# njspix/frender

Measured on AMD Instinct MI355X. Metric: M reads/sec scanned+classified (96 samples, 8+8bp, n=1) at 1/2/4/8 MI355X, higher is better.
Workload: dtype u8; 1 GPU; BASELINE config 2: 100000000 SYN-v1 reads/GPU, 96 samples, 8+8bp, n=1, R=8 (74 B/record), decoded FASTQ resident in HBM; reads_per_gpu=100000000, bytes_per_record=74, samples=96, nsubs=1, rc=False, unique_codes=1383958, table_checksum=a89b0e2c6adb2921, parallelism=1 GPU

## Files before the change

frender_amd/_lib.py:

```python
from __future__ import annotations

import ctypes as C
import os

import numpy as np

from . import _runtime

torch = None
if _runtime.USE_TORCH:
    try:
        import torch
    except Exception:
        torch = None

HERE = os.path.dirname(os.path.abspath(__file__))
LIB_PATH = os.environ.get("FRENDER_HIP_LIB", os.path.join(HERE, "libfrender_hip.so"))


def source_tree_hash() -> str:
    import hashlib

    h = hashlib.sha256()
    csrc = os.path.join(HERE, "csrc")
# ... 720 lines not shown
    def exotic_table(self):
        n, nb, npres = C.c_uint64(), C.c_uint64(), C.c_uint64()
        self._ck(lib.fr_exotic_sizes(self.h, C.byref(n), C.byref(nb), C.byref(npres)), "fr_exotic_sizes")
        counts = np.empty(n.value, np.uint64)
        first = np.empty(n.value, np.uint64)
        offs = np.empty(n.value + 1, np.uint64)
        data = np.empty(max(nb.value, 1), np.uint8)
        pc = np.empty(npres.value, np.uint32)
        pf = np.empty(npres.value, np.uint32)
        self._ck(lib.fr_get_exotic_table(self.h, _ptr(counts), _ptr(first), _ptr(offs), _ptr(data), _ptr(pc),
                                         _ptr(pf)), "fr_get_exotic_table")
        raw = data.tobytes()
        o = offs.tolist()
        codes = [raw[o[i]:o[i + 1]] for i in range(n.value)]
        return codes, counts, first, pc, pf

    def classify(self, num_subs: int, rc: bool, to_host: bool = True):
        n = self.U if to_host else 0
        out = {k: (np.empty(n, dtype=np.int16) if to_host else None) for k in ("m1", "m2", "row", "rc_m2", "rc_row")}
        out["cls"] = np.empty(n, dtype=np.uint8) if to_host else None
        out["rc_cls"] = np.empty(n, dtype=np.uint8) if to_host else None
        eu, ew = C.c_int64(), C.c_int32()
        self._ck(lib.fr_classify(self.h, num_subs, 1 if rc else 0, _ptr(out["m1"]), _ptr(out["m2"]),
                                 _ptr(out["cls"]), _ptr(out["row"]), _ptr(out["rc_m2"]), _ptr(out["rc_cls"]),
                                 _ptr(out["rc_row"]), C.byref(eu), C.byref(ew)), "fr_classify")
        out["err_unique"], out["err_which"] = eu.value, ew.value
        return out

    def rc_counts(self):
        f = np.zeros(max(self.n_names, 1), dtype=np.uint64)
        r = np.zeros(max(self.n_names, 1), dtype=np.uint64)
        self._ck(lib.fr_rc_counts(self.h, _ptr(f), _ptr(r)), "fr_rc_counts")
        return f[:self.n_names], r[:self.n_names]

    def classify_cp(self, q1: list, q2: list, num_subs: int, rc: bool):
        n = len(q1)
        stride = self.cp_stride
        a1 = np.zeros((n, stride), dtype=np.uint32)
        a2 = np.zeros((n, stride), dtype=np.uint32)
        for i, (x, y) in enumerate(zip(q1, q2)):
            a1[i, :min(len(x), stride)] = [ord(c) for c in x[:stride]]
            a2[i, :min(len(y), stride)] = [ord(c) for c in y[:stride]]
        l1 = np.array([len(x) for x in q1], dtype=np.int32)
        l2 = np.array([len(y) for y in q2], dtype=np.int32)
        out = {k: np.empty(n, dtype=np.int16) for k in ("m1", "m2", "row", "rc_m2", "rc_row")}
        out["cls"] = np.empty(n, dtype=np.uint8)
        out["rc_cls"] = np.empty(n, dtype=np.uint8)
        out["err"] = np.zeros(n, dtype=np.int32)
        self._ck(lib.fr_classify_cp(self.h, n, _ptr(a1), _ptr(l1), _ptr(a2), _ptr(l2), stride, num_subs,
                                    1 if rc else 0, _ptr(out["m1"]), _ptr(out["m2"]), _ptr(out["cls"]),
                                    _ptr(out["row"]), _ptr(out["rc_m2"]), _ptr(out["rc_cls"]), _ptr(out["rc_row"]),
                                    _ptr(out["err"])), "fr_classify_cp")
        return out

    def device_alloc(self, nbytes: int) -> int:
        p = lib.fr_device_alloc(self.h, nbytes)
        if not p:
            raise FrenderError(f"fr_device_alloc({nbytes}) failed")
        return p

    def device_free(self, p: int):
        self._ck(lib.fr_device_free(self.h, P(p)), "fr_device_free")

    def copy_to_host(self, dev_ptr: int, nbytes: int) -> bytes:
        out = np.empty(nbytes, dtype=np.uint8)
        self._ck(lib.fr_copy_to_host(self.h, _ptr(out), P(dev_ptr), nbytes), "fr_copy_to_host")
        return out.tobytes()

    def copy_to_device(self, dev_ptr: int, data: bytes):
        a = np.frombuffer(data, dtype=np.uint8)
        self._ck(lib.fr_copy_to_device(self.h, P(dev_ptr), _ptr(a), a.size), "fr_copy_to_device")

    def synth_device(self, dev_ptr: int, r0: int, n: int, R: int, seed: int, idx1: list, idx2: list):
        L1, L2 = len(idx1[0]), len(idx2[0])
        self._ck(lib.fr_synth_device(self.h, P(dev_ptr), r0, n, R, seed, "".join(idx1).encode(),
                                     "".join(idx2).encode(), len(idx1), L1, L2), "fr_synth_device")

    def timing(self) -> Timing:
        t = Timing()
        self._ck(lib.fr_get_timing(self.h, C.byref(t)), "fr_get_timing")
        return t

    def diag(self) -> dict:
        v = np.zeros(24, dtype=np.uint64)
        self._ck(lib.fr_get_diag(self.h, _ptr(v), 24), "fr_get_diag")
        d = dict(zip(("spin_max", "spin_total", "keys", "overflow", "presence", "exotic", "grid", "slots"),
                     v[:8].tolist()))
        d["spec_replays"] = int(v[16])
        d["exo_replays"] = int(v[17])
        d["chunk_tiles"] = int(v[18])
        d["heavy_launches"] = int(v[19])
        d["big_rollbacks"] = int(v[20])
        d["fold_max"] = int(v[21])
        d["fold_over"] = int(v[22])
        d["feed_step"] = int(v[23])
        if v[8:16].any():
            names = ("guess", "walk0", "wait0", "resolve", "walk1", "commit", "kernel", "chunks")
            d["stamps"] = dict(zip(names, v[8:].tolist()))
        return d

    def sync(self):
        self._ck(lib.fr_sync(self.h), "fr_sync")

    def set_timing(self, on: bool):
        self._ck(lib.fr_set_timing(self.h, 1 if on else 0), "fr_set_timing")

    def export_unique_device(self, keys_ptr: int, counts_ptr: int, first_ptr: int, cap: int):
        _torch_stream_done(self.device)
        self._ck(lib.fr_export_unique_device(self.h, P(keys_ptr), P(counts_ptr), P(first_ptr), cap),
                 "fr_export_unique_device")

    def merge_unique_device(self, keys_ptr: int, counts_ptr: int, first_ptr: int, n: int):
        self._ck(lib.fr_merge_unique_device(self.h, P(keys_ptr), P(counts_ptr), P(first_ptr), n),
                 "fr_merge_unique_device")

    def export_partitioned(self, world: int):
        U = int(self.U)
        dev = torch.device("cuda", self.device)
        rows = torch.empty((max(U, 1), 3), dtype=torch.int64, device=dev)
        cnt = torch.empty(2 * world, dtype=torch.int64, device=dev)
        _torch_stream_done(self.device)
        self._ck(lib.fr_export_partitioned_device(self.h, int(world), P(rows.data_ptr()), P(cnt.data_ptr()),
                                                  max(U, 1)), "fr_export_partitioned_device")
        return rows[:U], cnt[:world]

    def merge_rows_rowmajor(self, rows):
        n = int(rows.shape[0])
        if not n:
            return
        rows = rows.contiguous()
        torch.cuda.current_stream(rows.device).synchronize()
        self._ck(lib.fr_merge_rows_device(self.h, P(rows.data_ptr()), n), "fr_merge_rows_device")
        self.sync()

    def export_rows(self, device):
        U = int(self.U)
        cols = torch.empty((3, max(U, 1)), dtype=torch.int64, device=torch.device("cuda", self.device))
        if U:
            self.export_unique_device(cols[0].data_ptr(), cols[1].data_ptr(), cols[2].data_ptr(), U)
        return cols[:, :U].t().to(device)

    def merge_rows(self, rows):
        n = int(rows.shape[0])
        if not n:
            return
        cols = rows.t().contiguous().to(torch.device("cuda", self.device))
        torch.cuda.current_stream(cols.device).synchronize()
        self.merge_unique_device(cols[0].data_ptr(), cols[1].data_ptr(), cols[2].data_ptr(), n)
        self.sync()
```

frender_amd/csrc/fr_api.hip:

```cpp
#include <hip/hip_runtime.h>

#include <algorithm>
#include <cstddef>
#include <cstdio>
#include <cstdlib>
#include <cstring>
#include <string>
#include <thread>
#include <unordered_map>
#include <vector>

#include "../../include/frender_amd.h"
#include "fr_internal.h"

using namespace fr;

static void pinned_copy(u8* dst, const u8* src, u64 n) {
    constexpr u64 PART = 16ull << 20;
    const unsigned hw = std::max(1u, std::thread::hardware_concurrency());
    const u64 k = std::min<u64>({8, hw, n / PART});
    if (k < 2) {
        std::memcpy(dst, src, n);
        return;
    }
    std::vector<std::thread> t;
    const u64 per = (n + k - 1) / k;
    for (u64 i = 1; i < k; ++i) {
        const u64 b = i * per, e = std::min(n, b + per);
        if (b < e) t.emplace_back([=] { std::memcpy(dst + b, src + b, e - b); });
    }
    std::memcpy(dst, src, std::min(n, per));
    for (auto& x : t) x.join();
}

struct fr_ctx {
    int device = 0;
    GSlot* snap = nullptr;
    u64 snap_cap = 0;
    hipStream_t stream = nullptr;
    hipStream_t copy = nullptr;
    std::string err;
    int grid = 0;
    u32 flush_at = NS * 3 / 4;
    u64* cold = nullptr;
    u32 cold_cap = 8192;
    LogEntry* log = nullptr;
    u64 log_cap = 0;
    u32 log_rcap = 0;
    LogEntry* log_sub = nullptr;
    u32 log_scap = 0;
    void* log_temp = nullptr;
    size_t log_temp_bytes = 0;
    u32 log_min = 0;
    u32 log_hot = 0xFFFFFFFFu;
    uint4* rare = nullptr;

    DevState* st = nullptr;
    DevState* h_st = nullptr;
    DevState* h_zero = nullptr;
    u8* h_byte = nullptr;
    u64* h_fin = nullptr;
    hipEvent_t fin_e0 = nullptr, fin_e1 = nullptr;
    hipEvent_t cls_e0 = nullptr, cls_e1 = nullptr;
    bool fin_pending = false;
    u64 fin_expect = 0;
    bool st_fresh = false;
    Table* d_tab = nullptr;
    Table* h_tab = nullptr;
    hipEvent_t st_ev = nullptr;
    bool st_pending = false;
    u64* tiles = nullptr;
    u64* chunk_info = nullptr;
    u64 tiles_cap = 0;
    bool spec_ok = true;
    u64 spec_replays = 0;
    u64 big_rollbacks = 0;
    bool grow_sync = false;
    u32 spec_commit = 0;
    u32 epoch = 0;
    u32 par = 0;

    Table tab{};
    u64 nslots = 0;

    u64 chunk_bytes = 0;
    u64 ring_bytes = 0;
    u64 feed_keys = ~0ull;
    bool feed_logged = true;
    u32 feed_fold_max = 0;
    u32 feed_fold_over = 0;
    u64 feed_step = 0;
    u32 chunk_tiles = 320;
    u32 chunk_tiles_heavy = 448;
    u32 ramp_up_s = 1, ramp_down_s = 1;
    u32 ramp_down_pct = 100;
    u32 ramp_down_pct_h = 70;
    bool ramp = true;
    u8* pin[2] = {nullptr, nullptr};
    u8* dbuf[2] = {nullptr, nullptr};
    hipEvent_t copied[2] = {nullptr, nullptr};
    hipEvent_t consumed[2] = {nullptr, nullptr};
    bool used[2] = {false, false};
    int cur = 0;
    std::vector<u8> carry;

    bool scanning = false;
    bool file_open = false;
    u32 file_tag = 0;
    u32 first_tag = 0;
    u32 pres_defer_tag = 0;
    u64 file_base = 0;
    bool merged = false;
    u64 max_file_bytes = 0;
    u64 file_offset = 0;
    i64 max_records = 0;
    int last_byte = -1;
    u64 pres_before = 0;
    struct ExoCode {
        u64 count, first;
        u32 last_tag;
        u32 last_pair;
    };
    std::unordered_map<std::string, u32> exo_index;
    std::vector<std::string> exo_str;
    std::vector<ExoCode> exo_codes;
    std::vector<u32> exo_pres_code, exo_pres_file;
    std::vector<u64> exo_pres_count;
    u64 exo_new_file = 0;
    u64 exo_records_file = 0;
    bool host_feed = false;
    ScanArgs last_args{};
    int last_grid = 0;
    bool last_valid = false;
    u64 exo_replays = 0;
    bool sample_done = false;

    int S = -1;
    int n_names = 0;
    int L1u = -1, L2u = -1;
    u64 *d_i1 = nullptr, *d_i2 = nullptr, *d_i2rc = nullptr;
    int32_t* d_name = nullptr;
    u32 *d_cp1 = nullptr, *d_cp2 = nullptr, *d_cp2rc = nullptr;
    int32_t *d_cpl1 = nullptr, *d_cpl2 = nullptr;
    u8* d_sheet = nullptr;
    u8* h_sheet = nullptr;
    u64 sheet_cap = 0;
    u64 sheet_bytes = 0;
    int cp_stride = 0;
    int32_t* d_canon = nullptr;
    u64 sheet_ver = 0;

    u8* d_nbr = nullptr;
    u64 nbr_cap = 0;
    u64 nbr_ver = ~0ull;
    int nbr_nsubs = -1, nbr_rc = 0;
    NbrMap nbr{};
    bool nbr_enabled = true;

    u64 U = 0;
    u64 ucap = 0;
    u64 *d_keys = nullptr, *d_counts = nullptr, *d_first = nullptr;
    u64 *d_keys_s = nullptr, *d_counts_s = nullptr, *d_first_s = nullptr;
    u32 *d_pos = nullptr, *d_perm = nullptr, *d_rank = nullptr;
    u64* d_counter = nullptr;
    void* d_temp = nullptr;
    size_t temp_bytes = 0;
    u32 *d_bins = nullptr, *d_binbase = nullptr;
    u64 bins_cap = 0;
    u32* d_arr = nullptr;
    u64 arr_cap = 0;
    FinRow* d_rows = nullptr;
    u64 rows_cap = 0;
    u64 n_pres = 0;
    u64 pmap_cap = 0;
    u32 *d_pres_u = nullptr, *d_pres_f = nullptr;
    u64* d_pres_c = nullptr;
    u64 n_exo = 0;

    u64 ccap = 0;
    int16_t *d_m1 = nullptr, *d_m2 = nullptr, *d_row = nullptr, *d_rm2 = nullptr, *d_rrow = nullptr;
    u8 *d_cls = nullptr, *d_rcls = nullptr;
    int32_t* d_errw = nullptr;
    u64* d_errf = nullptr;
    u64 *d_rcf = nullptr, *d_rcr = nullptr;
    int rc_names_cap = 0;

    std::vector<hipEvent_t> ev_a, ev_b, ev_l;
    size_t ev_used = 0;
    u64 scan_launches = 0, scan_bytes = 0;
    double classify_ms = 0, finalize_ms = 0;
    bool timing = true;
    bool fin_timed = false;

    fr_infl* infl = nullptr;
};

namespace fr {
int infl_bgzf_file(fr_infl* z, const char* path, int* ok, const uint8_t** dev_out, uint64_t* out_len,
                   uint64_t* members);
}

#define CK(x)                                                                                  \
    do {                                                                                       \
        hipError_t e_ = (x);                                                                   \
        if (e_ != hipSuccess) {                                                                \
            ctx->err = std::string(#x) + ": " + hipGetErrorString(e_);                         \
            return FR_ERR_HIP;                                                                 \
        }                                                                                      \
    } while (0)

static int fail(fr_ctx* ctx, int code, const std::string& msg) {
    ctx->err = msg;
    return code;
}

template <class T>
static hipError_t dalloc(T** p, u64 n) {
    return hipMalloc((void**)p, std::max<u64>(n, 1) * sizeof(T));
}

static u64 pow2_at_least(u64 x) {
    u64 p = 1;
    while (p < x) p <<= 1;
    return p;
}

static int state_reset_counts(fr_ctx* ctx) {
    if (ctx->st_pending) CK(hipStreamSynchronize(ctx->stream));
    *ctx->h_st = *ctx->h_zero;
    CK(hipMemcpyAsync(ctx->st, ctx->h_zero, sizeof(DevState), hipMemcpyHostToDevice, ctx->stream));
    ctx->st_pending = false;
    ctx->st_fresh = true;
    return FR_OK;
}

static int read_state(fr_ctx* ctx) {
    if (ctx->st_fresh && !ctx->st_pending) return FR_OK;
    CK(hipMemcpyAsync(ctx->h_st, ctx->st, sizeof(DevState), hipMemcpyDeviceToHost, ctx->stream));
    CK(hipStreamSynchronize(ctx->stream));
    ctx->st_pending = false;
    ctx->st_fresh = true;
    return FR_OK;
}

static int grow_table(fr_ctx* ctx, bool force_bigger) {
    int rc = read_state(ctx);
    if (rc) return rc;
    const u64 nkeys = ctx->h_st->n_keys;
    const u64 novf = std::min<u64>(ctx->h_st->n_overflow, ctx->tab.ovf_cap);
    if (force_bigger || (nkeys + novf) * 2 > ctx->nslots) {
        u64 ns = ctx->nslots;
        while ((nkeys + novf) * 4 > ns) ns <<= 1;
        if (ns == ctx->nslots) ns <<= 1;
        GSlot* ns_slots = nullptr;
        CK(dalloc(&ns_slots, ns));
        CK(launch_table_init(ns_slots, ns, ctx->stream));
        Table t = ctx->tab;
        t.slots = ns_slots;
        t.mask = ns - 1;
        CK(launch_rehash(t, ctx->st, ctx->tab.slots, ctx->nslots, ctx->stream));
        CK(hipStreamSynchronize(ctx->stream));
        CK(hipFree(ctx->tab.slots));
        ctx->tab = t;
        ctx->nslots = ns;
    }
    if (novf) {
        Overflow* old = ctx->tab.ovf;
        Overflow* fresh = nullptr;
        CK(dalloc(&fresh, ctx->tab.ovf_cap));
        ctx->tab.ovf = fresh;
        CK(hipMemsetAsync(&ctx->st->n_overflow, 0, sizeof(u64), ctx->stream));
        CK(launch_reinsert_overflow(ctx->tab, ctx->st, old, novf, ctx->stream));
        ctx->st_fresh = false;
        CK(hipStreamSynchronize(ctx->stream));
        CK(hipFree(old));
    }
    return FR_OK;
}

static int ensure_presence_cap(fr_ctx* ctx) {
    int rc = read_state(ctx);
    if (rc) return rc;
    const u64 need = ctx->h_st->n_presence + ctx->h_st->n_keys + 1024;
    if (need <= ctx->tab.pres_cap) return FR_OK;
    u64 ncap = ctx->tab.pres_cap;
    while (ncap < need * 2) ncap *= 2;
    Presence* np = nullptr;
    CK(dalloc(&np, ncap));
    CK(hipMemcpyAsync(np, ctx->tab.pres, std::min(ctx->h_st->n_presence, ctx->tab.pres_cap) * sizeof(Presence),
                      hipMemcpyDeviceToDevice, ctx->stream));
    CK(hipStreamSynchronize(ctx->stream));
    CK(hipFree(ctx->tab.pres));
    ctx->tab.pres = np;
    ctx->tab.pres_cap = ncap;
    return FR_OK;
}

static int flush_presence(fr_ctx* ctx) {
    if (!ctx->pres_defer_tag) return FR_OK;
    int rc = ensure_presence_cap(ctx);
    if (rc) return rc;
    ctx->st_fresh = false;
    CK(launch_presence_scan(ctx->tab.slots, ctx->nslots, ctx->pres_defer_tag, ctx->tab.pres, ctx->tab.pres_cap,
                            ctx->st, ctx->stream));
    ctx->pres_defer_tag = 0;
    return read_state(ctx);
}

static int maybe_grow(fr_ctx* ctx) {
    if (ctx->st_pending) {
        if (ctx->grow_sync) CK(hipEventSynchronize(ctx->st_ev));
        else if (hipEventQuery(ctx->st_ev) != hipSuccess) return FR_OK;
        ctx->st_pending = false;
    } else if (!ctx->st_fresh) {
        return FR_OK;
    }
    const DevState& s = *ctx->h_st;
    if (s.n_overflow || s.n_keys * 2 > ctx->nslots) return grow_table(ctx, false);
    return FR_OK;
}

static int snapshot_async(fr_ctx* ctx) {
    CK(hipMemcpyAsync(ctx->h_st, ctx->st, sizeof(DevState), hipMemcpyDeviceToHost, ctx->stream));
    CK(hipEventRecord(ctx->st_ev, ctx->stream));
    ctx->st_pending = true;
    return FR_OK;
}

static int settle_finalize(fr_ctx* ctx) {
    if (!ctx->fin_pending) return FR_OK;
    ctx->fin_pending = false;
    CK(hipEventSynchronize(ctx->fin_e1));
    float ms = 0;
    if (ctx->fin_timed) CK(hipEventElapsedTime(&ms, ctx->fin_e0, ctx->fin_e1));
    ctx->finalize_ms = ms;
    if (*ctx->h_fin != ctx->fin_expect) return fail(ctx, FR_ERR_DEVICE, "compaction count mismatch");
    return FR_OK;
}

static int upload_table(fr_ctx* ctx) {
    if (std::memcmp(&ctx->tab, ctx->h_tab, sizeof(Table)) != 0) {
        CK(hipStreamSynchronize(ctx->stream));
        std::memcpy(ctx->h_tab, &ctx->tab, sizeof(Table));
        CK(hipMemcpyAsync(ctx->d_tab, ctx->h_tab, sizeof(Table), hipMemcpyHostToDevice, ctx->stream));
    }
    return FR_OK;
}

static int grow_exotic(fr_ctx* ctx, u64 need, u64 need_bytes) {
    if (need > ctx->tab.exo_cap) {
        CK(hipStreamSynchronize(ctx->stream));
        const u64 cap = std::max<u64>(need + need / 4, 2 * ctx->tab.exo_cap);
        CK(hipFree(ctx->tab.exo_ord));
        CK(hipFree(ctx->tab.exo_off));
        CK(hipFree(ctx->tab.exo_len));
        ctx->tab.exo_ord = nullptr;
        ctx->tab.exo_off = nullptr;
        ctx->tab.exo_len = nullptr;
        CK(dalloc(&ctx->tab.exo_ord, cap));
        CK(dalloc(&ctx->tab.exo_off, cap));
        CK(dalloc(&ctx->tab.exo_len, cap));
        ctx->tab.exo_cap = cap;
    }
    if (need_bytes > ctx->tab.exo_pool_cap) {
        CK(hipStreamSynchronize(ctx->stream));
        const u64 cap = std::max<u64>(need_bytes + need_bytes / 4, 2 * ctx->tab.exo_pool_cap);
        CK(hipFree(ctx->tab.exo_pool));
        ctx->tab.exo_pool = nullptr;
        CK(dalloc(&ctx->tab.exo_pool, cap));
        ctx->tab.exo_pool_cap = cap;
    }
    return upload_table(ctx);
}

static int drain_exotic(fr_ctx* ctx) {
    DevState& s = *ctx->h_st;
    const u64 n = s.n_exotic, used = s.exo_pool_used;
    if (!n) return FR_OK;
    if (n > ctx->tab.exo_cap || used > ctx->tab.exo_pool_cap)
        return fail(ctx, FR_ERR_DEVICE, "exotic list drained while overflowed");
    std::vector<u64> ord(n), off(n);
    std::vector<u32> len(n);
    std::vector<u8> pool(used);
    CK(hipMemcpyAsync(ord.data(), ctx->tab.exo_ord, n * 8, hipMemcpyDeviceToHost, ctx->stream));
    CK(hipMemcpyAsync(off.data(), ctx->tab.exo_off, n * 8, hipMemcpyDeviceToHost, ctx->stream));
    CK(hipMemcpyAsync(len.data(), ctx->tab.exo_len, n * 4, hipMemcpyDeviceToHost, ctx->stream));
    if (used) CK(hipMemcpyAsync(pool.data(), ctx->tab.exo_pool, used, hipMemcpyDeviceToHost, ctx->stream));
    CK(hipMemsetAsync(&ctx->st->n_exotic, 0, 2 * sizeof(u64), ctx->stream));
    CK(hipStreamSynchronize(ctx->stream));
    s.n_exotic = 0;
    s.exo_pool_used = 0;
    for (u64 i = 0; i < n; ++i) {
        std::string code((const char*)pool.data() + off[i], len[i]);
        auto it = ctx->exo_index.find(code);
        u32 k;
        if (it == ctx->exo_index.end()) {
            k = (u32)ctx->exo_codes.size();
            ctx->exo_index.emplace(code, k);
            ctx->exo_str.push_back(std::move(code));
            ctx->exo_codes.push_back({0, ~0ull, 0, 0});
        } else {
            k = it->second;
        }
        auto& e = ctx->exo_codes[k];
        e.count += 1;
        e.first = std::min(e.first, ord[i]);
        const u32 tag = (u32)(ord[i] >> ORD_SHIFT);
        if (e.last_tag != tag) {
            e.last_tag = tag;
            e.last_pair = (u32)ctx->exo_pres_code.size();
            ctx->exo_pres_code.push_back(k);
            ctx->exo_pres_file.push_back(tag - 1u);
            ctx->exo_pres_count.push_back(0);
            ctx->exo_new_file++;
        }
        ctx->exo_pres_count[e.last_pair] += 1;
    }
    ctx->exo_records_file += n;
    return FR_OK;
}

static int launch_args(fr_ctx* ctx, const ScanArgs& a, int grid);

static int replay_exotic(fr_ctx* ctx) {
    if (!ctx->last_valid) return fail(ctx, FR_ERR_DEVICE, "exotic overflow without a launch to replay");
    DevState& s = *ctx->h_st;
    int rc = grow_exotic(ctx, s.n_exotic, s.exo_pool_used);
    if (rc) return rc;
    s.n_exotic = 0;
    s.exo_pool_used = 0;
    s.cap_flags &= ~4u;
    CK(hipMemsetAsync(&ctx->st->n_exotic, 0, 2 * sizeof(u64), ctx->stream));
    CK(hipMemcpyAsync(&ctx->st->cap_flags, &s.cap_flags, sizeof(u32), hipMemcpyHostToDevice, ctx->stream));
    ScanArgs a = ctx->last_args;
    a.exo_only = 1;
    a.spec_commit = 0;
    a.log = nullptr;
    a.epoch = ++ctx->epoch;
    a.tab = ctx->d_tab;
    a.tabv = ctx->tab;
    CK(hipMemsetAsync(&ctx->st->ticket, 0, 2 * sizeof(u32), ctx->stream));
    rc = launch_args(ctx, a, ctx->last_grid);
    if (rc) return rc;
    ctx->exo_replays++;
    ctx->st_fresh = false;
    rc = read_state(ctx);
    if (rc) return rc;
    if (ctx->h_st->cap_flags & 4u) return fail(ctx, FR_ERR_DEVICE, "exotic replay overflowed");
    return FR_OK;
}

static int settle_exotic(fr_ctx* ctx) {
    int rc = read_state(ctx);
    if (rc) return rc;
    if (ctx->h_st->cap_flags & 4u) {
        rc = replay_exotic(ctx);
        if (rc) return rc;
    }
    return drain_exotic(ctx);
}

static int launch_args(fr_ctx* ctx, const ScanArgs& a, int grid) {
    if (a.num_tiles > ctx->tiles_cap) return fail(ctx, FR_ERR_INVALID, "range larger than the look-back array");
    ctx->st_fresh = false;
    CK(launch_chunk_scan(a, grid, ctx->stream));
    return FR_OK;
}

static int launch_range(fr_ctx* ctx, const u8* dptr, u64 len, u64 avail, int own_start, int own_end, int pre_valid,
                        int exo_only = 0) {
    if (len == 0) return FR_OK;
    int rc = FR_OK;
    if (ctx->host_feed && ctx->last_valid) {
        rc = settle_exotic(ctx);
        if (rc) return rc;
    }
    rc = maybe_grow(ctx);
    if (rc) return rc;
    ScanArgs a;
    std::memset(&a, 0, sizeof(a));
    a.buf = dptr;
    a.len = len;
    a.avail = avail;
    a.file_offset = ctx->file_offset;
    a.file_tag = ctx->file_tag;
    a.par = ctx->par;
    a.epoch = ++ctx->epoch;
    a.num_tiles = (u32)((len + TSTEP - 1) / TSTEP);
    a.own_start = own_start;
    a.own_end = own_end;
    a.pre_valid = pre_valid;
    a.flush_at = ctx->flush_at;
    a.max_records = ctx->max_records;
    a.st = ctx->st;
    a.tiles = ctx->tiles;
    a.chunk_info = ctx->chunk_info;
    a.spec_commit = exo_only ? 0u : ctx->spec_commit;
    a.exo_only = (u32)exo_only;
    rc = upload_table(ctx);
    if (rc) return rc;
    a.tab = ctx->d_tab;
    a.tabv = ctx->tab;
    if (ctx->epoch >= 0x7FFFFFFFu) {
        CK(hipMemsetAsync(ctx->tiles, 0, ctx->tiles_cap * sizeof(u64), ctx->stream));
        ctx->epoch = 1;
        a.epoch = 1;
    }
    ctx->st_fresh = false;
    const bool timed = ctx->timing;
    if (timed && ctx->ev_used == ctx->ev_a.size()) {
        hipEvent_t e1, e2, e3;
        CK(hipEventCreate(&e1));
        CK(hipEventCreate(&e2));
        CK(hipEventCreate(&e3));
        ctx->ev_a.push_back(e1);
        ctx->ev_b.push_back(e2);
        ctx->ev_l.push_back(e3);
    }
    if (timed) CK(hipEventRecord(ctx->ev_a[ctx->ev_used], ctx->stream));
    const u64 G = (u64)ctx->grid, C = ctx->chunk_tiles, Ch = ctx->chunk_tiles_heavy;
    const u64 Gd = std::max<u64>(1, G * ctx->ramp_down_pct / 100), Gdh = std::max<u64>(1, G * ctx->ramp_down_pct_h / 100);
    a.ramp_up_s = ctx->ramp_up_s;
    a.ramp_down_s = ctx->ramp_down_s;
    a.ramp_down_g = (u32)Gd;
    a.ramp_down_g_h = (u32)Gdh;
    auto ramps = [&](u64 c, u64 gd) {
        return ramp_tiles_before(c, G, std::min<u64>(ctx->ramp_up_s, c), G) +
               ramp_tiles_before(c, gd, std::min<u64>(ctx->ramp_down_s, c), gd);
    };
    const u64 rg = ramps(C, Gd), rgh = ramps(Ch, Gdh);
    if (ctx->ramp && (u64)a.num_tiles >= rg + C) {
        a.ramp_g = (u32)G;
        a.chunk_tiles = (u32)C;
        a.mid_chunks = (u32)(((u64)a.num_tiles - rg + C - 1) / C);
        a.num_chunks = (u32)(G + Gd) + a.mid_chunks;
        if (Ch != C && (u64)a.num_tiles >= rgh + Ch) {
            a.chunk_tiles_h = (u32)Ch;
            a.mid_chunks_h = (u32)(((u64)a.num_tiles - rgh + Ch - 1) / Ch);
            a.num_chunks_h = (u32)(G + Gdh) + a.mid_chunks_h;
        }
    } else {
        a.ramp_g = 0;
        a.mid_chunks = 0;
        a.chunk_tiles = (u32)std::max<u64>(1, (a.num_tiles + G - 1) / G);
        a.num_chunks = (a.num_tiles + a.chunk_tiles - 1) / a.chunk_tiles;
    }
    a.cold_cap = ctx->cold_cap;
    a.cold = ctx->cold;
    a.log = exo_only ? nullptr : LOG_DIRECT ? ctx->log_sub : ctx->log;
    a.log_cap = LOG_DIRECT ? (u64)ctx->log_scap * LOG_NSUB : ctx->log_cap;
    a.log_rcap = LOG_DIRECT ? ctx->log_scap : ctx->log_rcap;
    a.log_min = ctx->log_min;
    a.log_hot = ctx->log_hot;
    a.rare = ctx->rare;
    const int grid = (int)std::min<u64>(a.num_chunks, G);
    rc = launch_args(ctx, a, grid);
    if (rc) return rc;
    ctx->last_args = a;
    ctx->last_grid = grid;
    ctx->last_valid = true;
    if (timed) CK(hipEventRecord(ctx->ev_b[ctx->ev_used], ctx->stream));
    if (a.log)
        CK(launch_log_aggregate(ctx->tab, ctx->st, ctx->log, ctx->log_rcap, ctx->log_sub, ctx->log_scap, a.file_tag,
                                a.file_offset, ctx->stream));
    if (timed) {
        CK(hipEventRecord(ctx->ev_l[ctx->ev_used], ctx->stream));
        ctx->ev_used++;
    }
    ctx->scan_launches++;
    ctx->scan_bytes += len;
    ctx->par ^= 1u;
    ctx->file_offset += len;
    ctx->max_file_bytes = std::max(ctx->max_file_bytes, ctx->file_offset);
    return snapshot_async(ctx);
}

extern "C" {

void fr_tuning_defaults(fr_tuning* t) {
    if (!t) return;
    const fr_ctx d{};
    std::memset(t, 0, sizeof(*t));
    t->size = sizeof(fr_tuning);
    t->grid = 0;
    t->flush_at = d.flush_at;
    t->cold_cap = d.cold_cap;
    t->log = 1;
    t->log_min = d.log_min;
    t->log_hot = d.log_hot;
    t->chunk_tiles = d.chunk_tiles;
    t->chunk_tiles_heavy = d.chunk_tiles_heavy;
    t->ramp = d.ramp ? 1 : 0;
    t->ramp_up_s = d.ramp_up_s;
    t->ramp_down_s = d.ramp_down_s;
    t->ramp_down_pct = d.ramp_down_pct;
    t->ramp_down_pct_h = d.ramp_down_pct_h;
    t->spec_commit = d.spec_ok ? 1 : 0;
    t->nbr = d.nbr_enabled ? 1 : 0;
    t->ovf_cap = 0;
}

fr_ctx* fr_create(int device, uint64_t chunk_bytes, uint64_t table_slots) {
    return fr_create_tuned(device, chunk_bytes, table_slots, nullptr);
}

fr_ctx* fr_create_tuned(int device, uint64_t chunk_bytes, uint64_t table_slots, const fr_tuning* tuning) {
    fr_tuning t;
    fr_tuning_defaults(&t);
    if (tuning) {
        const size_t n = std::min<size_t>(std::max<uint32_t>(tuning->size, sizeof(uint32_t)), sizeof(fr_tuning));
        std::memcpy((char*)&t + sizeof(uint32_t), (const char*)tuning + sizeof(uint32_t), n - sizeof(uint32_t));
    }
    fr_ctx* ctx = new fr_ctx();
    ctx->device = device;
    auto bad = [&](const char* what, hipError_t e) {
        ctx->err = std::string(what) + ": " + hipGetErrorString(e);
        return ctx;
    };
    hipError_t e;
    if ((e = hipSetDevice(device)) != hipSuccess) return bad("hipSetDevice", e);
    if ((e = hipStreamCreateWithFlags(&ctx->stream, hipStreamNonBlocking)) != hipSuccess) return bad("stream", e);
    if ((e = hipStreamCreateWithFlags(&ctx->copy, hipStreamNonBlocking)) != hipSuccess) return bad("stream", e);
    hipDeviceProp_t prop;
    if ((e = hipGetDeviceProperties(&prop, device)) != hipSuccess) return bad("props", e);
    const int per_cu = chunk_occupancy();
    ctx->grid = t.grid > 0 ? t.grid : prop.multiProcessorCount * per_cu;
    ctx->flush_at = std::min<u32>(t.flush_at, NS);
    ctx->nbr_enabled = t.nbr != 0;
    ctx->cold_cap = std::max<u32>(1024, t.cold_cap);
    ctx->log_min = t.log_min;
    ctx->log_hot = std::max<u32>(1, t.log_hot);
    ctx->chunk_tiles = std::max<u32>(2, t.chunk_tiles);
    ctx->chunk_tiles_heavy = std::max<u32>(2, t.chunk_tiles_heavy);
    ctx->ramp = t.ramp != 0;
    ctx->ramp_up_s = std::max<u32>(1, t.ramp_up_s);
    ctx->ramp_down_s = std::max<u32>(1, t.ramp_down_s);
    ctx->ramp_down_pct = std::min<u32>(100, std::max<u32>(1, t.ramp_down_pct));
    ctx->ramp_down_pct_h = std::min<u32>(100, std::max<u32>(1, t.ramp_down_pct_h));
    ctx->spec_ok = t.spec_commit != 0;
    if ((e = dalloc(&ctx->cold, 2ull * ctx->cold_cap * (u64)ctx->grid)) != hipSuccess) return bad("cold lists", e);
    if ((e = dalloc(&ctx->rare, (u64)RARE_RING * (u64)ctx->grid)) != hipSuccess) return bad("rare rings", e);

    ctx->chunk_bytes = chunk_bytes ? ((chunk_bytes + TILE - 1) / TILE) * TILE : (256ull << 20);
    if (ctx->chunk_bytes > RANGE_MAX) ctx->chunk_bytes = RANGE_MAX;
    ctx->ring_bytes = std::min<u64>(ctx->chunk_bytes, HOST_CHUNK_MAX);
    if (t.log) {
        const u64 want = std::min<u64>(std::max<u64>(ctx->chunk_bytes / 256, 1ull << 16), 1ull << 26);
        ctx->log_rcap = (u32)(want / LOG_NR);
        ctx->log_cap = (u64)ctx->log_rcap * LOG_NR;
        ctx->log_scap = (u32)std::max<u64>(2ull * ctx->log_rcap / LOG_SUBS, 64);
        if (!LOG_DIRECT && (e = dalloc(&ctx->log, ctx->log_cap)) != hipSuccess) return bad("launch log", e);
        if ((e = dalloc(&ctx->log_sub, (u64)ctx->log_scap * LOG_NSUB)) != hipSuccess) return bad("launch log parts", e);
    }
    ctx->tiles_cap = RANGE_MAX / TSTEP + 2;
    ctx->nslots = pow2_at_least(std::max<u64>(table_slots, 1024));
    if ((e = hipMalloc((void**)&ctx->st, sizeof(DevState))) != hipSuccess) return bad("state", e);
    if ((e = hipMalloc((void**)&ctx->d_tab, sizeof(Table))) != hipSuccess) return bad("table copy", e);
    if ((e = hipHostMalloc((void**)&ctx->h_tab, sizeof(Table), hipHostMallocDefault)) != hipSuccess)
        return bad("table staging", e);
    std::memset(ctx->h_tab, 0, sizeof(Table));
    if ((e = hipHostMalloc((void**)&ctx->h_st, sizeof(DevState), hipHostMallocDefault)) != hipSuccess)
        return bad("pinned state", e);
    if ((e = hipHostMalloc((void**)&ctx->h_byte, 64, hipHostMallocDefault)) != hipSuccess) return bad("pinned byte", e);
    if ((e = hipHostMalloc((void**)&ctx->h_fin, 64, hipHostMallocDefault)) != hipSuccess) return bad("pinned count", e);
    if ((e = hipEventCreate(&ctx->fin_e0)) != hipSuccess) return bad("event", e);
    if ((e = hipEventCreate(&ctx->fin_e1)) != hipSuccess) return bad("event", e);
    if ((e = hipEventCreate(&ctx->cls_e0)) != hipSuccess) return bad("event", e);
    if ((e = hipEventCreate(&ctx->cls_e1)) != hipSuccess) return bad("event", e);
    if ((e = hipHostMalloc((void**)&ctx->h_zero, sizeof(DevState), hipHostMallocDefault)) != hipSuccess)
        return bad("pinned reset state", e);
    std::memset(ctx->h_zero, 0, sizeof(DevState));
    ctx->h_zero->err_nospace = ~0ull;
    if ((e = hipEventCreateWithFlags(&ctx->st_ev, hipEventDisableTiming)) != hipSuccess) return bad("event", e);
    if ((e = dalloc(&ctx->tiles, ctx->tiles_cap)) != hipSuccess) return bad("tiles", e);
    if ((e = dalloc(&ctx->chunk_info, ctx->tiles_cap)) != hipSuccess) return bad("chunk info", e);
    if ((e = hipMemset(ctx->tiles, 0, ctx->tiles_cap * sizeof(u64))) != hipSuccess) return bad("tiles", e);
    if ((e = dalloc(&ctx->tab.slots, ctx->nslots)) != hipSuccess) return bad("table", e);
    ctx->tab.mask = ctx->nslots - 1;
    ctx->tab.ovf_cap = t.ovf_cap ? std::max<u64>(t.ovf_cap, 1024) : (1ull << 22);
    ctx->tab.pres_cap = 1ull << 22;
    ctx->tab.exo_cap = 1ull << 20;
    ctx->tab.exo_pool_cap = 64ull << 20;
    if ((e = dalloc(&ctx->tab.ovf, ctx->tab.ovf_cap)) != hipSuccess) return bad("overflow", e);
    if ((e = dalloc(&ctx->tab.pres, ctx->tab.pres_cap)) != hipSuccess) return bad("presence", e);
    if ((e = dalloc(&ctx->tab.exo_ord, ctx->tab.exo_cap)) != hipSuccess) return bad("exotic", e);
    if ((e = dalloc(&ctx->tab.exo_off, ctx->tab.exo_cap)) != hipSuccess) return bad("exotic", e);
    if ((e = dalloc(&ctx->tab.exo_len, ctx->tab.exo_cap)) != hipSuccess) return bad("exotic", e);
    if ((e = dalloc(&ctx->tab.exo_pool, ctx->tab.exo_pool_cap)) != hipSuccess) return bad("exotic", e);
    for (int i = 0; i < 2; ++i) {
        if ((e = hipHostMalloc((void**)&ctx->pin[i], ctx->ring_bytes, hipHostMallocDefault)) != hipSuccess)
            return bad("pinned ring", e);
        if ((e = dalloc(&ctx->dbuf[i], ctx->ring_bytes + 64)) != hipSuccess) return bad("device ring", e);
        if ((e = hipEventCreateWithFlags(&ctx->copied[i], hipEventDisableTiming)) != hipSuccess) return bad("event", e);
        if ((e = hipEventCreateWithFlags(&ctx->consumed[i], hipEventDisableTiming)) != hipSuccess)
            return bad("event", e);
        if ((e = hipEventRecord(ctx->consumed[i], ctx->stream)) != hipSuccess) return bad("event", e);
    }
    if ((e = dalloc(&ctx->d_counter, 1)) != hipSuccess) return bad("counter", e);
    if (fr_reset(ctx) != FR_OK) return ctx;
    ctx->err.clear();
    return ctx;
}

void fr_destroy(fr_ctx* ctx) {
    if (!ctx) return;
    if (ctx->infl) fr_infl_destroy(ctx->infl);
    (void)hipSetDevice(ctx->device);
    if (ctx->stream) (void)hipStreamSynchronize(ctx->stream);
    if (ctx->copy) (void)hipStreamSynchronize(ctx->copy);
    void* dev[] = {ctx->st, ctx->d_tab, ctx->tiles, ctx->tab.slots, ctx->tab.ovf, ctx->tab.pres, ctx->tab.exo_ord,
                   ctx->tab.exo_off, ctx->tab.exo_len, ctx->tab.exo_pool, ctx->dbuf[0], ctx->dbuf[1], ctx->d_sheet,
                   ctx->d_keys, ctx->d_counts, ctx->d_first, ctx->d_keys_s, ctx->d_counts_s,
                   ctx->d_first_s, ctx->d_pos, ctx->d_perm, ctx->d_rank, ctx->d_counter, ctx->d_temp, ctx->d_bins, ctx->d_binbase, ctx->d_arr, ctx->d_rows, ctx->d_pres_u,
                   ctx->d_pres_f, ctx->d_pres_c, ctx->d_m1, ctx->d_m2, ctx->d_row, ctx->d_rm2, ctx->d_rrow, ctx->d_cls, ctx->d_rcls,
                   ctx->d_errw, ctx->d_errf, ctx->d_nbr, ctx->cold, ctx->rare, ctx->chunk_info, ctx->log, ctx->log_sub, ctx->log_temp,
                   ctx->snap};
    for (void* p : dev)
        if (p) (void)hipFree(p);
    if (ctx->h_st) (void)hipHostFree(ctx->h_st);
    if (ctx->h_zero) (void)hipHostFree(ctx->h_zero);
    if (ctx->h_byte) (void)hipHostFree(ctx->h_byte);
    if (ctx->h_fin) (void)hipHostFree(ctx->h_fin);
    if (ctx->fin_e0) (void)hipEventDestroy(ctx->fin_e0);
    if (ctx->fin_e1) (void)hipEventDestroy(ctx->fin_e1);
    if (ctx->cls_e0) (void)hipEventDestroy(ctx->cls_e0);
    if (ctx->cls_e1) (void)hipEventDestroy(ctx->cls_e1);
    if (ctx->h_sheet) (void)hipHostFree(ctx->h_sheet);
    if (ctx->h_tab) (void)hipHostFree(ctx->h_tab);
    for (int i = 0; i < 2; ++i) {
        if (ctx->pin[i]) (void)hipHostFree(ctx->pin[i]);
        if (ctx->copied[i]) (void)hipEventDestroy(ctx->copied[i]);
        if (ctx->consumed[i]) (void)hipEventDestroy(ctx->consumed[i]);
    }
    for (auto e : ctx->ev_a) (void)hipEventDestroy(e);
    for (auto e : ctx->ev_b) (void)hipEventDestroy(e);
    for (auto e : ctx->ev_l) (void)hipEventDestroy(e);
    if (ctx->st_ev) (void)hipEventDestroy(ctx->st_ev);
    if (ctx->stream) (void)hipStreamDestroy(ctx->stream);
    if (ctx->copy) (void)hipStreamDestroy(ctx->copy);
    delete ctx;
}

const char* fr_last_error(const fr_ctx* ctx) { return ctx ? ctx->err.c_str() : "null context"; }

int fr_get_diag(fr_ctx* ctx, uint64_t* out, int n) {
    if (int src = settle_finalize(ctx)) return src;
    int rc = read_state(ctx);
    if (rc) return rc;
    const DevState& s = *ctx->h_st;
    const uint64_t v[] = {s.spin_max,   s.spin_total, s.n_keys,   s.n_overflow, s.n_presence, s.n_exotic,
                          (uint64_t)ctx->grid, ctx->nslots, s.stamp[0], s.stamp[1], s.stamp[2], s.stamp[3],
                          s.stamp[4],  s.stamp[5],  s.stamp[6], s.stamp[7], ctx->spec_replays, ctx->exo_replays,
                          s.heavy[ctx->par] ? ctx->chunk_tiles_heavy : ctx->chunk_tiles,
                          s.heavy_launches, ctx->big_rollbacks, ctx->feed_fold_max, ctx->feed_fold_over, ctx->feed_step};
    for (int i = 0; i < n && i < (int)(sizeof(v) / sizeof(v[0])); ++i) out[i] = v[i];
    return FR_OK;
}

int fr_sync(fr_ctx* ctx) {
    CK(hipStreamSynchronize(ctx->stream));
    CK(hipStreamSynchronize(ctx->copy));
    return settle_finalize(ctx);
}

int fr_get_timing(fr_ctx* ctx, fr_timing* out) {
    CK(hipStreamSynchronize(ctx->stream));
    if (int src = settle_finalize(ctx)) return src;
    double tot = 0, last = 0, lg = 0;
    for (size_t i = 0; i < ctx->ev_used; ++i) {
        float ms = 0, ml = 0;
        CK(hipEventElapsedTime(&ms, ctx->ev_a[i], ctx->ev_b[i]));
        CK(hipEventElapsedTime(&ml, ctx->ev_b[i], ctx->ev_l[i]));
        tot += ms;
        last = ms;
        lg += ml;
    }
    out->log_ms = lg;
    out->scan_launches = ctx->scan_launches;
    out->scan_bytes = ctx->scan_bytes;
    out->scan_ms = tot;
    out->last_scan_ms = last;
    out->classify_ms = ctx->classify_ms;
    out->finalize_ms = ctx->finalize_ms;
    return FR_OK;
}

int fr_set_timing(fr_ctx* ctx, int on) {
    if (!ctx) return FR_ERR_INVALID;
    ctx->timing = on != 0;
    return FR_OK;
}

int fr_set_sheet(fr_ctx* ctx, int S, const uint64_t* idx1_packed, const int32_t* idx1_len,
                 const uint64_t* idx2_packed, const int32_t* idx2_len, const uint64_t* idx2rc_packed,
                 const int32_t* name_id, int n_names, const uint32_t* idx1_cp, const uint32_t* idx2_cp,
                 const uint32_t* idx2rc_cp, int cp_stride) {
    if (S < 0 || S > 32767) return fail(ctx, FR_ERR_INVALID, "sheet rows must be in [0, 32767]");
    const bool with_cp = idx1_cp && idx2_cp && idx2rc_cp && cp_stride > 0 && S > 0;
    const u64 ncp = with_cp ? (u64)S * cp_stride : 0;
    auto al = [](u64 b) { return (b + 7) & ~7ull; };
    const u64 o_i2 = al(S * 8ull), o_i2rc = o_i2 + al(S * 8ull), o_name = o_i2rc + al(S * 8ull);
    const u64 o_cp1 = o_name + al(S * 4ull), o_cp2 = o_cp1 + al(ncp * 4), o_cp2rc = o_cp2 + al(ncp * 4);
    const u64 o_l1 = o_cp2rc + al(ncp * 4), o_l2 = o_l1 + (with_cp ? al(S * 4ull) : 0);
    const u64 o_canon = o_l2 + (with_cp ? al(S * 4ull) : 0);
    const u64 total = o_canon + al(3 * S * 4ull) + 8;
    std::vector<u8> blob(total, 0);
    u8* h = blob.data();
    if (S) {
        std::memcpy(h, idx1_packed, S * 8ull);
        std::memcpy(h + o_i2, idx2_packed, S * 8ull);
        std::memcpy(h + o_i2rc, idx2rc_packed, S * 8ull);
        std::memcpy(h + o_name, name_id, S * 4ull);
    }
    if (with_cp) {
        std::memcpy(h + o_cp1, idx1_cp, ncp * 4);
        std::memcpy(h + o_cp2, idx2_cp, ncp * 4);
        std::memcpy(h + o_cp2rc, idx2rc_cp, ncp * 4);
        std::memcpy(h + o_l1, idx1_len, S * 4ull);
        std::memcpy(h + o_l2, idx2_len, S * 4ull);
    }
    const bool same = ctx->h_sheet && total == ctx->sheet_bytes && std::memcmp(h, ctx->h_sheet, o_canon) == 0;
    if (!same && S) {
        const uint64_t* lists[3] = {idx1_packed, idx2_packed, idx2rc_packed};
        int32_t* canon = (int32_t*)(h + o_canon);
        for (int l = 0; l < 3; ++l) {
            std::unordered_map<u64, int32_t> first;
            first.reserve(S * 2);
            for (int i = 0; i < S; ++i) canon[l * S + i] = first.emplace(lists[l][i], i).first->second;
        }
    }
    if (!same) {
        CK(hipStreamSynchronize(ctx->stream));
        if (total > ctx->sheet_cap) {
            if (ctx->d_sheet) CK(hipFree(ctx->d_sheet));
            if (ctx->h_sheet) CK(hipHostFree(ctx->h_sheet));
            ctx->d_sheet = nullptr;
            ctx->h_sheet = nullptr;
            const u64 cap = std::max<u64>(total * 2, 4096);
            CK(hipMalloc(&ctx->d_sheet, cap));
            CK(hipHostMalloc(&ctx->h_sheet, cap, hipHostMallocDefault));
            ctx->sheet_cap = cap;
        }
        std::memcpy(ctx->h_sheet, h, total);
        ctx->sheet_bytes = total;
        ++ctx->sheet_ver;
        CK(hipMemcpyAsync(ctx->d_sheet, ctx->h_sheet, total, hipMemcpyHostToDevice, ctx->stream));
    }
    u8* d = ctx->d_sheet;
    ctx->d_i1 = (u64*)d;
    ctx->d_i2 = (u64*)(d + o_i2);
    ctx->d_i2rc = (u64*)(d + o_i2rc);
    ctx->d_name = (int32_t*)(d + o_name);
    ctx->d_cp1 = with_cp ? (u32*)(d + o_cp1) : nullptr;
    ctx->d_cp2 = with_cp ? (u32*)(d + o_cp2) : nullptr;
    ctx->d_cp2rc = with_cp ? (u32*)(d + o_cp2rc) : nullptr;
    ctx->d_cpl1 = with_cp ? (int32_t*)(d + o_l1) : nullptr;
    ctx->d_cpl2 = with_cp ? (int32_t*)(d + o_l2) : nullptr;
    ctx->d_canon = (int32_t*)(d + o_canon);
    ctx->cp_stride = with_cp ? cp_stride : 0;
    ctx->S = S;
    ctx->n_names = n_names;
    auto common = [&](const int32_t* l) {
        if (S == 0) return -1;
        for (int i = 1; i < S; ++i)
            if (l[i] != l[0]) return -2;
        return (int)l[0];
    };
    ctx->L1u = common(idx1_len);
    ctx->L2u = common(idx2_len);
    return FR_OK;
}

int fr_reset(fr_ctx* ctx) {
    if (int src = settle_finalize(ctx)) return src;
    CK(hipSetDevice(ctx->device));
    CK(hipStreamSynchronize(ctx->copy));
    CK(launch_table_init(ctx->tab.slots, ctx->nslots, ctx->stream));
    int rc = state_reset_counts(ctx);
    if (rc) return rc;
    ctx->scanning = true;
    ctx->file_open = false;
    ctx->file_tag = 0;
    ctx->first_tag = 0;
    ctx->pres_defer_tag = 0;
    ctx->merged = false;
    ctx->max_file_bytes = 0;
    ctx->par = 0;
    ctx->U = 0;
    ctx->n_pres = 0;
    ctx->n_exo = 0;
    ctx->exo_index.clear();
    ctx->exo_str.clear();
    ctx->exo_codes.clear();
    ctx->exo_pres_code.clear();
    ctx->exo_pres_file.clear();
    ctx->exo_pres_count.clear();
    ctx->last_valid = false;
    ctx->ev_used = 0;
    ctx->scan_launches = ctx->scan_bytes = 0;
    ctx->classify_ms = ctx->finalize_ms = 0;
    ctx->st_pending = false;
    return FR_OK;
}

int fr_begin_file(fr_ctx* ctx, int64_t max_records) {
    return fr_begin_file_at(ctx, (int64_t)ctx->file_tag, 0, max_records);
}

int fr_begin_file_at(fr_ctx* ctx, int64_t file_index, uint64_t byte_base, int64_t max_records) {
    if (int src = settle_finalize(ctx)) return src;
    if (ctx->file_open) return fail(ctx, FR_ERR_INVALID, "fr_begin_file: a file is already open");
    if (file_index < 0 || file_index + 1 >= (1 << 19)) return fail(ctx, FR_ERR_INVALID, "too many files in one scan");
    if ((u32)file_index + 1u <= ctx->file_tag)
        return fail(ctx, FR_ERR_INVALID, "fr_begin_file_at: file indices must increase within a scan");
    if (byte_base >= (1ull << ORD_SHIFT)) return fail(ctx, FR_ERR_INVALID, "fr_begin_file_at: byte base too large");
    int rc = flush_presence(ctx);
    if (rc) return rc;
    rc = read_state(ctx);
    if (rc) return rc;
    ctx->pres_before = ctx->h_st->n_presence;
    ctx->exo_new_file = 0;
    ctx->exo_records_file = 0;
    ctx->last_valid = false;
    static_assert(offsetof(DevState, utf8_bad) + sizeof(u32) - offsetof(DevState, lines) == 32, "per-file block");
    CK(hipMemcpyAsync(&ctx->st->lines[0], &ctx->h_zero->lines[0], 32, hipMemcpyHostToDevice, ctx->stream));
    ctx->h_st->lines[0] = ctx->h_st->lines[1] = 0;
    ctx->h_st->err_nospace = ~0ull;
    ctx->h_st->nonascii = ctx->h_st->utf8_bad = 0;
    ctx->file_tag = (u32)file_index + 1u;
    if (!ctx->first_tag) ctx->first_tag = ctx->file_tag;
    ctx->file_offset = byte_base;
    ctx->file_base = byte_base;
    ctx->max_records = max_records > 0 ? max_records : 0;
    ctx->last_byte = -1;
    ctx->carry.clear();
    ctx->sample_done = false;
    ctx->par = 0;
    ctx->file_open = true;
    return FR_OK;
}

static int check_sample(fr_ctx* ctx) {
    if (ctx->max_records <= 0) return FR_OK;
    int rc = read_state(ctx);
    if (rc) return rc;
    const u64 lines = ctx->h_st->lines[ctx->par];
    if (lines + 3 >= 4ull * (u64)ctx->max_records) ctx->sample_done = true;
    return FR_OK;
}

static int ship_slot(fr_ctx* ctx, int slot, u64 n) {
    CK(hipStreamWaitEvent(ctx->copy, ctx->consumed[slot], 0));
    CK(hipMemcpyAsync(ctx->dbuf[slot], ctx->pin[slot], n, hipMemcpyHostToDevice, ctx->copy));
    CK(hipEventRecord(ctx->copied[slot], ctx->copy));
    CK(hipStreamWaitEvent(ctx->stream, ctx->copied[slot], 0));
    int rc = launch_range(ctx, ctx->dbuf[slot], n, n, 1, 0, 0);
    if (rc) return rc;
    CK(hipEventRecord(ctx->consumed[slot], ctx->stream));
    ctx->used[slot] = true;
    return FR_OK;
}

int fr_feed(fr_ctx* ctx, const uint8_t* data, uint64_t len) {
    if (!ctx->file_open) return fail(ctx, FR_ERR_INVALID, "fr_feed: no open file");
    ctx->host_feed = true;
    if (ctx->sample_done) return FR_SAMPLE_DONE;
    if (len) ctx->last_byte = data[len - 1];
    u64 done = 0;
    while (done < len) {
        const int slot = ctx->cur;
        if (ctx->used[slot]) CK(hipEventSynchronize(ctx->copied[slot]));
        u8* pin = ctx->pin[slot];
        const u64 nc = ctx->carry.size();
        if (nc >= ctx->ring_bytes) return fail(ctx, FR_ERR_CAPACITY, "a line is longer than the chunk size");
        if (nc) std::memcpy(pin, ctx->carry.data(), nc);
        const u64 take = std::min<u64>(len - done, ctx->ring_bytes - nc);
        pinned_copy(pin + nc, data + done, take);
        done += take;
        const u64 n = nc + take;
        u64 cut = n;
        while (cut > 0 && !(pin[cut - 1] == '\n' || (pin[cut - 1] == '\r' && cut < n && pin[cut] != '\n'))) --cut;
        if (cut == 0) {
            ctx->carry.assign(pin, pin + n);
            continue;
        }
        ctx->carry.assign(pin + cut, pin + n);
        int rc = ship_slot(ctx, slot, cut);
        if (rc) return rc;
        ctx->cur ^= 1;
        rc = check_sample(ctx);
        if (rc) return rc;
        if (ctx->sample_done) return FR_SAMPLE_DONE;
    }
    return FR_OK;
}

int fr_feed_device(fr_ctx* ctx, const uint8_t* dev_data, uint64_t len) {
    if (!ctx->file_open) return fail(ctx, FR_ERR_INVALID, "fr_feed_device: no open file");
    if (ctx->file_offset != ctx->file_base || !ctx->carry.empty())
        return fail(ctx, FR_ERR_INVALID, "fr_feed_device takes a whole file (no prior fr_feed)");
    if (((uintptr_t)dev_data & 15u) != 0) return fail(ctx, FR_ERR_INVALID, "device data must be 16-byte aligned");
    ctx->host_feed = false;
    int rc = settle_exotic(ctx);
    if (rc) return rc;
    const DevState saved = *ctx->h_st;
    const u32 par0 = ctx->par;
    const u64 snap_slots = ctx->nslots;
    const bool empty = saved.n_keys == 0 && saved.n_overflow == 0;
    const bool spec = ctx->spec_ok && ctx->max_records == 0 && saved.n_overflow == 0;
    GSlot* snap = nullptr;
    if (spec && !empty) {
        if (ctx->snap_cap < snap_slots) {
            if (ctx->snap) {
                CK(hipStreamSynchronize(ctx->stream));
                CK(hipFree(ctx->snap));
                ctx->snap = nullptr;
            }
            ctx->snap_cap = 0;
            CK(dalloc(&ctx->snap, snap_slots));
            ctx->snap_cap = snap_slots;
        }
        snap = ctx->snap;
        CK(hipMemcpyAsync(snap, ctx->tab.slots, snap_slots * sizeof(GSlot), hipMemcpyDeviceToDevice, ctx->stream));
    }
    const double big_range = (double)std::min<u64>(ctx->chunk_bytes, len);
    const bool fold_room = (u64)ctx->feed_fold_over * 64 <= ctx->feed_fold_max && ctx->feed_step > 0 &&
                           (double)ctx->feed_fold_max * big_range <= 0.85 * AGG_LNS * (double)ctx->feed_step;
    bool big = spec && (!ctx->feed_logged || fold_room) && ctx->feed_keys != ~0ull &&
               (saved.n_keys + ctx->feed_keys) * 2 <= ctx->nslots;
    bool spec_now = spec;
    u64 step = 0, lim_room = ~0ull;
    for (int attempt = 0; attempt < 12; ++attempt) {
        CK(hipMemsetAsync(&ctx->st->log_fold_max, 0, 2 * sizeof(u32), ctx->stream));
        const u64 lim = std::min<u64>(big ? ctx->chunk_bytes : std::min<u64>(ctx->chunk_bytes, RANGE_FIRST_MAX),
                                      lim_room);
        const u64 nr = (len + lim - 1) / lim;
        step = nr ? (len + nr - 1) / nr : 0;
        ctx->spec_commit = spec_now ? 1u : 0u;
        for (u64 off = 0; off < len; off += step) {
            const u64 n = std::min<u64>(step, len - off);
            rc = launch_range(ctx, dev_data + off, n, len - off, off == 0 ? 1 : 0, 1, off ? 1 : 0);
            if (rc) break;
        }
        ctx->spec_commit = 0;
        if (!rc && len) CK(hipMemcpyAsync(ctx->h_byte, dev_data + len - 1, 1, hipMemcpyDeviceToHost, ctx->stream));
        if (!rc) rc = read_state(ctx);
        if (rc) break;
        const bool spec_bad = spec_now && ctx->h_st->spec_fail;
        const bool room_bad = spec && (ctx->h_st->cap_flags & 2u) && step > RANGE_ROOM_MIN;
        if (!spec_bad && !room_bad) break;
        if (room_bad) {
            big = false;
            lim_room = std::max<u64>(RANGE_ROOM_MIN, ((step / 8) + TILE - 1) / TILE * TILE);
            ctx->grow_sync = true;
            ctx->big_rollbacks++;
        } else {
            spec_now = false;
        }
        if (ctx->nslots != snap_slots) {
            GSlot* fresh = nullptr;
            if ((rc = (dalloc(&fresh, snap_slots) == hipSuccess) ? FR_OK : fail(ctx, FR_ERR_DEVICE, "rollback alloc")))
                break;
            CK(hipStreamSynchronize(ctx->stream));
            CK(hipFree(ctx->tab.slots));
            ctx->tab.slots = fresh;
            ctx->tab.mask = snap_slots - 1;
            ctx->nslots = snap_slots;
        }
        if (empty) CK(launch_table_init(ctx->tab.slots, ctx->nslots, ctx->stream));
        else CK(hipMemcpyAsync(ctx->tab.slots, snap, snap_slots * sizeof(GSlot), hipMemcpyDeviceToDevice, ctx->stream));
        *ctx->h_st = saved;
        CK(hipMemcpyAsync(ctx->st, ctx->h_st, sizeof(DevState), hipMemcpyHostToDevice, ctx->stream));
        CK(hipStreamSynchronize(ctx->stream));
        ctx->st_pending = false;
        ctx->st_fresh = true;
        ctx->par = par0;
        ctx->file_offset = ctx->file_base;
        if (!room_bad) ctx->spec_replays++;
    }
    ctx->grow_sync = false;
    if (rc) return rc;
    ctx->feed_keys = ctx->h_st->n_keys - saved.n_keys;
    ctx->feed_logged = ctx->h_st->log_commits != saved.log_commits;
    ctx->feed_fold_max = ctx->h_st->log_fold_max;
    ctx->feed_fold_over = ctx->h_st->log_fold_over;
    ctx->feed_step = step;
    rc = read_state(ctx);
    if (rc) return rc;
    if (ctx->h_st->cap_flags & 4u) {
        DevState& s = *ctx->h_st;
        rc = grow_exotic(ctx, s.n_exotic, s.exo_pool_used);
        if (rc) return rc;
        s.n_exotic = 0;
        s.exo_pool_used = 0;
        s.cap_flags &= ~4u;
        s.lines[par0] = saved.lines[par0];
        CK(hipMemcpyAsync(ctx->st, ctx->h_st, sizeof(DevState), hipMemcpyHostToDevice, ctx->stream));
        ctx->par = par0;
        ctx->file_offset = ctx->file_base;
        ctx->exo_replays++;
        for (u64 off = 0; off < len && !rc; off += step) {
            const u64 n = std::min<u64>(step, len - off);
            rc = launch_range(ctx, dev_data + off, n, len - off, off == 0 ? 1 : 0, 1, off ? 1 : 0, 1);
        }
        if (rc) return rc;
        ctx->st_fresh = false;
        rc = read_state(ctx);
        if (rc) return rc;
        if (ctx->h_st->cap_flags & 4u) return fail(ctx, FR_ERR_DEVICE, "exotic replay overflowed");
    }
    rc = drain_exotic(ctx);
    if (rc) return rc;
    if (len) ctx->last_byte = *ctx->h_byte;
    ctx->carry.clear();
    return FR_OK;
}

int fr_feed_bgzf(fr_ctx* ctx, const char* path, int* decoded, uint64_t* members, uint64_t* bytes) {
    if (!decoded || !path) return fail(ctx, FR_ERR_INVALID, "fr_feed_bgzf: null argument");
    *decoded = 0;
    if (members) *members = 0;
    if (bytes) *bytes = 0;
    if (!ctx->file_open) return fail(ctx, FR_ERR_INVALID, "fr_feed_bgzf: no open file");
    if (ctx->file_base != 0 || ctx->file_offset != 0 || !ctx->carry.empty())
        return fail(ctx, FR_ERR_INVALID, "fr_feed_bgzf takes a whole file from its first byte (no prior feed)");
    if (ctx->max_records > 0) return FR_OK;
    if (!ctx->infl) {
        ctx->infl = fr_infl_create(ctx->device);
        if (!ctx->infl || *fr_infl_last_error(ctx->infl)) {
            const std::string msg = ctx->infl ? fr_infl_last_error(ctx->infl) : "fr_infl_create returned NULL";
            if (ctx->infl) fr_infl_destroy(ctx->infl);
            ctx->infl = nullptr;
            return fail(ctx, FR_ERR_HIP, msg);
        }
    }
    int ok = 0;
    const uint8_t* dev = nullptr;
    uint64_t len = 0, n = 0;
    int rc = infl_bgzf_file(ctx->infl, path, &ok, &dev, &len, &n);
    if (rc) return fail(ctx, rc, std::string("fr_feed_bgzf: ") + fr_infl_last_error(ctx->infl));
    if (!ok) return FR_OK;
    rc = fr_feed_device(ctx, dev, len);
    if (rc) return rc;
    *decoded = 1;
    if (members) *members = n;
    if (bytes) *bytes = len;
    return FR_OK;
}

int fr_end_file(fr_ctx* ctx, fr_file_stats* out) {
    if (!ctx->file_open) return fail(ctx, FR_ERR_INVALID, "fr_end_file: no open file");
    if (!ctx->carry.empty() && !ctx->sample_done) {
        const int slot = ctx->cur;
        if (ctx->used[slot]) CK(hipEventSynchronize(ctx->copied[slot]));
        std::memcpy(ctx->pin[slot], ctx->carry.data(), ctx->carry.size());
        const u64 n = ctx->carry.size();
        ctx->carry.clear();
        int rc = ship_slot(ctx, slot, n);
        if (rc) return rc;
        ctx->cur ^= 1;
    }
    ctx->carry.clear();
    CK(hipStreamSynchronize(ctx->copy));
    int rc = ctx->host_feed ? settle_exotic(ctx) : FR_OK;
    if (rc) return rc;
    ctx->last_valid = false;
    rc = grow_table(ctx, false);
    if (rc) return rc;
    const bool defer = ctx->file_tag == ctx->first_tag && !ctx->merged && ctx->pres_before == 0 &&
                       ctx->h_st->n_presence == 0;
    if (!defer) {
        rc = ensure_presence_cap(ctx);
        if (rc) return rc;
        ctx->st_fresh = false;
        CK(launch_presence_scan(ctx->tab.slots, ctx->nslots, ctx->file_tag, ctx->tab.pres, ctx->tab.pres_cap,
                                ctx->st, ctx->stream));
    }
    rc = read_state(ctx);
    if (rc) return rc;
    const DevState& s = *ctx->h_st;
    if (s.spin_fail) return fail(ctx, FR_ERR_DEVICE, "tally look-back exceeded its spin bound");
    if (s.cap_flags) return fail(ctx, FR_ERR_CAPACITY, "a device list overflowed (flags " + std::to_string(s.cap_flags) + ")");
    u64 lines = s.lines[ctx->par];
    const bool ended = ctx->last_byte == '\n' || ctx->last_byte == '\r';
    if (ctx->last_byte >= 0 && !ended && !ctx->sample_done) lines += 1;
    u64 records = (lines + 3) / 4;
    if (ctx->max_records > 0 && records > (u64)ctx->max_records) records = (u64)ctx->max_records;
    std::memset(out, 0, sizeof(*out));
    out->records = records;
    out->lines = lines;
    out->new_keys = (defer ? s.n_keys : s.n_presence - ctx->pres_before) + ctx->exo_new_file;
    if (defer) ctx->pres_defer_tag = ctx->file_tag;
    out->exotic = ctx->exo_records_file;
    out->error = FR_SCAN_OK;
    if (s.utf8_bad) {
        out->error = FR_SCAN_UTF8;
        out->utf8_bad = 1;
    }
    if (s.err_nospace != ~0ull) {
        out->error = FR_SCAN_NO_SPACE;
        out->error_offset = s.err_nospace;
    }
    ctx->file_open = false;
    return FR_OK;
}

int fr_finalize(fr_ctx* ctx, uint64_t* n_unique, uint64_t* n_presence, uint64_t* n_exotic) {
    if (ctx->file_open) return fail(ctx, FR_ERR_INVALID, "fr_finalize: a file is still open");
    int rc = settle_finalize(ctx);
    if (rc) return rc;
    hipEvent_t e0 = ctx->fin_e0, e1 = ctx->fin_e1;
    rc = grow_table(ctx, false);
    if (rc) return rc;
    rc = read_state(ctx);
    if (rc) return rc;
    const u64 nk = ctx->h_st->n_keys;
    if (nk > 0xFFFFFFFFull) return fail(ctx, FR_ERR_CAPACITY, "more than 2^32 unique codes");
    if (nk > ctx->ucap) {
        void* old[] = {ctx->d_keys, ctx->d_counts, ctx->d_first, ctx->d_keys_s, ctx->d_counts_s, ctx->d_first_s,
                       ctx->d_pos, ctx->d_perm, ctx->d_rank, ctx->d_temp};
        for (void* p : old)
            if (p) CK(hipFree(p));
        ctx->d_temp = nullptr;
        ctx->temp_bytes = 0;
        const u64 cap = std::max<u64>(nk + nk / 4, 1024);
        CK(dalloc(&ctx->d_keys, cap));
        CK(dalloc(&ctx->d_counts, cap));
        CK(dalloc(&ctx->d_first, cap));
        CK(dalloc(&ctx->d_keys_s, cap));
        CK(dalloc(&ctx->d_counts_s, cap));
        CK(dalloc(&ctx->d_first_s, cap));
        CK(dalloc(&ctx->d_pos, cap));
        CK(dalloc(&ctx->d_perm, cap));
        CK(dalloc(&ctx->d_rank, cap));
        ctx->ucap = cap;
    }
    if (ctx->timing) CK(hipEventRecord(e0, ctx->stream));
    ctx->fin_timed = ctx->timing;
    BinMap bm{0, 0, 0, 0, 0};
    u64 nbins = 0;
    if (!ctx->merged && ctx->first_tag && ctx->file_tag >= ctx->first_tag) {
        const u64 ntags = (u64)(ctx->file_tag - ctx->first_tag) + 1u;
        bm.span = std::max<u64>(ctx->max_file_bytes, 1);
        bm.first_tag = ctx->first_tag;
        bm.shift = 13;
        const u64 range = ntags * bm.span;
        while (bm.shift < 20 && ((range >> bm.shift) + 1) > (1ull << 21)) ++bm.shift;
        nbins = (range >> bm.shift) + 1;
        if (nbins > (1ull << 21)) nbins = 0;
    }
    if (nbins) {
        bm.nbins = nbins;
        bm.cap = ctx->ucap;
        if (ctx->nslots > ctx->arr_cap) {
            if (ctx->d_arr) CK(hipFree(ctx->d_arr));
            ctx->d_arr = nullptr;
            CK(hipMalloc(&ctx->d_arr, ctx->nslots * sizeof(u32)));
            ctx->arr_cap = ctx->nslots;
        }
        if (ctx->ucap > ctx->rows_cap) {
            if (ctx->d_rows) CK(hipFree(ctx->d_rows));
            ctx->d_rows = nullptr;
            CK(hipMalloc(&ctx->d_rows, ctx->ucap * sizeof(FinRow)));
            ctx->rows_cap = ctx->ucap;
        }
        if (nbins + 1 > ctx->bins_cap) {
            if (ctx->d_bins) CK(hipFree(ctx->d_bins));
            if (ctx->d_binbase) CK(hipFree(ctx->d_binbase));
            ctx->d_bins = ctx->d_binbase = nullptr;
            const u64 cap = std::max<u64>(nbins + 1, 1u << 16);
            CK(hipMalloc(&ctx->d_bins, cap * sizeof(u32)));
            CK(hipMalloc(&ctx->d_binbase, cap * sizeof(u32)));
            ctx->bins_cap = cap;
        }
        size_t need = 0;
        CK(launch_fin_scan(ctx->d_bins, ctx->d_binbase, nbins + 1, nullptr, &need, ctx->stream));
        if (need > ctx->temp_bytes) {
            if (ctx->d_temp) CK(hipFree(ctx->d_temp));
            CK(hipMalloc(&ctx->d_temp, need));
            ctx->temp_bytes = need;
        }
        size_t tb = ctx->temp_bytes;
        const bool set_uidx = ctx->pres_defer_tag == 0;
        CK(hipMemsetAsync(ctx->d_bins, 0, (nbins + 1) * sizeof(u32), ctx->stream));
        CK(launch_fin_hist(ctx->tab.slots, ctx->nslots, bm, ctx->d_bins, ctx->d_arr, ctx->stream));
        CK(launch_fin_scan(ctx->d_bins, ctx->d_binbase, nbins + 1, ctx->d_temp, &tb, ctx->stream));
        CK(launch_fin_scatter(ctx->tab.slots, ctx->nslots, bm, ctx->d_binbase, ctx->d_arr, ctx->d_rows, ctx->stream));
        CK(launch_fin_rank(ctx->tab.slots, nk, bm, ctx->d_binbase, ctx->d_rows, ctx->d_keys_s, ctx->d_counts_s,
                           ctx->d_first_s, set_uidx, ctx->stream));
    } else {
        CK(hipMemsetAsync(ctx->d_counter, 0, sizeof(u64), ctx->stream));
        CK(launch_compact(ctx->tab.slots, ctx->nslots, ctx->d_keys, ctx->d_counts, ctx->d_first, ctx->d_pos,
                          ctx->d_counter, ctx->stream));
        int begin_bit = 0, end_bit = 64;
        if (!ctx->merged) {
            begin_bit = 2;
            end_bit = ORD_SHIFT;
            while (end_bit < 64 && ((u64)ctx->file_tag >> (end_bit - ORD_SHIFT)) != 0) ++end_bit;
            if (ctx->file_tag == ctx->first_tag) {
                end_bit = begin_bit + 1;
                while (end_bit < ORD_SHIFT && (ctx->max_file_bytes >> end_bit) != 0) ++end_bit;
            }
        }
        size_t need = 0;
        CK(launch_order(ctx->d_first, ctx->d_pos, nk, ctx->d_first_s, ctx->d_perm, nullptr, &need, begin_bit, end_bit,
                        ctx->stream));
        if (need > ctx->temp_bytes) {
            if (ctx->d_temp) CK(hipFree(ctx->d_temp));
            CK(hipMalloc(&ctx->d_temp, need));
            ctx->temp_bytes = need;
        }
        size_t tb = ctx->temp_bytes;
        if (nk)
            CK(launch_order(ctx->d_first, ctx->d_pos, nk, ctx->d_first_s, ctx->d_perm, ctx->d_temp, &tb, begin_bit,
                            end_bit, ctx->stream));
        CK(launch_gather(ctx->d_perm, nk, ctx->d_keys, ctx->d_counts, ctx->d_keys_s, ctx->d_counts_s, ctx->d_rank,
                         ctx->stream));
        CK(launch_set_uidx(ctx->tab.slots, ctx->tab.mask, ctx->d_keys_s, nk, ctx->d_rank, ctx->stream));
    }
    const u64 np = ctx->pres_defer_tag ? nk : std::min<u64>(ctx->h_st->n_presence, ctx->tab.pres_cap);
    if (np > ctx->pmap_cap) {
        if (ctx->d_pres_u) CK(hipFree(ctx->d_pres_u));
        if (ctx->d_pres_f) CK(hipFree(ctx->d_pres_f));
        if (ctx->d_pres_c) CK(hipFree(ctx->d_pres_c));
        CK(dalloc(&ctx->d_pres_u, np));
        CK(dalloc(&ctx->d_pres_f, np));
        CK(dalloc(&ctx->d_pres_c, np));
        ctx->pmap_cap = np;
    }
    if (ctx->pres_defer_tag)
        CK(launch_presence_one_file(ctx->d_counts_s, np, ctx->pres_defer_tag, ctx->d_pres_u, ctx->d_pres_f,
                                    ctx->d_pres_c, ctx->stream));
    else
        CK(launch_presence_map(ctx->tab.slots, ctx->tab.mask, ctx->tab.pres, np, ctx->d_pres_u, ctx->d_pres_f,
                               ctx->d_pres_c, ctx->stream));
    *ctx->h_fin = 0;
    if (nbins)
        CK(hipMemcpyAsync(ctx->h_fin, ctx->d_binbase + nbins, sizeof(u32), hipMemcpyDeviceToHost, ctx->stream));
    else
        CK(hipMemcpyAsync(ctx->h_fin, ctx->d_counter, sizeof(u64), hipMemcpyDeviceToHost, ctx->stream));
    CK(hipEventRecord(e1, ctx->stream));
    ctx->fin_pending = true;
    ctx->fin_expect = nk;
    ctx->U = nk;
    ctx->n_pres = np;
    ctx->n_exo = ctx->exo_codes.size();
    if (n_unique) *n_unique = ctx->U;
    if (n_presence) *n_presence = ctx->n_pres;
    if (n_exotic) *n_exotic = ctx->n_exo;
    return FR_OK;
}

int fr_get_unique(fr_ctx* ctx, uint64_t* keys, uint64_t* counts, uint64_t* first_ordinal) {
    if (int src = settle_finalize(ctx)) return src;
    const u64 n = ctx->U;
    if (!n) return FR_OK;
    if (keys) CK(hipMemcpy(keys, ctx->d_keys_s, n * 8, hipMemcpyDeviceToHost));
    if (counts) CK(hipMemcpy(counts, ctx->d_counts_s, n * 8, hipMemcpyDeviceToHost));
    if (first_ordinal) CK(hipMemcpy(first_ordinal, ctx->d_first_s, n * 8, hipMemcpyDeviceToHost));
    return FR_OK;
}

int fr_get_presence(fr_ctx* ctx, uint32_t* unique_idx, uint32_t* file_idx) {
    if (int src = settle_finalize(ctx)) return src;
    const u64 n = ctx->n_pres;
    if (!n) return FR_OK;
    CK(hipMemcpy(unique_idx, ctx->d_pres_u, n * 4, hipMemcpyDeviceToHost));
    CK(hipMemcpy(file_idx, ctx->d_pres_f, n * 4, hipMemcpyDeviceToHost));
    return FR_OK;
}

int fr_get_presence_counts(fr_ctx* ctx, uint64_t* counts, uint64_t* exotic_counts) {
    if (int src = settle_finalize(ctx)) return src;
    const u64 n = ctx->n_pres;
    if (counts && n) {
        std::vector<u32> u(n);
        CK(hipMemcpy(u.data(), ctx->d_pres_u, n * 4, hipMemcpyDeviceToHost));
        CK(hipMemcpy(counts, ctx->d_pres_c, n * 8, hipMemcpyDeviceToHost));
        std::vector<u64> last(ctx->U, 0);
        const u64 m = (1ull << (64 - PRES_TAG_BITS)) - 1ull;
        for (u64 i = 0; i < n; ++i) {
            if (u[i] >= ctx->U) return fail(ctx, FR_ERR_DEVICE, "presence pair without a unique code");
            const u64 snap = counts[i];
            counts[i] = (snap - last[u[i]]) & m;
            last[u[i]] = snap;
        }
    }
    const u64 ne = ctx->exo_pres_count.size();
    if (exotic_counts && ne) std::memcpy(exotic_counts, ctx->exo_pres_count.data(), ne * 8);
    return FR_OK;
}

int fr_exotic_sizes(fr_ctx* ctx, uint64_t* n_codes, uint64_t* code_bytes, uint64_t* n_presence) {
    if (int src = settle_finalize(ctx)) return src;
    u64 b = 0;
    for (const auto& c : ctx->exo_str) b += c.size();
    if (n_codes) *n_codes = ctx->exo_str.size();
    if (code_bytes) *code_bytes = b;
    if (n_presence) *n_presence = ctx->exo_pres_code.size();
    return FR_OK;
}

int fr_get_exotic_table(fr_ctx* ctx, uint64_t* counts, uint64_t* first, uint64_t* offsets, uint8_t* bytes,
                        uint32_t* pres_code, uint32_t* pres_file) {
    if (int src = settle_finalize(ctx)) return src;
    const u64 n = ctx->exo_str.size();
    u64 b = 0;
    for (u64 i = 0; i < n; ++i) {
        if (counts) counts[i] = ctx->exo_codes[i].count;
        if (first) first[i] = ctx->exo_codes[i].first;
        if (offsets) offsets[i] = b;
        if (bytes) std::memcpy(bytes + b, ctx->exo_str[i].data(), ctx->exo_str[i].size());
        b += ctx->exo_str[i].size();
    }
    if (offsets) offsets[n] = b;
    const u64 np = ctx->exo_pres_code.size();
    if (pres_code && np) std::memcpy(pres_code, ctx->exo_pres_code.data(), np * 4);
    if (pres_file && np) std::memcpy(pres_file, ctx->exo_pres_file.data(), np * 4);
    return FR_OK;
}

static int ensure_class_scratch(fr_ctx* ctx, u64 n) {
    if (n <= ctx->ccap && ctx->n_names <= ctx->rc_names_cap && ctx->d_errf) return FR_OK;
    void* old[] = {ctx->d_m1, ctx->d_m2, ctx->d_row, ctx->d_rm2, ctx->d_rrow, ctx->d_cls, ctx->d_rcls, ctx->d_errw,
                   ctx->d_errf};
    for (void* p : old)
        if (p) CK(hipFree(p));
    const u64 cap = std::max<u64>(std::max(n, ctx->ccap), 1024);
    CK(dalloc(&ctx->d_m1, cap));
    CK(dalloc(&ctx->d_m2, cap));
    CK(dalloc(&ctx->d_row, cap));
    CK(dalloc(&ctx->d_rm2, cap));
    CK(dalloc(&ctx->d_rrow, cap));
    CK(dalloc(&ctx->d_cls, cap));
    CK(dalloc(&ctx->d_rcls, cap));
    CK(dalloc(&ctx->d_errw, cap));
    const int names = std::max(ctx->n_names, 1);
    CK(dalloc(&ctx->d_errf, 1 + 2 * (u64)names));
    ctx->d_rcf = ctx->d_errf + 1;
    ctx->d_rcr = ctx->d_rcf + names;
    ctx->ccap = cap;
    ctx->rc_names_cap = names;
    return FR_OK;
}

static int ensure_nbr(fr_ctx* ctx, const SheetArgs& sh, int nsubs, int rc) {
    constexpr u64 NBR_MAX = 1ull << 21;
    if (ctx->nbr_ver == ctx->sheet_ver && ctx->nbr_nsubs == nsubs && (ctx->nbr_rc || !rc)) return FR_OK;
    ctx->nbr.on = 0;
    ctx->nbr_ver = ctx->sheet_ver;
    ctx->nbr_nsubs = nsubs;
    ctx->nbr_rc = rc;
    if (!ctx->nbr_enabled || sh.S <= 0 || nsubs < 0 || sh.L1u < 0 || sh.L1u > 21 || sh.L2u < 0 || sh.L2u > 21)
        return FR_OK;
    const u64 c1 = (u64)sh.S * nbr_codes_per_row(sh.L1u, nsubs), c2 = (u64)sh.S * nbr_codes_per_row(sh.L2u, nsubs);
    if (c1 > NBR_MAX || c2 > NBR_MAX) return FR_OK;
    const u64 n1 = std::max<u64>(pow2_at_least(2 * c1), 1024), n2 = std::max<u64>(pow2_at_least(2 * c2), 1024);
    const u64 np = std::max<u64>(pow2_at_least(2 * (u64)sh.S), 64);
    const u64 bytes = (n1 + 2 * n2) * sizeof(NSlot) + 2 * np * sizeof(PSlot);
    if (bytes > ctx->nbr_cap) {
        CK(hipStreamSynchronize(ctx->stream));
        if (ctx->d_nbr) CK(hipFree(ctx->d_nbr));
        ctx->d_nbr = nullptr;
        ctx->nbr_cap = 0;
        CK(hipMalloc(&ctx->d_nbr, bytes));
        ctx->nbr_cap = bytes;
    }
    NbrMap& m = ctx->nbr;
    m.m[0] = (NSlot*)ctx->d_nbr;
    m.m[1] = m.m[0] + n1;
    m.m[2] = m.m[1] + n2;
    m.p[0] = (PSlot*)(m.m[2] + n2);
    m.p[1] = m.p[0] + np;
    m.mmask[0] = (u32)(n1 - 1);
    m.mmask[1] = m.mmask[2] = (u32)(n2 - 1);
    m.pmask[0] = m.pmask[1] = (u32)(np - 1);
    CK(hipMemsetAsync(ctx->d_nbr, 0, bytes, ctx->stream));
    CK(launch_nbr_build(sh, ctx->d_canon, nsubs, rc, m, ctx->stream));
    m.on = 1;
    return FR_OK;
}

int fr_classify(fr_ctx* ctx, int num_subs, int rc_mode, int16_t* m1, int16_t* m2, uint8_t* cls, int16_t* row,
                int16_t* rc_m2, uint8_t* rc_cls, int16_t* rc_row, int64_t* err_unique, int32_t* err_which) {
    if (ctx->S < 0) return fail(ctx, FR_ERR_INVALID, "fr_classify: no sheet");
    const u64 n = ctx->U;
    int rc = ensure_class_scratch(ctx, n);
    if (rc) return rc;
    hipEvent_t e0 = ctx->cls_e0, e1 = ctx->cls_e1;
    CK(hipMemsetAsync(ctx->d_errf, 0, (1 + 2 * (u64)ctx->rc_names_cap) * 8, ctx->stream));
    SheetArgs sh{ctx->S, ctx->n_names, ctx->L1u, ctx->L2u, ctx->d_i1, ctx->d_i2, ctx->d_i2rc, ctx->d_name};
    if ((rc = ensure_nbr(ctx, sh, num_subs, rc_mode ? 1 : 0))) return rc;
    ClassOut o{ctx->d_m1, ctx->d_m2, ctx->d_cls, ctx->d_row, ctx->d_rm2, ctx->d_rcls, ctx->d_rrow,
               ctx->d_rcf, ctx->d_rcr, ctx->d_errf, ctx->d_errw};
    const bool timed = ctx->timing;
    if (timed) CK(hipEventRecord(e0, ctx->stream));
    CK(launch_classify(ctx->d_keys_s, ctx->d_counts_s, n, sh, num_subs, rc_mode ? 1 : 0, o, ctx->nbr, ctx->stream));
    if (timed) CK(hipEventRecord(e1, ctx->stream));
    CK(hipMemcpyAsync(ctx->h_byte + 8, ctx->d_errf, 8, hipMemcpyDeviceToHost, ctx->stream));
    CK(hipStreamSynchronize(ctx->stream));
    u64 ef;
    std::memcpy(&ef, ctx->h_byte + 8, 8);
    ef = ~ef;
    if (int src = settle_finalize(ctx)) return src;
    float ms = 0;
    if (timed) CK(hipEventElapsedTime(&ms, e0, e1));
    ctx->classify_ms = ms;
    if (err_unique) *err_unique = ef == ~0ull ? -1 : (int64_t)ef;
    if (err_which) {
        *err_which = 0;
        if (ef != ~0ull) CK(hipMemcpy(err_which, ctx->d_errw + ef, 4, hipMemcpyDeviceToHost));
    }
    if (n) {
        if (m1) CK(hipMemcpy(m1, ctx->d_m1, n * 2, hipMemcpyDeviceToHost));
        if (m2) CK(hipMemcpy(m2, ctx->d_m2, n * 2, hipMemcpyDeviceToHost));
        if (cls) CK(hipMemcpy(cls, ctx->d_cls, n, hipMemcpyDeviceToHost));
        if (row) CK(hipMemcpy(row, ctx->d_row, n * 2, hipMemcpyDeviceToHost));
        if (rc_mode) {
            if (rc_m2) CK(hipMemcpy(rc_m2, ctx->d_rm2, n * 2, hipMemcpyDeviceToHost));
            if (rc_cls) CK(hipMemcpy(rc_cls, ctx->d_rcls, n, hipMemcpyDeviceToHost));
            if (rc_row) CK(hipMemcpy(rc_row, ctx->d_rrow, n * 2, hipMemcpyDeviceToHost));
        }
    }
    return FR_OK;
}

int fr_rc_counts(fr_ctx* ctx, uint64_t* reads_f, uint64_t* reads_rc) {
    if (int src = settle_finalize(ctx)) return src;
    if (!ctx->d_rcf) return fail(ctx, FR_ERR_INVALID, "fr_rc_counts: no rc classify yet");
    const int names = std::max(ctx->n_names, 1);
    std::vector<u64> f(names), r(names);
    CK(hipMemcpy(f.data(), ctx->d_rcf, names * 8, hipMemcpyDeviceToHost));
    CK(hipMemcpy(r.data(), ctx->d_rcr, names * 8, hipMemcpyDeviceToHost));
    for (int i = 0; i < ctx->n_names; ++i) {
        reads_f[i] = f[i];
        reads_rc[i] = r[i];
    }
    return FR_OK;
}

int fr_classify_cp(fr_ctx* ctx, int n, const uint32_t* q1, const int32_t* q1len, const uint32_t* q2,
                   const int32_t* q2len, int cp_stride, int num_subs, int rc_mode, int16_t* m1, int16_t* m2,
                   uint8_t* cls, int16_t* row, int16_t* rc_m2, uint8_t* rc_cls, int16_t* rc_row,
                   int32_t* err_which) {
    if (int src = settle_finalize(ctx)) return src;
    if (n <= 0) return FR_OK;
    if (ctx->S > 0 && (!ctx->d_cp1 || cp_stride != ctx->cp_stride))
        return fail(ctx, FR_ERR_INVALID, "fr_classify_cp: sheet code points missing or stride mismatch");
    u32 *dq1, *dq2;
    int32_t *dl1, *dl2;
    int16_t *o_m1, *o_m2, *o_row, *o_rm2, *o_rrow;
    u8 *o_cls, *o_rcls;
    int32_t* o_err;
    const u64 qn = (u64)n * cp_stride;
    CK(dalloc(&dq1, qn));
    CK(dalloc(&dq2, qn));
    CK(dalloc(&dl1, n));
    CK(dalloc(&dl2, n));
    CK(dalloc(&o_m1, n));
    CK(dalloc(&o_m2, n));
    CK(dalloc(&o_row, n));
    CK(dalloc(&o_rm2, n));
    CK(dalloc(&o_rrow, n));
    CK(dalloc(&o_cls, n));
    CK(dalloc(&o_rcls, n));
    CK(dalloc(&o_err, n));
    CK(hipMemcpy(dq1, q1, qn * 4, hipMemcpyHostToDevice));
    CK(hipMemcpy(dq2, q2, qn * 4, hipMemcpyHostToDevice));
    CK(hipMemcpy(dl1, q1len, n * 4, hipMemcpyHostToDevice));
    CK(hipMemcpy(dl2, q2len, n * 4, hipMemcpyHostToDevice));
    ClassOut o{o_m1, o_m2, o_cls, o_row, o_rm2, o_rcls, o_rrow, nullptr, nullptr, nullptr, o_err};
    CK(launch_classify_cp(n, dq1, dl1, dq2, dl2, cp_stride, ctx->S > 0 ? ctx->S : 0, ctx->d_cp1, ctx->d_cpl1,
                          ctx->d_cp2, ctx->d_cpl2, ctx->d_cp2rc, ctx->d_name, num_subs, rc_mode ? 1 : 0, o,
                          ctx->stream));
    CK(hipStreamSynchronize(ctx->stream));
    CK(hipMemcpy(m1, o_m1, n * 2, hipMemcpyDeviceToHost));
    CK(hipMemcpy(m2, o_m2, n * 2, hipMemcpyDeviceToHost));
    CK(hipMemcpy(cls, o_cls, n, hipMemcpyDeviceToHost));
    CK(hipMemcpy(row, o_row, n * 2, hipMemcpyDeviceToHost));
    if (err_which) CK(hipMemcpy(err_which, o_err, n * 4, hipMemcpyDeviceToHost));
    if (rc_mode) {
        CK(hipMemcpy(rc_m2, o_rm2, n * 2, hipMemcpyDeviceToHost));
        CK(hipMemcpy(rc_cls, o_rcls, n, hipMemcpyDeviceToHost));
        CK(hipMemcpy(rc_row, o_rrow, n * 2, hipMemcpyDeviceToHost));
    }
    void* tmp[] = {dq1, dq2, dl1, dl2, o_m1, o_m2, o_row, o_rm2, o_rrow, o_cls, o_rcls, o_err};
    for (void* p : tmp) CK(hipFree(p));
    return FR_OK;
}

int fr_export_unique_device(fr_ctx* ctx, void* dev_keys, void* dev_counts, void* dev_first, uint64_t cap) {
    if (int src = settle_finalize(ctx)) return src;
    if (ctx->U > cap) return fail(ctx, FR_ERR_CAPACITY, "export buffer too small");
    if (ctx->U) {
        CK(hipMemcpyAsync(dev_keys, ctx->d_keys_s, ctx->U * 8, hipMemcpyDeviceToDevice, ctx->stream));
        CK(hipMemcpyAsync(dev_counts, ctx->d_counts_s, ctx->U * 8, hipMemcpyDeviceToDevice, ctx->stream));
        CK(hipMemcpyAsync(dev_first, ctx->d_first_s, ctx->U * 8, hipMemcpyDeviceToDevice, ctx->stream));
    }
    CK(hipStreamSynchronize(ctx->stream));
    return FR_OK;
}

int fr_export_partitioned_device(fr_ctx* ctx, int world, void* dev_rows, void* dev_counts, uint64_t cap) {
    if (int src = settle_finalize(ctx)) return src;
    if (world < 1 || world > 1024) return fail(ctx, FR_ERR_INVALID, "fr_export_partitioned_device: world out of range");
    if (ctx->U > cap) return fail(ctx, FR_ERR_CAPACITY, "export buffer too small");
    CK(launch_partition_rows(ctx->d_keys_s, ctx->d_counts_s, ctx->d_first_s, ctx->U, (u32)world, (u64*)dev_counts,
                             (u64*)dev_counts + world, (u64*)dev_rows, ctx->stream));
    CK(hipStreamSynchronize(ctx->stream));
    return FR_OK;
}

int fr_merge_rows_device(fr_ctx* ctx, const void* dev_rows, uint64_t n) {
    if (int src = settle_finalize(ctx)) return src;
    if (ctx->file_open) return fail(ctx, FR_ERR_INVALID, "fr_merge_rows_device: a file is open");
    int rc = flush_presence(ctx);
    if (rc) return rc;
    ctx->merged = true;
    rc = read_state(ctx);
    if (rc) return rc;
    if ((ctx->h_st->n_keys + n) * 2 > ctx->nslots) {
        rc = grow_table(ctx, true);
        if (rc) return rc;
    }
    ctx->st_fresh = false;
    CK(launch_merge_rows(ctx->tab, ctx->st, (const u64*)dev_rows, n, ctx->stream));
    return grow_table(ctx, false);
}

int fr_merge_unique_device(fr_ctx* ctx, const void* dev_keys, const void* dev_counts, const void* dev_first,
                           uint64_t n) {
    if (int src = settle_finalize(ctx)) return src;
    if (ctx->file_open) return fail(ctx, FR_ERR_INVALID, "fr_merge_unique_device: a file is open");
    int rc = flush_presence(ctx);
    if (rc) return rc;
    ctx->merged = true;
    rc = read_state(ctx);
    if (rc) return rc;
    if ((ctx->h_st->n_keys + n) * 2 > ctx->nslots) {
        rc = grow_table(ctx, true);
        if (rc) return rc;
    }
    ctx->st_fresh = false;
    CK(launch_merge(ctx->tab, ctx->st, (const u64*)dev_keys, (const u64*)dev_counts, (const u64*)dev_first, n,
                    ctx->stream));
    return grow_table(ctx, false);
}

void* fr_device_alloc(fr_ctx* ctx, uint64_t bytes) {
    void* p = nullptr;
    if (hipSetDevice(ctx->device) != hipSuccess || hipMalloc(&p, std::max<u64>(bytes, 1)) != hipSuccess) {
        ctx->err = "fr_device_alloc failed";
        return nullptr;
    }
    return p;
}

int fr_device_free(fr_ctx* ctx, void* ptr) {
    CK(hipFree(ptr));
    return FR_OK;
}

int fr_copy_to_host(fr_ctx* ctx, void* dst, const void* dev_src, uint64_t bytes) {
    CK(hipStreamSynchronize(ctx->stream));
    CK(hipMemcpy(dst, dev_src, bytes, hipMemcpyDeviceToHost));
    return FR_OK;
}

int fr_copy_to_device(fr_ctx* ctx, void* dev_dst, const void* src, uint64_t bytes) {
    CK(hipStreamSynchronize(ctx->stream));
    CK(hipMemcpy(dev_dst, src, bytes, hipMemcpyHostToDevice));
    return FR_OK;
}

int fr_synth_device(fr_ctx* ctx, uint8_t* dev_out, uint64_t r0, uint64_t n, int R, uint64_t seed,
                    const char* idx1_ascii, const char* idx2_ascii, int S, int L1, int L2) {
    if (S <= 0 || L1 <= 0 || L2 <= 0 || L1 + L2 > 32 || R < 0 || R > 256)
        return fail(ctx, FR_ERR_INVALID, "fr_synth_device: bad shape");
    u8 *d1, *d2;
    CK(dalloc(&d1, (u64)S * L1));
// ... 12 lines not shown
```

frender_amd/csrc/fr_internal.h:

```cpp
#pragma once
#include <hip/hip_runtime.h>
#include <stdint.h>

#include <vector>

namespace fr {

typedef uint8_t u8;
typedef uint16_t u16;
typedef uint32_t u32;
typedef uint64_t u64;
typedef int64_t i64;

constexpr int WG = 256;
constexpr int SEG = 64;
constexpr int TILE = 64 * SEG;
constexpr int TSTEP = TILE - SEG;
#ifndef FR_LOG_NS
#define FR_LOG_NS 10
#endif
constexpr int LOG_NS = FR_LOG_NS;
constexpr int NS = 1 << LOG_NS;
#ifndef FR_LPROBE
#define FR_LPROBE 2
// ... 13 lines not shown
constexpr int EXO_BUF = 32;
#ifndef FR_PHASE_LINES
#define FR_PHASE_LINES 16
#endif
constexpr int PHASE_LINES = FR_PHASE_LINES;
constexpr u32 RARE_RING = 8192;

struct alignas(32) GSlot {
    u64 key;
    u64 count;
    u64 first;
    u32 last_tag;
    u32 uidx;
};

constexpr int PRES_TAG_BITS = 20;
struct alignas(16) Presence {
    u64 key;
    u64 tc;
};

struct alignas(32) Overflow {
    u64 key, count, first;
    u32 tag, pad;
};

struct alignas(16) LogEntry {
    u64 key;
    u64 oc;
};
constexpr int LOG_CNT_BITS = 24;
constexpr u64 LOG_CNT_MAX = (1ull << LOG_CNT_BITS) - 1ull;
__host__ __device__ inline u64 log_pack(u64 off, u64 cnt) { return (off << LOG_CNT_BITS) | cnt; }
__host__ __device__ inline u64 log_off(u64 oc) { return oc >> LOG_CNT_BITS; }
__host__ __device__ inline u32 log_cnt(u64 oc) { return (u32)(oc & LOG_CNT_MAX); }
#ifndef FR_LOG_REGION_BITS
#define FR_LOG_REGION_BITS 6
#endif
#ifndef FR_LOG_SUB_BITS
#define FR_LOG_SUB_BITS 3
#endif
constexpr int LOG_REGION_BITS = FR_LOG_REGION_BITS;
constexpr int LOG_NR = 1 << LOG_REGION_BITS;
constexpr int LOG_SUB_BITS = FR_LOG_SUB_BITS;
constexpr int LOG_SUBS = 1 << LOG_SUB_BITS;
constexpr int LOG_NSUB = LOG_NR * LOG_SUBS;
#ifndef FR_LOG_DIRECT
#define FR_LOG_DIRECT 1
#endif
constexpr bool LOG_DIRECT = FR_LOG_DIRECT != 0;
constexpr int LOG_NB = LOG_DIRECT ? LOG_NSUB : LOG_NR;
constexpr int AGG_LNS = 4096;

struct DevState {
    u64 lines[2];
    u64 err_nospace;
    u32 nonascii;
    u32 utf8_bad;
    u32 ticket;
    u32 chunks_done;
    u32 exits;
    u32 spin_fail;
    u32 spec_fail;
    u64 n_keys;
    u64 n_overflow;
    u64 n_presence;
    u64 n_exotic;
    u64 exo_pool_used;
    u32 cap_flags;
    u32 spin_max;
    u64 spin_total;
    u64 log_n;
    u64 log_commits;
    u64 stamp[8];
    u32 heavy[2];
    u32 commits_done;
    u32 heavy_launches;
    u64 chunks_total;
    u32 log_rcur[LOG_NR];
    u32 log_scur[LOG_NSUB];
    u32 log_red_done;
    u32 log_fold_max;
    u32 log_fold_over;
};

struct Table {
    GSlot* slots;
    u64 mask;
    Overflow* ovf;
    u64 ovf_cap;
    Presence* pres;
    u64 pres_cap;
    u64* exo_ord;
    u64* exo_off;
    u32* exo_len;
    u64 exo_cap;
    u8* exo_pool;
    u64 exo_pool_cap;
};

struct ScanArgs {
    const u8* buf;
    u64 len;
    u64 avail;
    u64 file_offset;
    u32 file_tag;
    u32 par;
    u32 epoch;
    u32 num_tiles;
    int own_start;
    int own_end;
    int pre_valid;
    u32 flush_at;
    i64 max_records;
    u32 chunk_tiles;
    u32 num_chunks;
    u32 ramp_g;
    u32 mid_chunks;
    u32 ramp_up_s;
    u32 ramp_down_s;
    u32 ramp_down_g;
    u32 ramp_down_g_h;
    u32 chunk_tiles_h;
    u32 mid_chunks_h;
    u32 num_chunks_h;
    u32 cold_cap;
    u64* cold;
    uint4* rare;
    u64* chunk_info;
    LogEntry* log;
    u64 log_cap;
    u32 log_rcap;
    u32 log_min;
    u32 log_hot;
    u32 exo_only;
    u32 spec_commit;
    DevState* st;
    u64* tiles;
    const Table* tab;
    Table tabv;
};

__host__ __device__ inline u64 ramp_tiles_before(u64 C, u64 G, u64 s, u64 j) {
    return s * j + ((C - s) * j * (j + 1)) / (2ull * G);
}

struct SheetArgs {
    int S;
    int n_names;
    int L1u;
    int L2u;
    const u64* i1;
    const u64* i2;
    const u64* i2rc;
    const int32_t* name;
};

struct ClassOut {
    int16_t* m1;
    int16_t* m2;
    u8* cls;
    int16_t* row;
    int16_t* rc_m2;
    u8* rc_cls;
    int16_t* rc_row;
    u64* rc_f;
    u64* rc_r;
    u64* err_first;
    int32_t* err_which;
};

enum { CLS_UNDET = 0, CLS_HOP = 1, CLS_DEMUX = 2, CLS_AMBIG = 3 };

constexpr u64 NBR_KEY = 1ull << 63;
struct NSlot {
    u64 key;
    u32 vmin_c;
    u32 vmax1;
};
struct PSlot {
    u64 key;
    u32 cnt;
    u32 first_c;
};
struct NbrMap {
    NSlot* m[3];
    u32 mmask[3];
    PSlot* p[2];
    u32 pmask[2];
    int on;
};

__host__ __device__ inline u64 mix64(u64 x) {
    x ^= x >> 30;
    x *= 0xBF58476D1CE4E5B9ull;
    x ^= x >> 27;
    x *= 0x94D049BB133111EBull;
    x ^= x >> 31;
    return x;
}

__host__ __device__ inline u32 log_region(u64 key) { return (u32)(mix64(key) >> (64 - LOG_REGION_BITS)); }
__host__ __device__ inline u32 log_bucket(u64 key) {
    return (u32)(mix64(key) >> (64 - LOG_REGION_BITS - (LOG_DIRECT ? LOG_SUB_BITS : 0)));
}
__host__ __device__ inline u32 log_subregion(u64 key) {
    return (u32)(mix64(key) >> (64 - LOG_REGION_BITS - LOG_SUB_BITS)) & (LOG_SUBS - 1);
}

hipError_t launch_table_init(GSlot* slots, u64 n, hipStream_t s);
hipError_t launch_chunk_scan(const ScanArgs& a, int grid, hipStream_t s);
int chunk_occupancy();
hipError_t launch_reinsert_overflow(Table t, DevState* st, const Overflow* src, u64 n, hipStream_t s);
hipError_t launch_rehash(Table dst, DevState* st, const GSlot* src, u64 nsrc, hipStream_t s);
hipError_t launch_compact(const GSlot* slots, u64 nslots, u64* keys, u64* counts, u64* first, u32* pos,
                          u64* counter, hipStream_t s);
hipError_t launch_set_uidx(GSlot* slots, u64 mask, const u64* keys, u64 n, const u32* rank_of_pos,
                           hipStream_t s);
hipError_t launch_order(const u64* first_in, const u32* pos_in, u64 n, u64* first_out, u32* perm_out,
                        void* temp, size_t* temp_bytes, int begin_bit, int end_bit, hipStream_t s);
hipError_t launch_gather(const u32* perm, u64 n, const u64* keys, const u64* counts, u64* keys_o,
                         u64* counts_o, u32* rank, hipStream_t s);
hipError_t launch_presence_one_file(const u64* counts, u64 n, u32 tag, u32* uidx, u32* file_idx, u64* snap,
                                    hipStream_t s);
hipError_t launch_presence_map(const GSlot* slots, u64 mask, const Presence* pres, u64 n, u32* uidx,
                               u32* file_idx, u64* snap, hipStream_t s);
struct BinMap {
    u64 span;
    u32 first_tag;
    u32 shift;
    u64 nbins;
    u64 cap;
};
struct alignas(32) FinRow {
    u64 first, key, count;
    u32 slot, pad;
};
hipError_t launch_fin_hist(const GSlot* slots, u64 nslots, const BinMap& m, u32* cnt, u32* arr, hipStream_t s);
hipError_t launch_fin_scan(const u32* cnt, u32* base, u64 n, void* temp, size_t* temp_bytes, hipStream_t s);
hipError_t launch_fin_scatter(const GSlot* slots, u64 nslots, const BinMap& m, const u32* base, const u32* arr,
                              FinRow* rows, hipStream_t s);
hipError_t launch_fin_rank(GSlot* slots, u64 nk, const BinMap& m, const u32* base, const FinRow* rows, u64* keys_o,
                           u64* counts_o, u64* first_o, bool set_uidx, hipStream_t s);
hipError_t launch_classify(const u64* keys, const u64* counts, u64 n, SheetArgs sh, int nsubs, int rc,
                           ClassOut o, const NbrMap& nm, hipStream_t s);
u64 nbr_codes_per_row(int L, int nsubs);
hipError_t launch_nbr_build(const SheetArgs& sh, const int32_t* canon, int nsubs, int rc, const NbrMap& nm,
                            hipStream_t s);
hipError_t launch_classify_cp(int n, const u32* q1, const int32_t* q1len, const u32* q2, const int32_t* q2len,
                              int stride, int S, const u32* s1, const int32_t* s1len, const u32* s2,
                              const int32_t* s2len, const u32* s2rc, const int32_t* name, int nsubs, int rc,
                              ClassOut o, hipStream_t s);
hipError_t launch_presence_scan(const GSlot* slots, u64 n, u32 tag, Presence* pres, u64 cap, DevState* st,
                                hipStream_t s);
hipError_t launch_merge(Table t, DevState* st, const u64* keys, const u64* counts, const u64* first, u64 n,
                        hipStream_t s);
hipError_t launch_partition_rows(const u64* keys, const u64* counts_in, const u64* first, u64 n, u32 world,
                                 u64* counts, u64* cursor, u64* rows, hipStream_t s);
hipError_t launch_merge_rows(Table t, DevState* st, const u64* rows, u64 n, hipStream_t s);
hipError_t launch_log_aggregate(Table t, DevState* st, const LogEntry* log, u32 rcap, LogEntry* sub, u32 scap,
                                u32 file_tag, u64 file_offset, hipStream_t s);
size_t log_aggregate_temp_bytes();
hipError_t launch_synth(u8* out, u64 r0, u64 n, int R, u64 seed, const u8* idx1, const u8* idx2, int S, int L1,
                        int L2, hipStream_t s);

struct BgzfMember {
    size_t in_off, in_len, dst;
    u32 isize, crc;
};
constexpr u64 BGZF_MAX_IN = 1ull << 30;
bool bgzf_member_table(const u8* data, size_t n, std::vector<BgzfMember>& out);
void crc_shift_table(u64 n, u32* T);

}
```

frender_amd/csrc/fr_kernels.hip:

```cpp
#include <algorithm>
#include <cstdlib>
#include <cstring>

#include <rocprim/rocprim.hpp>

#include "fr_internal.h"

namespace fr {

#if defined(FR_STAMPS) && FR_STAMPS == 1
#define FR_STAMP_DECL u64 st_[8] = {0, 0, 0, 0, 0, 0, 0, 0}; u64 tq_ = __builtin_amdgcn_s_memtime();
#define FR_STAMP(i) do { const u64 n_ = __builtin_amdgcn_s_memtime(); st_[i] += n_ - tq_; tq_ = n_; } while (0)
#define FR_STAMP_FLUSH(k0) do { st_[6] = __builtin_amdgcn_s_memtime() - (k0); \
    if ((threadIdx.x & 63) == 0) for (int i_ = 0; i_ < 8; ++i_) atomicAdd((unsigned long long*)&a.st->stamp[i_], \
        (unsigned long long)st_[i_]); } while (0)
#else
#define FR_STAMP_DECL
#define FR_STAMP(i) do { } while (0)
#define FR_STAMP_FLUSH(k0) do { } while (0)
#endif

#if defined(FR_STAMPS) && FR_STAMPS == 2
#define FR_CSTAMP(i) do { const u64 n_ = __builtin_amdgcn_s_memtime(); cst_[i] += n_ - cq_; cq_ = n_; } while (0)
#else
// ... 1364 lines not shown
        const u64 info = agent_load(&a.chunk_info[c]);
        const u32 f = (u32)(info >> 32);
        if ((f & 1u) && ((f >> 1) & 3u) != (u32)(run & 3ull)) bad = true;
        run += (u32)info;
    }
    if (bad) atomicOr(&a.st->spec_fail, 1u);
    if (tid == 0) a.st->lines[a.par ^ 1u] = base_lines + total;
    __syncthreads();
}

__device__ __forceinline__ void chunk_bounds(const ScanArgs& a, const Geom& g, u32 c, u32& tb, u32& te) {
    if (a.ramp_g == 0) {
        tb = min(c * g.chunk_tiles, a.num_tiles);
        te = min(tb + g.chunk_tiles, a.num_tiles);
        return;
    }
    const u32 su = min(a.ramp_up_s, g.chunk_tiles), sd = min(a.ramp_down_s, g.chunk_tiles);
    const u64 G = a.ramp_g, Gd = g.down_g;
    const u64 rg = ramp_prefix(g, G, G, su), mid_end = (u64)a.num_tiles - ramp_prefix(g, Gd, Gd, sd);
    if (c < G) {
        tb = (u32)ramp_prefix(g, G, c, su);
        te = (u32)ramp_prefix(g, G, c + 1, su);
    } else if (c < G + g.mid_chunks) {
        const u64 b = rg + (u64)(c - G) * g.chunk_tiles;
        tb = (u32)b;
        te = (u32)min(b + g.chunk_tiles, mid_end);
    } else {
        const u64 j = c - G - g.mid_chunks;
        tb = (u32)((u64)a.num_tiles - ramp_prefix(g, Gd, Gd - j, sd));
        te = (u32)((u64)a.num_tiles - ramp_prefix(g, Gd, Gd - j - 1, sd));
    }
}

#if defined(FR_STAMPS) && FR_STAMPS == 3
constexpr u32 TRACE_CHUNKS = 1u << 14;
constexpr u32 TRACE_WGS = 4096;
__device__ u64 g_chunk_trace[2 * TRACE_CHUNKS * 4];
__device__ u64 g_wg_trace[2 * TRACE_WGS * 2];
__device__ __forceinline__ u32 xcc_id() {
    u32 x;
    asm volatile("s_getreg_b32 %0, hwreg(HW_REG_XCC_ID)" : "=s"(x));
    return x & 0xFu;
}
extern "C" int fr_trace_read(u64* chunks, u64* wgs) {
    if (hipMemcpyFromSymbol(chunks, HIP_SYMBOL(g_chunk_trace), sizeof(g_chunk_trace)) != hipSuccess) return 1;
    if (hipMemcpyFromSymbol(wgs, HIP_SYMBOL(g_wg_trace), sizeof(g_wg_trace)) != hipSuccess) return 1;
    return 0;
}
extern "C" int fr_trace_clear() {
    static u64 zero[2 * TRACE_CHUNKS * 4];
    if (hipMemcpyToSymbol(HIP_SYMBOL(g_chunk_trace), zero, sizeof(g_chunk_trace)) != hipSuccess) return 1;
    if (hipMemcpyToSymbol(HIP_SYMBOL(g_wg_trace), zero, sizeof(g_wg_trace)) != hipSuccess) return 1;
    return 0;
}
#endif

#ifndef FR_OCC
#define FR_OCC 4
#endif
template <bool LIM>
__global__ __launch_bounds__(WG, FR_OCC) void chunk_kernel(ScanArgs args) {
    (void)args;
    const ScanArgs& a = *(const ScanArgs*)__builtin_amdgcn_kernarg_segment_ptr();
    __shared__ ScanShared sh;
    const int tid = threadIdx.x;
    const int lane = tid & 63;
    const u32 wid = wave_id();
    for (int i = tid; i < NS; i += WG) sh.ls[i] = LSlot{0, 0, 0xFFFFFFFFu};
    if (lane == 0) {
        sh.bsp[wid][SEGS] = sh.bsp[wid][SEGS + 1] = 0;
        sh.bcol[wid][SEGS] = sh.bcol[wid][SEGS + 1] = 0;
        sh.beol[wid][SEGS] = sh.beol[wid][SEGS + 1] = 0;
        sh.rq_tail[wid] = 0;
    }
    if (tid == 0) {
        sh.nkeys = 0;
        sh.created = 0;
        sh.flags = 0;
        sh.spec = 0;
        sh.spec_bad = 0;
        sh.ncold = 0;
        sh.nexo = 0;
        sh.err_off = 0xFFFFFFFFu;
    }
#if defined(FR_STAMPS) && FR_STAMPS == 3
    if (tid == 0 && blockIdx.x < TRACE_WGS) g_wg_trace[(a.par * TRACE_WGS + blockIdx.x) * 2] = __builtin_amdgcn_s_memrealtime();
    u64 tl_t0 = 0;
#endif
    const u64 base_lines = a.st->lines[a.par];
    const bool hv = a.num_chunks_h != 0 &&
                    __builtin_amdgcn_readfirstlane(__hip_atomic_load(&a.st->heavy[a.par], __ATOMIC_RELAXED,
                                                                     __HIP_MEMORY_SCOPE_AGENT)) != 0;
    const Geom g = hv ? Geom{a.chunk_tiles_h, a.mid_chunks_h, a.num_chunks_h, a.ramp_down_g_h}
                      : Geom{a.chunk_tiles, a.mid_chunks, a.num_chunks, a.ramp_down_g};
    constexpr bool limited = LIM;
#if defined(FR_STAMPS) && (FR_STAMPS == 1 || FR_STAMPS == 4)
    const u64 k0_ = __builtin_amdgcn_s_memtime();
#endif
    FR_STAMP_DECL
    for (;;) {
        if (tid == 0) {
            const u32 cn = atomicAdd(&a.st->ticket, 1u);
            sh.chunk = cn;
            if (cn < g.num_chunks) {
                u32 tb0, te0;
                chunk_bounds(a, g, cn, tb0, te0);
                sh.cbase = (u64)tb0 * TSTEP;
            }
            sh.spec = 1u;
        }
        __syncthreads();
        const u32 c = sh.chunk;
        FR_TRACE("w%d ticket %u of %u\n", (int)wid, c, g.num_chunks);
        if (c >= g.num_chunks) break;
        u32 tb, te;
        chunk_bounds(a, g, c, tb, te);
#if defined(FR_STAMPS) && FR_STAMPS == 3
        if (tid == 0) tl_t0 = __builtin_amdgcn_s_memrealtime();
#endif
        const u32 per = (te - tb + NW - 1) / NW;
        const u32 wb = min(tb + wid * per, te), we = min(wb + per, te);
        u64 L0 = 0;
        bool parse = false;
        FR_STAMP(3);
        if (wb < we) {
            if (c == 0 && wid == 0) {
                L0 = base_lines;
                parse = true;
            } else if (!limited && !a.exo_only) {
                const int P = guess_phase(sh, a, wb, lane, wid);
                parse = P >= 0;
                L0 = (u64)max(P, 0);
            }
        }
        FR_STAMP(0);
#if defined(FR_STAMPS) && FR_STAMPS == 1
        st_[7] += 1;
#endif
        bool run = wb < we, exact = true, force = false;
        u64 base = base_lines;
        for (int pass = 0;; ++pass) {
            FR_TRACE("w%d pass %d run %d [%u,%u) parse %d\n", (int)wid, pass, (int)run, wb, we, (int)parse);
            const u64 n = run ? walk_wave<LIM>(sh, a, tb, wb, we, L0, parse, lane, wid) : 0ull;
            FR_TRACE("w%d walked %llu\n", (int)wid, (unsigned long long)n);
            FR_STAMP(pass == 0 ? 1 : 4);
            if (pass == 0) {
                if (lane == 0) {
                    sh.wcount[wid] = n;
                    sh.wphase[wid] = run && parse ? (int)(L0 & 3ull) : -1;
                }
                __syncthreads();
                FR_STAMP(2);
                u64 total = 0;
#pragma unroll
                for (int w = 0; w < NW; ++w) total += sh.wcount[w];
                const int p0 = sh.wphase[0];
                const bool fast = a.spec_commit && c != 0 && p0 >= 0 && !uniform_flag(sh.spec_bad);
                if (tid == 0) {
                    agent_store(&a.tiles[c], ((u64)(2u * a.epoch + (c == 0 ? 1u : 0u)) << 32) | (u32)total);
                    const u32 f = fast ? (1u | ((u32)p0 << 1)) : 0u;
                    agent_store(&a.chunk_info[c], ((u64)f << 32) | (u32)total);
                    asm volatile("s_waitcnt vmcnt(0)" ::: "memory");
                    const u32 prev = __hip_atomic_fetch_add(&a.st->chunks_done, 1u, __ATOMIC_RELAXED,
                                                            __HIP_MEMORY_SCOPE_AGENT);
                    sh.last = prev == g.num_chunks - 1u;
                }
// ... 12 lines not shown
                __syncthreads();
                if (exact || !uniform_flag(sh.spec_bad)) break;
                u64 total = 0;
#pragma unroll
                for (int w = 0; w < NW; ++w) total += sh.wcount[w];
                if (wid == 0) {
                    const u64 ex = lookback(a, c, (u32)total, lane);
                    if (lane == 0) sh.tile_excl = ex;
                }
                __syncthreads();
                base = base_lines + sh.tile_excl;
                exact = true;
                force = true;
            }
            u64 D = base;
            bool bad = force || uniform_flag(sh.spec_bad);
#pragma unroll
            for (int w = 0; w < NW; ++w) {
                const int pw = sh.wphase[w];
                if (w == (int)wid) L0 = D;
                if (pw >= 0 && (u64)pw != (D & 3ull)) bad = true;
                D += sh.wcount[w];
            }
            run = wb < we && (bad || sh.wphase[wid] < 0);
            parse = true;
            if (bad) discard_buffers(sh, tid);
            if (tid == 0) sh.spec = exact ? 0u : 1u;
            __syncthreads();
        }
        FR_TRACE("w%d commit\n", (int)wid);
        FR_STAMP(3);
#if defined(FR_STAMPS) && FR_STAMPS == 3
        const u64 tl_t1 = __builtin_amdgcn_s_memrealtime();
#endif
        commit_buffers(sh, a, tid, g, hv);
#if defined(FR_STAMPS) && FR_STAMPS == 3
        if (tid == 0 && c < TRACE_CHUNKS) {
            u64* e = &g_chunk_trace[(a.par * TRACE_CHUNKS + c) * 4];
            e[0] = (u64)blockIdx.x | ((u64)xcc_id() << 16) | ((u64)(te - tb) << 32);
            e[1] = tl_t0;
            e[2] = tl_t1;
            e[3] = __builtin_amdgcn_s_memrealtime();
        }
#endif
        FR_TRACE("w%d committed last %u\n", (int)wid, sh.last);
        if (sh.last) {
            __atomic_thread_fence(__ATOMIC_ACQUIRE);
            verify_launch(sh, a, g.num_chunks, base_lines, tid);
        }
        FR_STAMP(5);
    }
#if defined(FR_STAMPS) && FR_STAMPS == 1
    FR_STAMP_FLUSH(k0_);
#endif
#if defined(FR_STAMPS) && FR_STAMPS == 4
    if ((threadIdx.x & 63) == 0)
        atomicAdd((unsigned long long*)&a.st->stamp[5], (unsigned long long)(__builtin_amdgcn_s_memtime() - k0_));
#endif
#if defined(FR_STAMPS) && FR_STAMPS == 3
    if (tid == 0 && blockIdx.x < TRACE_WGS) g_wg_trace[(a.par * TRACE_WGS + blockIdx.x) * 2 + 1] = __builtin_amdgcn_s_memrealtime();
#endif
    __syncthreads();
    if (tid == 0) {
        if (sh.created) atomicAdd((unsigned long long*)&a.st->n_keys, (unsigned long long)sh.created);
        if (sh.flags & 1u) atomicOr(&a.st->nonascii, 1u);
        if (sh.flags & 2u) atomicOr(&a.st->utf8_bad, 1u);
        if (atomicAdd(&a.st->exits, 1u) == gridDim.x - 1u) {
            a.st->ticket = 0;
            a.st->chunks_done = 0;
            a.st->exits = 0;
        }
    }
}

int chunk_occupancy() { return FR_OCC; }

hipError_t launch_chunk_scan(const ScanArgs& a, int grid, hipStream_t s) {
    if (a.max_records > 0) hipLaunchKernelGGL(chunk_kernel<true>, dim3(grid), dim3(WG), 0, s, a);
    else hipLaunchKernelGGL(chunk_kernel<false>, dim3(grid), dim3(WG), 0, s, a);
    return hipGetLastError();
}


__global__ void table_init_kernel(GSlot* slots, u64 n) {
    for (u64 i = blockIdx.x * (u64)blockDim.x + threadIdx.x; i < n; i += (u64)gridDim.x * blockDim.x) {
        GSlot g;
        g.key = 0;
        g.count = 0;
        g.first = ~0ull;
        g.last_tag = 0;
        g.uidx = 0;
        slots[i] = g;
    }
}

hipError_t launch_table_init(GSlot* slots, u64 n, hipStream_t s) {
    const int grid = (int)std::min<u64>((n + 255) / 256, 8192);
    hipLaunchKernelGGL(table_init_kernel, dim3(grid > 0 ? grid : 1), dim3(256), 0, s, slots, n);
    return hipGetLastError();
}

__global__ void reinsert_kernel(Table t, DevState* st, const Overflow* src, u64 n) {
    u32 made = 0;
    for (u64 i = blockIdx.x * (u64)blockDim.x + threadIdx.x; i < n; i += (u64)gridDim.x * blockDim.x) {
        const Overflow o = src[i];
        made += global_insert(t, st, o.key, o.count, o.first, o.tag) ? 1u : 0u;
    }
    add_created(st, made);
}

hipError_t launch_reinsert_overflow(Table t, DevState* st, const Overflow* src, u64 n, hipStream_t s) {
    if (!n) return hipSuccess;
    const int grid = (int)std::min<u64>((n + 255) / 256, 4096);
    hipLaunchKernelGGL(reinsert_kernel, dim3(grid), dim3(256), 0, s, t, st, src, n);
    return hipGetLastError();
}

__global__ void rehash_kernel(Table t, const GSlot* src, u64 nsrc) {
    for (u64 i = blockIdx.x * (u64)blockDim.x + threadIdx.x; i < nsrc; i += (u64)gridDim.x * blockDim.x) {
        const GSlot g = src[i];
        if (!g.key) continue;
        u64 h = table_home(g.key, t.mask);
        for (;;) {
            const u64 old = atomicCAS((unsigned long long*)&t.slots[h].key, 0ull, (unsigned long long)g.key);
            if (old == 0) {
                t.slots[h].count = g.count;
                t.slots[h].first = g.first;
                t.slots[h].last_tag = g.last_tag;
                break;
            }
            h = (h + 1) & t.mask;
        }
    }
}

hipError_t launch_rehash(Table dst, DevState* st, const GSlot* src, u64 nsrc, hipStream_t s) {
    (void)st;
    const int grid = (int)std::min<u64>((nsrc + 255) / 256, 8192);
    hipLaunchKernelGGL(rehash_kernel, dim3(grid), dim3(256), 0, s, dst, src, nsrc);
    return hipGetLastError();
}

__device__ __forceinline__ bool last_block(u32* ctr) {
    __shared__ u32 last;
    __syncthreads();
    if (threadIdx.x == 0) {
        __threadfence();
        const u32 prev = atomicAdd(ctr, 1u);
        last = prev == gridDim.x - 1u;
        if (last) {
            *ctr = 0;
            __threadfence();
        }
    }
    __syncthreads();
    return last != 0;
}

constexpr int AGG_PROBE = 256;
constexpr int CLAIM_WORDS = 1024;
struct alignas(16) AggSlot {
    u64 key;
    u32 mino, cnt;
};

struct ClaimZone {
    u32* bits;
    u64 base, lo, hi;
};

template <int B, bool EXCL = false>
__device__ __forceinline__ u32 insert_rows(const Table& T, DevState* st, const u64 (&key)[B], const u32 (&cnt)[B],
                                           const u64 (&ord)[B], const u32 (&tag)[B], const bool (&valid)[B],
                                           const ClaimZone& cz = ClaimZone{nullptr, 0, 0, 0}) {
    u32 h[B];
    bool pend[B];
#pragma unroll
    for (int b = 0; b < B; ++b) {
        h[b] = (u32)table_home(key[b], T.mask);
        pend[b] = valid[b];
    }
// ... 98 lines not shown
}

constexpr int SPLIT_PER = 8;
constexpr int SPLIT_TILE = SPLIT_PER * 256;
#ifndef FR_SPLIT_WGS
#define FR_SPLIT_WGS 64
#endif
constexpr int SPLIT_WGS = FR_SPLIT_WGS;
__global__ __launch_bounds__(256) void log_split_kernel(Table t, DevState* st, const LogEntry* log, u32 rcap,
                                                        LogEntry* sub, u32 scap, u32 file_tag, u64 ord0) {
    if (st->log_n == 0) return;
    const u32 r = blockIdx.x / SPLIT_WGS, j = blockIdx.x % SPLIT_WGS;
    const u32 n = min(st->log_rcur[r], rcap);
    const LogEntry* part = log + (u64)r * rcap;
    __shared__ u32 wcnt[4][LOG_SUBS];
    __shared__ u32 sbase[4][LOG_SUBS];
    const int tid = threadIdx.x, lane = tid & 63, w = tid >> 6;
    const u64 lt = (1ull << lane) - 1ull;
    u32 made = 0;
    for (u32 t0 = j * SPLIT_TILE; t0 < n; t0 += SPLIT_WGS * SPLIT_TILE) {
        LogEntry e[SPLIT_PER];
        u32 sb[SPLIT_PER], rank[SPLIT_PER];
        u32 run[LOG_SUBS];
#pragma unroll
        for (int s = 0; s < LOG_SUBS; ++s) run[s] = 0;
#pragma unroll
        for (int q = 0; q < SPLIT_PER; ++q) {
            const u32 i = t0 + w * 64 * SPLIT_PER + q * 64 + lane;
            e[q] = i < n ? part[i] : LogEntry{0, 0};
        }
#pragma unroll
        for (int q = 0; q < SPLIT_PER; ++q) {
            sb[q] = e[q].key ? log_subregion(e[q].key) : (u32)LOG_SUBS;
            rank[q] = 0;
#pragma unroll
            for (int s = 0; s < LOG_SUBS; ++s) {
                const u64 m = __ballot(sb[q] == (u32)s);
                if (sb[q] == (u32)s) rank[q] = run[s] + (u32)__popcll(m & lt);
                run[s] += (u32)__popcll(m);
            }
        }
        if (lane == 0) {
#pragma unroll
            for (int s = 0; s < LOG_SUBS; ++s) wcnt[w][s] = run[s];
        }
        __syncthreads();
        if (tid < LOG_SUBS) {
            u32 tot = 0;
#pragma unroll
            for (int v = 0; v < 4; ++v) tot += wcnt[v][tid];
            u32 b = tot ? atomicAdd(&st->log_scur[r * LOG_SUBS + tid], tot) : 0u;
#pragma unroll
            for (int v = 0; v < 4; ++v) {
                sbase[v][tid] = b;
                b += wcnt[v][tid];
            }
        }
        __syncthreads();
#pragma unroll
        for (int q = 0; q < SPLIT_PER; ++q) {
            if (sb[q] >= (u32)LOG_SUBS) continue;
            const u32 pos = sbase[w][sb[q]] + rank[q];
            if (pos < scap) {
                sub[(u64)(r * LOG_SUBS + sb[q]) * scap + pos] = e[q];
            } else {
                const u64 key1[1] = {e[q].key};
                const u32 cnt1[1] = {log_cnt(e[q].oc)};
                const u64 ord1[1] = {(ord0 + log_off(e[q].oc)) & ~3ull};
                const u32 tag1[1] = {file_tag};
                const bool v1[1] = {true};
                made += insert_rows<1>(t, st, key1, cnt1, ord1, tag1, v1);
            }
        }
        __syncthreads();
    }
    add_created(st, made);
}

#ifndef FR_RED_WG
#define FR_RED_WG 512
#endif
constexpr int RED_WG = FR_RED_WG;
constexpr int RED_FB = RED_WG >= 512 ? 4 : 8;
__global__ __launch_bounds__(RED_WG) void log_reduce_kernel(Table t, DevState* st, const LogEntry* sub, u32 scap,
                                                         u32 file_tag, u64 ord0) {
    if (st->log_n == 0) return;
    __shared__ AggSlot ls[AGG_LNS];
    __shared__ u32 zone_bits[CLAIM_WORDS];
    __shared__ u16 occ[AGG_LNS];
    __shared__ u32 occ_n;
    u32 made = 0;
    for (int i = threadIdx.x; i < AGG_LNS; i += RED_WG) ls[i] = AggSlot{0, 0xFFFFFFFFu, 0};
    const u64 nslots = t.mask + 1ull, rn = nslots >= (u64)LOG_NSUB ? nslots / LOG_NSUB : 0ull;
    ClaimZone cz{nullptr, 0, 0, 0};
    if (rn > 2ull * GPROBE && rn <= 32ull * CLAIM_WORDS && !(ABLATE & 2048u)) {
        cz = ClaimZone{zone_bits, (u64)blockIdx.x * rn, (u64)blockIdx.x * rn + GPROBE, (u64)(blockIdx.x + 1) * rn};
        for (u32 i = threadIdx.x; i < (u32)(rn / 32); i += RED_WG) zone_bits[i] = 0;
    }
    __syncthreads();
    const u32 n = min(st->log_scur[blockIdx.x], scap);
    const LogEntry* part = sub + (u64)blockIdx.x * scap;
    const u64 base4 = (ord0 & ((1ull << ORD_SHIFT) - 1ull)) >> 2, tagpart = ord0 & ~((1ull << ORD_SHIFT) - 1ull);
    u64 sink = 0;
    constexpr int LB = 8;
    const u32 nn = (ABLATE & 512u) ? 0u : n;
    LogEntry nx[LB];
    if (nn) {
#pragma unroll
        for (int q = 0; q < LB; ++q) nx[q] = part[min(threadIdx.x + q * RED_WG, nn - 1u)];
    }
    for (u32 i0 = threadIdx.x; i0 < nn; i0 += LB * RED_WG) {
        LogEntry ev[LB];
#pragma unroll
        for (int q = 0; q < LB; ++q) {
            ev[q] = nx[q];
            nx[q] = part[min(i0 + (LB + q) * RED_WG, nn - 1u)];
        }
#pragma unroll
        for (int q = 0; q < LB; ++q) {
            const LogEntry e = ev[q];
            if (i0 + q * RED_WG >= nn || !e.key) continue;
            if (ABLATE & 1024u) {
                sink ^= e.key;
                continue;
            }
            const u32 eoff = (u32)((((ord0 & ((1ull << ORD_SHIFT) - 1ull)) + log_off(e.oc)) >> 2) - base4);
            const u32 ecnt = log_cnt(e.oc);
            u32 h = (u32)e.key * 0x9E3779B1u ^ (u32)(e.key >> 32) * 0x85EBCA6Bu;
            const u32 hstep = ((h >> 7) & (AGG_LNS - 1)) | 1u;
            h = (h ^ (h >> 15)) & (AGG_LNS - 1);
            bool done = false;
            for (int pr = 0; pr < AGG_PROBE && !done; ++pr) {
                const AggSlot sl = ls[h];
                u64 k = sl.key;
                u32 mino = sl.mino;
                if (k == 0) {
                    const u64 old = atomicCAS((unsigned long long*)&ls[h].key, 0ull, (unsigned long long)e.key);
                    k = old == 0 ? e.key : old;
                    mino = old == 0 ? 0xFFFFFFFFu : ls[h].mino;
                }
                if (k == e.key) {
                    atomicAdd(&ls[h].cnt, ecnt);
                    if (eoff < mino) atomicMin(&ls[h].mino, eoff);
                    done = true;
                    break;
                }
                h = (h + hstep) & (AGG_LNS - 1);
            }
            if (!done) {
                const u64 key1[1] = {e.key};
                const u32 cnt1[1] = {ecnt};
                const u64 ord1[1] = {tagpart | ((base4 + eoff) << 2)};
                const u32 tag1[1] = {file_tag};
                const bool v1[1] = {true};
                made += insert_rows<1>(t, st, key1, cnt1, ord1, tag1, v1, cz);
                atomicAdd(&st->log_fold_over, 1u);
            }
        }
    }
    if (sink == 1) atomicAdd((unsigned long long*)&st->stamp[7], 1ull);
    __syncthreads();
    if (threadIdx.x == 0) occ_n = 0;
    __syncthreads();
    for (int i = threadIdx.x; i < AGG_LNS; i += RED_WG)
        if (ls[i].key) occ[atomicAdd(&occ_n, 1u)] = (u16)i;
    __syncthreads();
    if (threadIdx.x == 0) atomicMax(&st->log_fold_max, occ_n);
    constexpr int FB = RED_FB;
    const u32 nocc = (ABLATE & 256u) ? 0u : occ_n;
    for (u32 i0 = threadIdx.x; i0 < nocc; i0 += FB * RED_WG) {
        u64 key[FB], ord[FB];
        u32 cnt[FB], tag[FB];
        bool v[FB];
#pragma unroll
        for (int b = 0; b < FB; ++b) {
            const u32 j = i0 + b * RED_WG;
            v[b] = j < nocc;
            const AggSlot e = v[b] ? ls[occ[j]] : AggSlot{0, 0, 0};
            key[b] = e.key;
            cnt[b] = e.cnt;
            ord[b] = tagpart | ((base4 + e.mino) << 2);
            tag[b] = file_tag;
        }
        made += insert_rows<FB, true>(t, st, key, cnt, ord, tag, v, cz);
    }
    add_created(st, made);
    if (last_block(&st->log_red_done)) {
        for (int i = threadIdx.x; i < LOG_NR; i += RED_WG)
            __hip_atomic_store(&st->log_rcur[i], 0u, __ATOMIC_RELAXED, __HIP_MEMORY_SCOPE_AGENT);
        for (int i = threadIdx.x; i < LOG_NSUB; i += RED_WG)
            __hip_atomic_store(&st->log_scur[i], 0u, __ATOMIC_RELAXED, __HIP_MEMORY_SCOPE_AGENT);
        if (threadIdx.x == 0) __hip_atomic_store(&st->log_n, 0ull, __ATOMIC_RELAXED, __HIP_MEMORY_SCOPE_AGENT);
    }
}

size_t log_aggregate_temp_bytes() { return 0; }

hipError_t launch_log_aggregate(Table t, DevState* st, const LogEntry* log, u32 rcap, LogEntry* sub, u32 scap,
                                u32 file_tag, u64 file_offset, hipStream_t s) {
    const u64 ord0 = ((u64)file_tag << ORD_SHIFT) | file_offset;
    if (!LOG_DIRECT)
        hipLaunchKernelGGL(log_split_kernel, dim3(LOG_NR * SPLIT_WGS), dim3(256), 0, s, t, st, log, rcap, sub, scap,
                           file_tag, ord0);
    hipLaunchKernelGGL(log_reduce_kernel, dim3(LOG_NSUB), dim3(RED_WG), 0, s, t, st, sub, scap, file_tag, ord0);
    return hipGetLastError();
}

constexpr int CWG = 256;

template <class Pred>
__device__ __forceinline__ u64 block_reserve(u64 lo, u64 hi, Pred pred, u64* counter, u32* red) {
    const int tid = threadIdx.x;
    u32 mine = 0;
    for (u64 i = lo + tid; i < hi; i += CWG) mine += pred(i) ? 1u : 0u;
    for (int o = 32; o > 0; o >>= 1) mine += __shfl_xor(mine, o, 64);
    if ((tid & 63) == 0) red[tid >> 6] = mine;
    __syncthreads();
    if (tid == 0) {
        const u32 tot = red[0] + red[1] + red[2] + red[3];
        *(u64*)&red[4] = tot ? atomicAdd((unsigned long long*)counter, (unsigned long long)tot) : 0ull;
    }
    __syncthreads();
    return *(const u64*)&red[4];
}

template <class Pred, class Emit>
__device__ __forceinline__ void block_emit(u64 lo, u64 hi, u64 base, Pred pred, Emit emit, u32* wc) {
    const int tid = threadIdx.x, lane = tid & 63, wid = tid >> 6;
    for (u64 b = lo; b < hi; b += CWG) {
        const u64 i = b + tid;
        const bool hit = i < hi && pred(i);
        const u64 m = __ballot(hit);
        if (lane == 0) wc[wid] = (u32)__popcll(m);
        __syncthreads();
        u32 before = 0, tot = 0;
        for (int w = 0; w < CWG / 64; ++w) {
            before += w < wid ? wc[w] : 0u;
            tot += wc[w];
        }
        if (hit) emit(base + before + (u64)__popcll(m & ((1ull << lane) - 1ull)), i);
        base += tot;
        __syncthreads();
    }
}

__device__ __forceinline__ void block_range(u64 n, u64& lo, u64& hi) {
    const u64 per = (n + gridDim.x - 1) / gridDim.x;
    lo = min(n, (u64)blockIdx.x * per);
    hi = min(n, lo + per);
}

__global__ __launch_bounds__(CWG) void compact_kernel(const GSlot* slots, u64 nslots, u64* keys, u64* counts,
                                                      u64* first, u32* pos, u64* counter) {
    __shared__ u32 red[8];
    u64 lo, hi;
    block_range(nslots, lo, hi);
    auto pred = [&](u64 i) { return slots[i].key != 0; };
    const u64 base = block_reserve(lo, hi, pred, counter, red);
    block_emit(lo, hi, base, pred, [&](u64 p, u64 i) {
        const GSlot g = slots[i];
        keys[p] = g.key;
        counts[p] = g.count;
        first[p] = g.first;
        pos[p] = (u32)p;
    }, red);
}

hipError_t launch_compact(const GSlot* slots, u64 nslots, u64* keys, u64* counts, u64* first, u32* pos,
                          u64* counter, hipStream_t s) {
    const int grid = (int)std::max<u64>(1, std::min<u64>((nslots + 4095) / 4096, 2048));
    hipLaunchKernelGGL(compact_kernel, dim3(grid), dim3(CWG), 0, s, slots, nslots, keys, counts, first, pos,
                       counter);
    return hipGetLastError();
}

hipError_t launch_order(const u64* first_in, const u32* pos_in, u64 n, u64* first_out, u32* perm_out, void* temp,
                        size_t* temp_bytes, int begin_bit, int end_bit, hipStream_t s) {
    return rocprim::radix_sort_pairs(temp, *temp_bytes, first_in, first_out, pos_in, perm_out, (size_t)n,
                                     (unsigned)begin_bit, (unsigned)end_bit, s);
}

__global__ void gather_kernel(const u32* perm, u64 n, const u64* keys, const u64* counts, u64* keys_o,
                              u64* counts_o, u32* rank) {
    for (u64 j = blockIdx.x * (u64)blockDim.x + threadIdx.x; j < n; j += (u64)gridDim.x * blockDim.x) {
        const u32 p = perm[j];
        keys_o[j] = keys[p];
        counts_o[j] = counts[p];
// ... 6 lines not shown
    if (!n) return hipSuccess;
    const int grid = (int)std::min<u64>((n + 255) / 256, 8192);
    hipLaunchKernelGGL(gather_kernel, dim3(grid), dim3(256), 0, s, perm, n, keys, counts, keys_o, counts_o, rank);
    return hipGetLastError();
}

__device__ __forceinline__ const GSlot* table_find(const GSlot* slots, u64 mask, u64 key) {
    u64 h = table_home(key, mask);
    for (u64 probe = 0; probe <= mask; ++probe) {
        const GSlot* s = &slots[h];
        if (s->key == key) return s;
        if (s->key == 0) return nullptr;
        h = (h + 1) & mask;
    }
    return nullptr;
}

__global__ void set_uidx_kernel(GSlot* slots, u64 mask, const u64* keys, u64 n) {
    for (u64 j = blockIdx.x * (u64)blockDim.x + threadIdx.x; j < n; j += (u64)gridDim.x * blockDim.x) {
        GSlot* s = const_cast<GSlot*>(table_find(slots, mask, keys[j]));
        if (s) s->uidx = (u32)j;
    }
}

hipError_t launch_set_uidx(GSlot* slots, u64 mask, const u64* keys, u64 n, const u32* rank_of_pos, hipStream_t s) {
    (void)rank_of_pos;
    if (!n) return hipSuccess;
    const int grid = (int)std::min<u64>((n + 255) / 256, 8192);
    hipLaunchKernelGGL(set_uidx_kernel, dim3(grid), dim3(256), 0, s, slots, mask, keys, n);
    return hipGetLastError();
}

__global__ void presence_map_kernel(const GSlot* slots, u64 mask, const Presence* pres, u64 n, u32* uidx,
                                    u32* file_idx, u64* snap) {
    for (u64 i = blockIdx.x * (u64)blockDim.x + threadIdx.x; i < n; i += (u64)gridDim.x * blockDim.x) {
        const Presence p = pres[i];
        const GSlot* s = table_find(slots, mask, p.key);
        uidx[i] = s ? s->uidx : 0xFFFFFFFFu;
        file_idx[i] = (u32)(p.tc & ((1u << PRES_TAG_BITS) - 1u)) - 1u;
        snap[i] = p.tc >> PRES_TAG_BITS;
    }
}

__global__ void presence_one_file_kernel(const u64* counts, u64 n, u32 tag, u32* uidx, u32* file_idx, u64* snap) {
    for (u64 i = blockIdx.x * (u64)blockDim.x + threadIdx.x; i < n; i += (u64)gridDim.x * blockDim.x) {
        uidx[i] = (u32)i;
        file_idx[i] = tag - 1u;
        snap[i] = counts[i] & ((1ull << (64 - PRES_TAG_BITS)) - 1ull);
    }
}

hipError_t launch_presence_one_file(const u64* counts, u64 n, u32 tag, u32* uidx, u32* file_idx, u64* snap,
                                    hipStream_t s) {
    if (!n) return hipSuccess;
    const int grid = (int)std::min<u64>((n + 255) / 256, 8192);
    hipLaunchKernelGGL(presence_one_file_kernel, dim3(grid), dim3(256), 0, s, counts, n, tag, uidx, file_idx, snap);
    return hipGetLastError();
}

hipError_t launch_presence_map(const GSlot* slots, u64 mask, const Presence* pres, u64 n, u32* uidx,
                               u32* file_idx, u64* snap, hipStream_t s) {
    if (!n) return hipSuccess;
    const int grid = (int)std::min<u64>((n + 255) / 256, 8192);
    hipLaunchKernelGGL(presence_map_kernel, dim3(grid), dim3(256), 0, s, slots, mask, pres, n, uidx, file_idx, snap);
    return hipGetLastError();
}

__device__ __forceinline__ u64 ord_bin(const BinMap& m, u64 ord) {
    const u64 tag = ord >> ORD_SHIFT, off = ord & ((1ull << ORD_SHIFT) - 1ull);
    return min(((tag - m.first_tag) * m.span + off) >> m.shift, m.nbins - 1ull);
}

__global__ __launch_bounds__(256) void fin_hist_kernel(const GSlot* slots, u64 n, BinMap m, u32* cnt, u32* arr) {
    const u64 i = blockIdx.x * (u64)blockDim.x + threadIdx.x;
    if (i >= n) return;
    const uint4 w0 = *(const uint4*)&slots[i];
    const uint4 w1 = *((const uint4*)&slots[i] + 1);
    u32 v = 0xFFFFFFFFu;
    if ((w0.x | w0.y) != 0u) v = atomicAdd(&cnt[ord_bin(m, ((u64)w1.y << 32) | w1.x)], 1u);
    arr[i] = v;
}

__global__ __launch_bounds__(256) void fin_scatter_kernel(const GSlot* slots, u64 n, BinMap m, const u32* base,
                                                          const u32* arr, FinRow* rows) {
    const u64 i = blockIdx.x * (u64)blockDim.x + threadIdx.x;
    if (i >= n) return;
    const u32 k = arr[i];
    if (k == 0xFFFFFFFFu) return;
    const uint4 w0 = *(const uint4*)&slots[i];
    const uint4 w1 = *((const uint4*)&slots[i] + 1);
    const u64 first = ((u64)w1.y << 32) | w1.x;
    const u32 q = base[ord_bin(m, first)] + k;
    if (q < m.cap) {
        typedef u32 u32x4 __attribute__((ext_vector_type(4)));
        u32x4* d = (u32x4*)&rows[q];
        d[0] = u32x4{w1.x, w1.y, w0.x, w0.y};
        d[1] = u32x4{w0.z, w0.w, (u32)i, 0u};
    }
}

__global__ __launch_bounds__(256) void fin_rank_kernel(GSlot* slots, u64 nk, BinMap m, const u32* base,
                                                       const FinRow* rows, u64* keys_o, u64* counts_o, u64* first_o,
                                                       int set_uidx) {
    const u64 q = blockIdx.x * (u64)blockDim.x + threadIdx.x;
    if (q >= nk) return;
    const FinRow row = rows[q];
    const u64 b = ord_bin(m, row.first);
    const u32 lo = base[b], hi = (u32)min((u64)base[b + 1], m.cap);
    u32 r = 0;
    for (u32 j = lo; j < hi; ++j) {
        const u64 fj = rows[j].first;
        r += (fj < row.first || (fj == row.first && rows[j].slot < row.slot)) ? 1u : 0u;
    }
    const u32 out = lo + r;
    if (out >= nk) return;
    keys_o[out] = row.key;
    counts_o[out] = row.count;
    first_o[out] = row.first;
    if (set_uidx) slots[row.slot].uidx = out;
}

static unsigned lane_grid(u64 n) { return (unsigned)std::max<u64>(1, (n + 255) / 256); }

hipError_t launch_fin_hist(const GSlot* slots, u64 nslots, const BinMap& m, u32* cnt, u32* arr, hipStream_t s) {
    hipLaunchKernelGGL(fin_hist_kernel, dim3(lane_grid(nslots)), dim3(256), 0, s, slots, nslots, m, cnt, arr);
    return hipGetLastError();
}

hipError_t launch_fin_scan(const u32* cnt, u32* base, u64 n, void* temp, size_t* temp_bytes, hipStream_t s) {
    return rocprim::exclusive_scan(temp, *temp_bytes, cnt, base, 0u, (size_t)n, rocprim::plus<u32>(), s);
}

hipError_t launch_fin_scatter(const GSlot* slots, u64 nslots, const BinMap& m, const u32* base, const u32* arr,
                              FinRow* rows, hipStream_t s) {
    hipLaunchKernelGGL(fin_scatter_kernel, dim3(lane_grid(nslots)), dim3(256), 0, s, slots, nslots, m, base, arr, rows);
    return hipGetLastError();
}

hipError_t launch_fin_rank(GSlot* slots, u64 nk, const BinMap& m, const u32* base, const FinRow* rows, u64* keys_o,
                           u64* counts_o, u64* first_o, bool set_uidx, hipStream_t s) {
    if (!nk) return hipSuccess;
    hipLaunchKernelGGL(fin_rank_kernel, dim3(lane_grid(nk)), dim3(256), 0, s, slots, nk, m, base, rows, keys_o,
                       counts_o, first_o, set_uidx ? 1 : 0);
    return hipGetLastError();
}

__global__ void merge_kernel(Table t, DevState* st, const u64* keys, const u64* counts, const u64* first, u64 n) {
    u32 made = 0;
    for (u64 i = blockIdx.x * (u64)blockDim.x + threadIdx.x; i < n; i += (u64)gridDim.x * blockDim.x)
        made += global_insert(t, st, keys[i], counts[i], first[i], 0u) ? 1u : 0u;
    add_created(st, made);
}

constexpr int PART_MAX = 1024;
__device__ __forceinline__ u32 owner_rank(u64 key, u32 world) {
    return (u32)(((key * 0x9E3779B97F4A7C15ull) >> 40) & 0xFFFFFFull) % world;
}
__global__ __launch_bounds__(256) void part_count_kernel(const u64* keys, u64 n, u32 world, u64* counts) {
    __shared__ u32 h[PART_MAX];
    for (u32 i = threadIdx.x; i < world; i += 256) h[i] = 0;
    __syncthreads();
    for (u64 i = blockIdx.x * 256ull + threadIdx.x; i < n; i += (u64)gridDim.x * 256ull) atomicAdd(&h[owner_rank(keys[i], world)], 1u);
    __syncthreads();
    for (u32 i = threadIdx.x; i < world; i += 256)
        if (h[i]) atomicAdd((unsigned long long*)&counts[i], (unsigned long long)h[i]);
}
__global__ __launch_bounds__(256) void part_scatter_kernel(const u64* keys, const u64* counts_in, const u64* first,
                                                          u64 n, u32 world, const u64* counts, u64* cursor, u64* rows) {
    __shared__ u32 h[PART_MAX];
    __shared__ u64 base[PART_MAX];
    for (u32 i = threadIdx.x; i < world; i += 256) h[i] = 0;
    __syncthreads();
    const u64 stride = (u64)gridDim.x * 256ull;
    for (u64 i = blockIdx.x * 256ull + threadIdx.x; i < n; i += stride) atomicAdd(&h[owner_rank(keys[i], world)], 1u);
    __syncthreads();
    if (threadIdx.x == 0) {
        u64 pre = 0;
        for (u32 r = 0; r < world; ++r) {
            base[r] = h[r] ? pre + atomicAdd((unsigned long long*)&cursor[r], (unsigned long long)h[r]) : 0ull;
            pre += counts[r];
            h[r] = 0;
        }
    }
    __syncthreads();
    for (u64 i = blockIdx.x * 256ull + threadIdx.x; i < n; i += stride) {
        const u64 k = keys[i];
        const u32 r = owner_rank(k, world);
        const u64 at = base[r] + atomicAdd(&h[r], 1u);
        rows[3 * at] = k;
        rows[3 * at + 1] = counts_in[i];
        rows[3 * at + 2] = first[i];
    }
}
__global__ void merge_rows_kernel(Table t, DevState* st, const u64* rows, u64 n) {
    u32 made = 0;
    for (u64 i = blockIdx.x * (u64)blockDim.x + threadIdx.x; i < n; i += (u64)gridDim.x * blockDim.x)
        made += global_insert(t, st, rows[3 * i], rows[3 * i + 1], rows[3 * i + 2], 0u) ? 1u : 0u;
    add_created(st, made);
}
hipError_t launch_partition_rows(const u64* keys, const u64* counts_in, const u64* first, u64 n, u32 world,
                                 u64* counts, u64* cursor, u64* rows, hipStream_t s) {
    if (world < 1 || world > (u32)PART_MAX) return hipErrorInvalidValue;
    hipError_t e = hipMemsetAsync(counts, 0, 2ull * world * sizeof(u64), s);
    if (e != hipSuccess || !n) return e;
    const int grid = (int)std::min<u64>((n + 255) / 256, 2048);
    hipLaunchKernelGGL(part_count_kernel, dim3(grid), dim3(256), 0, s, keys, n, world, counts);
    hipLaunchKernelGGL(part_scatter_kernel, dim3(grid), dim3(256), 0, s, keys, counts_in, first, n, world, counts,
                       cursor, rows);
    return hipGetLastError();
}
hipError_t launch_merge_rows(Table t, DevState* st, const u64* rows, u64 n, hipStream_t s) {
    if (!n) return hipSuccess;
    const int grid = (int)std::min<u64>((n + 255) / 256, 8192);
    hipLaunchKernelGGL(merge_rows_kernel, dim3(grid), dim3(256), 0, s, t, st, rows, n);
    return hipGetLastError();
}

constexpr int PS_K = 16;
// ... 244 lines not shown
    const u64* vals[3] = {sh.i1, sh.i2, sh.i2rc};
    const int len[3] = {sh.L1u, sh.L2u, sh.L2u};
    for (int l = 0; l < (rc ? 3 : 2); ++l) {
        const u64 T = nbr_codes_per_row(len[l], nsubs);
        const u64 n = (u64)sh.S * T;
        hipLaunchKernelGGL(nbr_insert_kernel, dim3((u32)((n + 255) / 256)), dim3(256), 0, s, vals[l], canon + l * sh.S,
                           sh.S, len[l], nsubs, T, nm.m[l], nm.mmask[l]);
    }
    hipLaunchKernelGGL(nbr_pair_kernel, dim3((u32)((sh.S + 255) / 256)), dim3(256), 0, s, canon, sh.S, rc, nm.p[0],
                       nm.pmask[0], nm.p[1], nm.pmask[1]);
    return hipGetLastError();
}

__device__ __forceinline__ int nbr_resolve(const NSlot* __restrict__ t, u32 mask, u64 key, u32 h, NSlot e) {
    for (;;) {
        if (e.key == key) return ~e.vmin_c == e.vmax1 - 1u ? (int)~e.vmin_c : -2;
        if (e.key == 0) return -1;
        h = (h + 1) & mask;
        e = t[h];
    }
}

__device__ __forceinline__ void nbr_find3(const NbrMap& nm, u64 q1, u64 q2, bool rc, int& a1, int& a2, int& a3) {
    const u64 k1 = q1 | NBR_KEY, k2 = q2 | NBR_KEY;
    const u32 h1 = (u32)mix64(k1) & nm.mmask[0], h2 = (u32)mix64(k2) & nm.mmask[1], h3 = (u32)mix64(k2) & nm.mmask[2];
    const NSlot e1 = nm.m[0][h1], e2 = nm.m[1][h2];
    const NSlot e3 = rc ? nm.m[2][h3] : NSlot{0, 0, 0};
    a1 = nbr_resolve(nm.m[0], nm.mmask[0], k1, h1, e1);
    a2 = nbr_resolve(nm.m[1], nm.mmask[1], k2, h2, e2);
    a3 = rc ? nbr_resolve(nm.m[2], nm.mmask[2], k2, h3, e3) : -1;
}

__device__ __forceinline__ void pair_resolve(const PSlot* __restrict__ t, u32 mask, u64 key, u32 h, PSlot e, int& both,
                                             int& r) {
    for (;;) {
        if (e.key == key) {
            both = (int)e.cnt;
            r = (int)~e.first_c;
            return;
        }
        if (e.key == 0) return;
        h = (h + 1) & mask;
        e = t[h];
    }
}

__device__ __forceinline__ void class_pair_nbr(const NbrMap& nm, int a1, int a2, int a3, int& m1, int& m2, int& cls,
                                               int& row, int& rm2, int& rcls, int& rrow) {
    int both = 0, r = -1, rboth = 0, rr = -1;
    const bool f0 = a1 >= 0 && a2 >= 0, f1 = a1 >= 0 && a3 >= 0;
    const u64 pk0 = ((u64)(u32)a1 << 32) | (u32)a2 | NBR_KEY, pk1 = ((u64)(u32)a1 << 32) | (u32)a3 | NBR_KEY;
    const u32 ph0 = (u32)mix64(pk0) & nm.pmask[0], ph1 = (u32)mix64(pk1) & nm.pmask[1];
    const PSlot p0 = f0 ? nm.p[0][ph0] : PSlot{0, 0, 0};
    const PSlot p1 = f1 ? nm.p[1][ph1] : PSlot{0, 0, 0};
    if (f0) pair_resolve(nm.p[0], nm.pmask[0], pk0, ph0, p0, both, r);
    if (f1) pair_resolve(nm.p[1], nm.pmask[1], pk1, ph1, p1, rboth, rr);
    m1 = a1;
    m2 = a2;
    rm2 = a3;
    if (m1 >= 0 && m2 >= 0) {
        cls = both == 0 ? CLS_HOP : both == 1 ? CLS_DEMUX : CLS_AMBIG;
        row = both == 1 ? r : -1;
    } else {
        cls = CLS_UNDET;
        row = -1;
    }
    if (m1 >= 0 && rm2 >= 0) {
        rcls = rboth == 0 ? CLS_HOP : rboth == 1 ? CLS_DEMUX : CLS_AMBIG;
        rrow = rboth == 1 ? rr : -1;
    } else {
        rcls = CLS_UNDET;
        rm2 = -1;
        rrow = -1;
    }
    if (cls == CLS_UNDET) {
        if (rcls == CLS_UNDET) m1 = -1;
        m2 = -1;
    }
}

template <typename W>
__global__ __launch_bounds__(CLS_WG) void classify_kernel(const u64* keys, const u64* counts, u64 n, SheetArgs sh,
                                                          int nsubs, int rc, ClassOut o, NbrMap nm,
                                                          int sheet_in_lds, int names_in_lds) {
    extern __shared__ __attribute__((aligned(16))) u8 cls_lds[];
    unsigned long long* lf = (unsigned long long*)cls_lds;
    unsigned long long* lr = lf + (names_in_lds ? sh.n_names : 0);
    W* s1 = (W*)(lr + (names_in_lds ? sh.n_names : 0));
    W* s2 = s1 + sh.S;
    W* s2rc = s2 + sh.S;
    if (sheet_in_lds) {
        for (int i = threadIdx.x; i < sh.S; i += CLS_WG) {
            s1[i] = (W)sh.i1[i];
            s2[i] = (W)sh.i2[i];
            s2rc[i] = rc ? (W)sh.i2rc[i] : (W)0;
        }
    }
    if (rc && names_in_lds)
        for (int i = threadIdx.x; i < sh.n_names; i += CLS_WG) lf[i] = lr[i] = 0;
    __syncthreads();
    const W* S1 = sheet_in_lds ? s1 : (const W*)sh.i1;
    const W* S2 = sheet_in_lds ? s2 : (const W*)sh.i2;
    const W* S2rc = sheet_in_lds ? s2rc : (const W*)sh.i2rc;

    for (u64 u = blockIdx.x * (u64)CLS_WG + threadIdx.x; u < n; u += (u64)gridDim.x * CLS_WG) {
        const u64 key = keys[u];
        int n1 = 0, n2 = 0;
        bool plus = false;
        u64 q1 = 0, q2 = 0;
        if (key & WIDE_BIT) {
            const u64 V = key & ((1ull << 57) - 1ull);
            const int pp = (int)((key >> 57) & 31u);
            int nl = 0;
            u64 off = 0, pw = 1;
            while (nl < WIDE_MAXN && off + pw <= V) {
                off += pw;
                pw *= 5;
                ++nl;
            }
            u64 D = V - off;
            plus = pp != WIDE_NOPLUS;
            n1 = plus ? pp : nl;
            n2 = plus ? nl - pp : 0;
            for (int i = 0; i < nl; ++i) {
                const u64 sy = D % 5u + 1u;
                D /= 5u;
                if (i < n1) q1 |= sy << (3 * i);
                else q2 |= sy << (3 * (i - n1));
            }
        } else {
            constexpr u64 G0 = 0x1249249249249249ull & ((1ull << 63) - 1ull);
            const u64 nz = (key | (key >> 1) | (key >> 2)) & G0;
            const u64 empty = ~nz & G0;
            const int len = empty ? (int)(__builtin_ctzll(empty) / 3) : MAXSYM;
            const u64 x = key ^ (G0 * 6ull);
            u64 pm = ~(x | (x >> 1) | (x >> 2)) & G0;
            pm &= len < MAXSYM ? (1ull << (3 * len)) - 1ull : ~0ull;
            const int p1 = pm ? (int)(__builtin_ctzll(pm) / 3) : -1;
            pm &= pm - 1ull;
            const int p2 = pm ? (int)(__builtin_ctzll(pm) / 3) : MAXSYM;
            plus = p1 >= 0;
            if (plus) {
                n1 = p1;
                const int e2 = p2 < len ? p2 : len;
                n2 = e2 - p1 - 1;
                q1 = n1 ? (key & ((1ull << (3 * n1)) - 1ull)) : 0ull;
                q2 = n2 ? ((key >> (3 * (p1 + 1))) & ((1ull << (3 * n2)) - 1ull)) : 0ull;
            }
        }
        int err = 0;
        int m1 = -1, m2 = -1, cls = CLS_UNDET, row = -1;
        int rm2 = -1, rcls = CLS_UNDET, rrow = -1;
        if (!plus) {
            err = 3;
        } else {
            if (sh.S > 0 && (sh.L1u == -2 || sh.L1u != n1)) err = 1;
            else if (sh.S > 0 && (sh.L2u == -2 || sh.L2u != n2)) err = 2;
            else {
                int a1 = -2, a2 = -2, a3 = -1;
                if (nm.on) nbr_find3(nm, q1, q2, rc != 0, a1, a2, a3);
                if (a1 != -2 && a2 != -2 && a3 != -2)
                    class_pair_nbr(nm, a1, a2, a3, m1, m2, cls, row, rm2, rcls, rrow);
                else if (FR_CLS_SCALAR && rc)
                    class_pair_s<W, true>((W)q1, (W)q2, sh.i1, sh.i2, sh.i2rc, sh.S, nsubs, m1, m2, cls, row, rm2,
                                          rcls, rrow);
                else if (FR_CLS_SCALAR)
                    class_pair_s<W, false>((W)q1, (W)q2, sh.i1, sh.i2, sh.i2rc, sh.S, nsubs, m1, m2, cls, row, rm2,
                                           rcls, rrow);
                else
                    class_pair<W>((W)q1, (W)q2, S1, S2, S2rc, sh.S, nsubs, rc != 0, m1, m2, cls, row, rm2, rcls, rrow);
                if (rc && cls == CLS_DEMUX && rcls == CLS_DEMUX && sh.name[row] != sh.name[rrow]) {
                    cls = CLS_AMBIG;
                    row = -1;
                    rcls = CLS_AMBIG;
                    rrow = -1;
                }
            }
        }
        if (err) {
            atomicMax((unsigned long long*)o.err_first, (unsigned long long)~u);
            if (o.err_which) o.err_which[u] = err;
        } else if (o.err_which) {
            o.err_which[u] = 0;
        }
        o.m1[u] = (int16_t)m1;
        o.m2[u] = (int16_t)m2;
        o.cls[u] = (u8)cls;
        o.row[u] = (int16_t)row;
        if (rc) {
            o.rc_m2[u] = (int16_t)rm2;
            o.rc_cls[u] = (u8)rcls;
            o.rc_row[u] = (int16_t)rrow;
            const u64 cnt = (cls == CLS_DEMUX || rcls == CLS_DEMUX) ? counts[u] : 0ull;
            if (cls == CLS_DEMUX) {
                const int nm = sh.name[row];
                if (names_in_lds) atomicAdd(&lf[nm], (unsigned long long)cnt);
                else atomicAdd((unsigned long long*)&o.rc_f[nm], (unsigned long long)cnt);
            }
            if (rcls == CLS_DEMUX) {
                const int nm = sh.name[rrow];
                if (names_in_lds) atomicAdd(&lr[nm], (unsigned long long)cnt);
                else atomicAdd((unsigned long long*)&o.rc_r[nm], (unsigned long long)cnt);
            }
        }
    }
    if (rc && names_in_lds) {
        __syncthreads();
        for (int i = threadIdx.x; i < sh.n_names; i += CLS_WG) {
            if (lf[i]) atomicAdd((unsigned long long*)&o.rc_f[i], lf[i]);
            if (lr[i]) atomicAdd((unsigned long long*)&o.rc_r[i], lr[i]);
        }
    }
}

hipError_t launch_classify(const u64* keys, const u64* counts, u64 n, SheetArgs sh, int nsubs, int rc, ClassOut o,
                           const NbrMap& nm, hipStream_t s) {
    if (!n) return hipSuccess;
    const bool narrow = sh.S > 0 && sh.L1u >= 0 && sh.L1u <= 10 && sh.L2u >= 0 && sh.L2u <= 10;
    const size_t wb = narrow ? 4 : 8;
    const size_t names_bytes = rc ? 2ull * 8 * sh.n_names : 0;
    const size_t sheet_bytes = 3 * wb * (size_t)std::max(sh.S, 0);
    const int names_in_lds = (rc && names_bytes <= CLS_LDS_BYTES / 2) ? 1 : 0;
    const size_t nb = names_in_lds ? names_bytes : 0;
    const int sheet_in_lds = (!FR_CLS_SCALAR && nb + sheet_bytes <= CLS_LDS_BYTES) ? 1 : 0;
    const size_t lds = nb + (sheet_in_lds ? sheet_bytes : 0) + 16;
    const u64 grid = std::min<u64>((n + CLS_WG - 1) / CLS_WG, 2048);
    const bool wide = !(narrow && (sheet_in_lds || FR_CLS_SCALAR));
    if (!wide)
        hipLaunchKernelGGL(classify_kernel<u32>, dim3((u32)grid), dim3(CLS_WG), lds, s, keys, counts, n, sh, nsubs, rc,
                           o, nm, sheet_in_lds, names_in_lds);
    else
        hipLaunchKernelGGL(classify_kernel<u64>, dim3((u32)grid), dim3(CLS_WG), lds, s, keys, counts, n, sh, nsubs, rc,
                           o, nm, sheet_in_lds, names_in_lds);
    return hipGetLastError();
}

__device__ void class_of_cp(const u32* q1, int n1, const u32* q2, int n2, const u32* s1, const u32* s2, int stride,
                            int S, int nsubs, int& m1, int& m2, int& cls, int& row) {
    m1 = -1;
    m2 = -1;
    int both = 0, r = -1;
    for (int i = 0; i < S; ++i) {
        int d1 = 0, d2 = 0;
        for (int k = 0; k < n1; ++k) d1 += q1[k] != s1[(u64)i * stride + k];
        for (int k = 0; k < n2; ++k) d2 += q2[k] != s2[(u64)i * stride + k];
        const bool a = d1 <= nsubs, b = d2 <= nsubs;
        if (a && m1 < 0) m1 = i;
        if (b && m2 < 0) m2 = i;
        if (a && b) {
            if (!both) r = i;
            ++both;
        }
    }
    if (m1 >= 0 && m2 >= 0) {
        cls = both == 0 ? CLS_HOP : both == 1 ? CLS_DEMUX : CLS_AMBIG;
        row = both == 1 ? r : -1;
    } else {
        cls = CLS_UNDET;
        m1 = m2 = row = -1;
    }
}

__global__ void classify_cp_kernel(int n, const u32* q1, const int32_t* q1len, const u32* q2, const int32_t* q2len,
                                   int stride, int S, const u32* s1, const int32_t* s1len, const u32* s2,
                                   const int32_t* s2len, const u32* s2rc, const int32_t* name, int nsubs, int rc,
                                   ClassOut o) {
    const int u = blockIdx.x * blockDim.x + threadIdx.x;
    if (u >= n) return;
    const int n1 = q1len[u], n2 = q2len[u];
    int err = 0;
    for (int i = 0; i < S && !err; ++i)
        if (s1len[i] != n1) err = 1;
    for (int i = 0; i < S && !err; ++i)
        if (s2len[i] != n2) err = 2;
    int m1 = -1, m2 = -1, cls = CLS_UNDET, row = -1, rm2 = -1, rcls = CLS_UNDET, rrow = -1;
    if (!err) {
        class_of_cp(q1 + (u64)u * stride, n1, q2 + (u64)u * stride, n2, s1, s2, stride, S, nsubs, m1, m2, cls, row);
        if (rc) {
            int rm1;
            class_of_cp(q1 + (u64)u * stride, n1, q2 + (u64)u * stride, n2, s1, s2rc, stride, S, nsubs, rm1, rm2,
                        rcls, rrow);
            if (cls == CLS_UNDET && rcls != CLS_UNDET) m1 = rm1;
            if (cls == CLS_DEMUX && rcls == CLS_DEMUX && name[row] != name[rrow]) {
                cls = rcls = CLS_AMBIG;
                row = rrow = -1;
            }
        }
    }
    if (o.err_which) o.err_which[u] = err;
    o.m1[u] = (int16_t)m1;
    o.m2[u] = (int16_t)m2;
    o.cls[u] = (u8)cls;
    o.row[u] = (int16_t)row;
    if (rc) {
        o.rc_m2[u] = (int16_t)rm2;
        o.rc_cls[u] = (u8)rcls;
        o.rc_row[u] = (int16_t)rrow;
    }
}

hipError_t launch_classify_cp(int n, const u32* q1, const int32_t* q1len, const u32* q2, const int32_t* q2len,
                              int stride, int S, const u32* s1, const int32_t* s1len, const u32* s2,
                              const int32_t* s2len, const u32* s2rc, const int32_t* name, int nsubs, int rc,
                              ClassOut o, hipStream_t s) {
    if (n <= 0) return hipSuccess;
    hipLaunchKernelGGL(classify_cp_kernel, dim3((n + 127) / 128), dim3(128), 0, s, n, q1, q1len, q2, q2len, stride,
                       S, s1, s1len, s2, s2len, s2rc, name, nsubs, rc, o);
    return hipGetLastError();
}

__device__ __forceinline__ u64 syn_h(u64 base, u64 r, u32 k) { return mix64(((r << 8) | k) ^ base); }

__global__ void synth_kernel(u8* out, u64 r0, u64 n, int R, u64 base, const u8* idx1, const u8* idx2, int S, int L1,
                             int L2) {
    const u64 i = blockIdx.x * (u64)blockDim.x + threadIdx.x;
    if (i >= n) return;
// ... 74 lines not shown
```

Baseline: 38720 M reads/s.

## Fold state resets and readbacks into kernels via pinned host mirror

Removes small hipMemsetAsync/hipMemcpyAsync calls on the hot path. It zeroes per-file state inside table_init, clears fold counters inside the scan, and clears next-round buffers inside the classify and fin_scatter kernels. The log_reduce kernel writes the DevState head and the last input byte straight into pinned host memory, which replaces separate D2H copies plus a synchronize. This trims launch and copy overhead per range, at the cost of more complex kernels and correctness that depends on system-scope fences and zero-copy memory.

```diff
diff --git a/frender_amd/_lib.py b/frender_amd/_lib.py
--- a/frender_amd/_lib.py
+++ b/frender_amd/_lib.py
@@ -826,8 +826,8 @@
         return t
 
     def diag(self) -> dict:
-        v = np.zeros(24, dtype=np.uint64)
-        self._ck(lib.fr_get_diag(self.h, _ptr(v), 24), "fr_get_diag")
+        v = np.zeros(26, dtype=np.uint64)
+        self._ck(lib.fr_get_diag(self.h, _ptr(v), 26), "fr_get_diag")
         d = dict(zip(("spin_max", "spin_total", "keys", "overflow", "presence", "exotic", "grid", "slots"),
                      v[:8].tolist()))
         d["spec_replays"] = int(v[16])
@@ -838,6 +838,8 @@
         d["fold_max"] = int(v[21])
         d["fold_over"] = int(v[22])
         d["feed_step"] = int(v[23])
+        d["stream_fills"] = int(v[24])
+        d["stream_copies"] = int(v[25])
         if v[8:16].any():
             names = ("guess", "walk0", "wait0", "resolve", "walk1", "commit", "kernel", "chunks")
             d["stamps"] = dict(zip(names, v[8:].tolist()))
diff --git a/frender_amd/csrc/fr_api.hip b/frender_amd/csrc/fr_api.hip
--- a/frender_amd/csrc/fr_api.hip
+++ b/frender_amd/csrc/fr_api.hip
@@ -60,9 +60,16 @@
     DevState* h_zero = nullptr;
     u8* h_byte = nullptr;
     u64* h_fin = nullptr;
+    HostMirror* h_mir = nullptr;
+    HostMirror* d_mir = nullptr;
+    u64 n_fills = 0, n_copies = 0;
+    bool perfile_clean = false;
+    bool fold_zero = false;
+    bool bins_dirty = false;
     hipEvent_t fin_e0 = nullptr, fin_e1 = nullptr;
     hipEvent_t cls_e0 = nullptr, cls_e1 = nullptr;
     bool fin_pending = false;
+    bool fin_binned = false;
     u64 fin_expect = 0;
     bool st_fresh = false;
     Table* d_tab = nullptr;
@@ -182,6 +189,8 @@
     u8 *d_cls = nullptr, *d_rcls = nullptr;
     int32_t* d_errw = nullptr;
     u64* d_errf = nullptr;
+    u64 errf_words = 0;
+    int errf_cur = 0;
     u64 *d_rcf = nullptr, *d_rcr = nullptr;
     int rc_names_cap = 0;
 
@@ -225,18 +234,19 @@
     return p;
 }
 
-static int state_reset_counts(fr_ctx* ctx) {
-    if (ctx->st_pending) CK(hipStreamSynchronize(ctx->stream));
-    *ctx->h_st = *ctx->h_zero;
-    CK(hipMemcpyAsync(ctx->st, ctx->h_zero, sizeof(DevState), hipMemcpyHostToDevice, ctx->stream));
-    ctx->st_pending = false;
-    ctx->st_fresh = true;
-    return FR_OK;
+static hipError_t fill_async(fr_ctx* ctx, void* dst, int value, size_t bytes) {
+    ctx->n_fills++;
+    return hipMemsetAsync(dst, value, bytes, ctx->stream);
+}
+
+static hipError_t copy_async(fr_ctx* ctx, void* dst, const void* src, size_t bytes, hipMemcpyKind kind) {
+    ctx->n_copies++;
+    return hipMemcpyAsync(dst, src, bytes, kind, ctx->stream);
 }
 
 static int read_state(fr_ctx* ctx) {
     if (ctx->st_fresh && !ctx->st_pending) return FR_OK;
-    CK(hipMemcpyAsync(ctx->h_st, ctx->st, sizeof(DevState), hipMemcpyDeviceToHost, ctx->stream));
+    CK(copy_async(ctx, ctx->h_st, ctx->st, sizeof(DevState), hipMemcpyDeviceToHost));
     CK(hipStreamSynchronize(ctx->stream));
     ctx->st_pending = false;
     ctx->st_fresh = true;
@@ -254,7 +264,7 @@
         if (ns == ctx->nslots) ns <<= 1;
         GSlot* ns_slots = nullptr;
         CK(dalloc(&ns_slots, ns));
-        CK(launch_table_init(ns_slots, ns, ctx->stream));
+        CK(launch_table_init(ns_slots, ns, nullptr, ctx->stream));
         Table t = ctx->tab;
         t.slots = ns_slots;
         t.mask = ns - 1;
@@ -269,7 +279,7 @@
         Overflow* fresh = nullptr;
         CK(dalloc(&fresh, ctx->tab.ovf_cap));
         ctx->tab.ovf = fresh;
-        CK(hipMemsetAsync(&ctx->st->n_overflow, 0, sizeof(u64), ctx->stream));
+        CK(fill_async(ctx, &ctx->st->n_overflow, 0, sizeof(u64)));
         CK(launch_reinsert_overflow(ctx->tab, ctx->st, old, novf, ctx->stream));
         ctx->st_fresh = false;
         CK(hipStreamSynchronize(ctx->stream));
@@ -287,8 +297,8 @@
     while (ncap < need * 2) ncap *= 2;
     Presence* np = nullptr;
     CK(dalloc(&np, ncap));
-    CK(hipMemcpyAsync(np, ctx->tab.pres, std::min(ctx->h_st->n_presence, ctx->tab.pres_cap) * sizeof(Presence),
-                      hipMemcpyDeviceToDevice, ctx->stream));
+    CK(copy_async(ctx, np, ctx->tab.pres, std::min(ctx->h_st->n_presence, ctx->tab.pres_cap) * sizeof(Presence),
+                      hipMemcpyDeviceToDevice));
     CK(hipStreamSynchronize(ctx->stream));
     CK(hipFree(ctx->tab.pres));
     ctx->tab.pres = np;
@@ -321,9 +331,17 @@
 }
 
 static int snapshot_async(fr_ctx* ctx) {
-    CK(hipMemcpyAsync(ctx->h_st, ctx->st, sizeof(DevState), hipMemcpyDeviceToHost, ctx->stream));
+    CK(copy_async(ctx, ctx->h_st, ctx->st, sizeof(DevState), hipMemcpyDeviceToHost));
     CK(hipEventRecord(ctx->st_ev, ctx->stream));
     ctx->st_pending = true;
+    return FR_OK;
+}
+
+static int take_mirror(fr_ctx* ctx) {
+    CK(hipStreamSynchronize(ctx->stream));
+    *ctx->h_st = ctx->h_mir->st;
+    ctx->st_pending = false;
+    ctx->st_fresh = true;
     return FR_OK;
 }
 
@@ -334,7 +352,8 @@
     float ms = 0;
     if (ctx->fin_timed) CK(hipEventElapsedTime(&ms, ctx->fin_e0, ctx->fin_e1));
     ctx->finalize_ms = ms;
-    if (*ctx->h_fin != ctx->fin_expect) return fail(ctx, FR_ERR_DEVICE, "compaction count mismatch");
+    const u64 counted = ctx->fin_binned ? ctx->h_mir->fin_count : *ctx->h_fin;
+    if (counted != ctx->fin_expect) return fail(ctx, FR_ERR_DEVICE, "compaction count mismatch");
     return FR_OK;
 }
 
@@ -342,7 +361,7 @@
     if (std::memcmp(&ctx->tab, ctx->h_tab, sizeof(Table)) != 0) {
         CK(hipStreamSynchronize(ctx->stream));
         std::memcpy(ctx->h_tab, &ctx->tab, sizeof(Table));
-        CK(hipMemcpyAsync(ctx->d_tab, ctx->h_tab, sizeof(Table), hipMemcpyHostToDevice, ctx->stream));
+        CK(copy_async(ctx, ctx->d_tab, ctx->h_tab, sizeof(Table), hipMemcpyHostToDevice));
     }
     return FR_OK;
 }
@@ -382,11 +401,11 @@
     std::vector<u64> ord(n), off(n);
     std::vector<u32> len(n);
     std::vector<u8> pool(used);
-    CK(hipMemcpyAsync(ord.data(), ctx->tab.exo_ord, n * 8, hipMemcpyDeviceToHost, ctx->stream));
-    CK(hipMemcpyAsync(off.data(), ctx->tab.exo_off, n * 8, hipMemcpyDeviceToHost, ctx->stream));
-    CK(hipMemcpyAsync(len.data(), ctx->tab.exo_len, n * 4, hipMemcpyDeviceToHost, ctx->stream));
-    if (used) CK(hipMemcpyAsync(pool.data(), ctx->tab.exo_pool, used, hipMemcpyDeviceToHost, ctx->stream));
-    CK(hipMemsetAsync(&ctx->st->n_exotic, 0, 2 * sizeof(u64), ctx->stream));
+    CK(copy_async(ctx, ord.data(), ctx->tab.exo_ord, n * 8, hipMemcpyDeviceToHost));
+    CK(copy_async(ctx, off.data(), ctx->tab.exo_off, n * 8, hipMemcpyDeviceToHost));
+    CK(copy_async(ctx, len.data(), ctx->tab.exo_len, n * 4, hipMemcpyDeviceToHost));
+    if (used) CK(copy_async(ctx, pool.data(), ctx->tab.exo_pool, used, hipMemcpyDeviceToHost));
+    CK(fill_async(ctx, &ctx->st->n_exotic, 0, 2 * sizeof(u64)));
     CK(hipStreamSynchronize(ctx->stream));
     s.n_exotic = 0;
     s.exo_pool_used = 0;
@@ -430,16 +449,17 @@
     s.n_exotic = 0;
     s.exo_pool_used = 0;
     s.cap_flags &= ~4u;
-    CK(hipMemsetAsync(&ctx->st->n_exotic, 0, 2 * sizeof(u64), ctx->stream));
-    CK(hipMemcpyAsync(&ctx->st->cap_flags, &s.cap_flags, sizeof(u32), hipMemcpyHostToDevice, ctx->stream));
+    CK(fill_async(ctx, &ctx->st->n_exotic, 0, 2 * sizeof(u64)));
+    CK(copy_async(ctx, &ctx->st->cap_flags, &s.cap_flags, sizeof(u32), hipMemcpyHostToDevice));
     ScanArgs a = ctx->last_args;
     a.exo_only = 1;
     a.spec_commit = 0;
+    a.zero_fold = 0;
     a.log = nullptr;
     a.epoch = ++ctx->epoch;
     a.tab = ctx->d_tab;
     a.tabv = ctx->tab;
-    CK(hipMemsetAsync(&ctx->st->ticket, 0, 2 * sizeof(u32), ctx->stream));
+    CK(fill_async(ctx, &ctx->st->ticket, 0, 2 * sizeof(u32)));
     rc = launch_args(ctx, a, ctx->last_grid);
     if (rc) return rc;
     ctx->exo_replays++;
@@ -468,7 +488,7 @@
 }
 
 static int launch_range(fr_ctx* ctx, const u8* dptr, u64 len, u64 avail, int own_start, int own_end, int pre_valid,
-                        int exo_only = 0) {
+                        int exo_only = 0, bool mirror = false, bool* mirrored = nullptr, bool zero_fold = false) {
     if (len == 0) return FR_OK;
     int rc = FR_OK;
     if (ctx->host_feed && ctx->last_valid) {
@@ -497,12 +517,13 @@
     a.chunk_info = ctx->chunk_info;
     a.spec_commit = exo_only ? 0u : ctx->spec_commit;
     a.exo_only = (u32)exo_only;
+    a.zero_fold = zero_fold ? 1u : 0u;
     rc = upload_table(ctx);
     if (rc) return rc;
     a.tab = ctx->d_tab;
     a.tabv = ctx->tab;
     if (ctx->epoch >= 0x7FFFFFFFu) {
-        CK(hipMemsetAsync(ctx->tiles, 0, ctx->tiles_cap * sizeof(u64), ctx->stream));
+        CK(fill_async(ctx, ctx->tiles, 0, ctx->tiles_cap * sizeof(u64)));
         ctx->epoch = 1;
         a.epoch = 1;
     }
@@ -560,9 +581,12 @@
     ctx->last_grid = grid;
     ctx->last_valid = true;
     if (timed) CK(hipEventRecord(ctx->ev_b[ctx->ev_used], ctx->stream));
-    if (a.log)
+    const bool mir = mirror && a.log;
+    if (a.log) {
         CK(launch_log_aggregate(ctx->tab, ctx->st, ctx->log, ctx->log_rcap, ctx->log_sub, ctx->log_scap, a.file_tag,
-                                a.file_offset, ctx->stream));
+                                a.file_offset, mir ? ctx->d_mir : nullptr, mir ? dptr + len - 1 : nullptr, ctx->stream));
+        ctx->fold_zero = false;
+    }
     if (timed) {
         CK(hipEventRecord(ctx->ev_l[ctx->ev_used], ctx->stream));
         ctx->ev_used++;
@@ -572,6 +596,10 @@
     ctx->par ^= 1u;
     ctx->file_offset += len;
     ctx->max_file_bytes = std::max(ctx->max_file_bytes, ctx->file_offset);
+    if (mir) {
+        *mirrored = true;
+        return FR_OK;
+    }
     return snapshot_async(ctx);
 }
 
@@ -663,6 +691,10 @@
         return bad("pinned state", e);
     if ((e = hipHostMalloc((void**)&ctx->h_byte, 64, hipHostMallocDefault)) != hipSuccess) return bad("pinned byte", e);
     if ((e = hipHostMalloc((void**)&ctx->h_fin, 64, hipHostMallocDefault)) != hipSuccess) return bad("pinned count", e);
+    if ((e = hipHostMalloc((void**)&ctx->h_mir, sizeof(HostMirror), hipHostMallocDefault)) != hipSuccess)
+        return bad("pinned mirror", e);
+    std::memset(ctx->h_mir, 0, sizeof(HostMirror));
+    if ((e = hipHostGetDevicePointer((void**)&ctx->d_mir, ctx->h_mir, 0)) != hipSuccess) return bad("pinned mirror", e);
     if ((e = hipEventCreate(&ctx->fin_e0)) != hipSuccess) return bad("event", e);
     if ((e = hipEventCreate(&ctx->fin_e1)) != hipSuccess) return bad("event", e);
     if ((e = hipEventCreate(&ctx->cls_e0)) != hipSuccess) return bad("event", e);
@@ -721,6 +753,7 @@
     if (ctx->h_zero) (void)hipHostFree(ctx->h_zero);
     if (ctx->h_byte) (void)hipHostFree(ctx->h_byte);
     if (ctx->h_fin) (void)hipHostFree(ctx->h_fin);
+    if (ctx->h_mir) (void)hipHostFree(ctx->h_mir);
     if (ctx->fin_e0) (void)hipEventDestroy(ctx->fin_e0);
     if (ctx->fin_e1) (void)hipEventDestroy(ctx->fin_e1);
     if (ctx->cls_e0) (void)hipEventDestroy(ctx->cls_e0);
@@ -752,7 +785,8 @@
                           (uint64_t)ctx->grid, ctx->nslots, s.stamp[0], s.stamp[1], s.stamp[2], s.stamp[3],
                           s.stamp[4],  s.stamp[5],  s.stamp[6], s.stamp[7], ctx->spec_replays, ctx->exo_replays,
                           s.heavy[ctx->par] ? ctx->chunk_tiles_heavy : ctx->chunk_tiles,
-                          s.heavy_launches, ctx->big_rollbacks, ctx->feed_fold_max, ctx->feed_fold_over, ctx->feed_step};
+                          s.heavy_launches, ctx->big_rollbacks, ctx->feed_fold_max, ctx->feed_fold_over, ctx->feed_step,
+                          ctx->n_fills, ctx->n_copies};
     for (int i = 0; i < n && i < (int)(sizeof(v) / sizeof(v[0])); ++i) out[i] = v[i];
     return FR_OK;
 }
@@ -844,7 +878,7 @@
         std::memcpy(ctx->h_sheet, h, total);
         ctx->sheet_bytes = total;
         ++ctx->sheet_ver;
-        CK(hipMemcpyAsync(ctx->d_sheet, ctx->h_sheet, total, hipMemcpyHostToDevice, ctx->stream));
+        CK(copy_async(ctx, ctx->d_sheet, ctx->h_sheet, total, hipMemcpyHostToDevice));
     }
     u8* d = ctx->d_sheet;
     ctx->d_i1 = (u64*)d;
@@ -875,9 +909,13 @@
     if (int src = settle_finalize(ctx)) return src;
     CK(hipSetDevice(ctx->device));
     CK(hipStreamSynchronize(ctx->copy));
-    CK(launch_table_init(ctx->tab.slots, ctx->nslots, ctx->stream));
-    int rc = state_reset_counts(ctx);
-    if (rc) return rc;
+    ctx->n_fills = ctx->n_copies = 0;
+    if (ctx->st_pending) CK(hipStreamSynchronize(ctx->stream));
+    CK(launch_table_init(ctx->tab.slots, ctx->nslots, ctx->st, ctx->stream));
+    *ctx->h_st = *ctx->h_zero;
+    ctx->st_fresh = true;
+    ctx->perfile_clean = true;
+    ctx->fold_zero = true;
     ctx->scanning = true;
     ctx->file_open = false;
     ctx->file_tag = 0;
@@ -923,7 +961,8 @@
     ctx->exo_records_file = 0;
     ctx->last_valid = false;
     static_assert(offsetof(DevState, utf8_bad) + sizeof(u32) - offsetof(DevState, lines) == 32, "per-file block");
-    CK(hipMemcpyAsync(&ctx->st->lines[0], &ctx->h_zero->lines[0], 32, hipMemcpyHostToDevice, ctx->stream));
+    if (!ctx->perfile_clean) CK(copy_async(ctx, &ctx->st->lines[0], &ctx->h_zero->lines[0], 32, hipMemcpyHostToDevice));
+    ctx->perfile_clean = false;
     ctx->h_st->lines[0] = ctx->h_st->lines[1] = 0;
     ctx->h_st->err_nospace = ~0ull;
     ctx->h_st->nonascii = ctx->h_st->utf8_bad = 0;
@@ -1021,7 +1060,7 @@
             ctx->snap_cap = snap_slots;
         }
         snap = ctx->snap;
-        CK(hipMemcpyAsync(snap, ctx->tab.slots, snap_slots * sizeof(GSlot), hipMemcpyDeviceToDevice, ctx->stream));
+        CK(copy_async(ctx, snap, ctx->tab.slots, snap_slots * sizeof(GSlot), hipMemcpyDeviceToDevice));
     }
     const double big_range = (double)std::min<u64>(ctx->chunk_bytes, len);
     const bool fold_room = (u64)ctx->feed_fold_over * 64 <= ctx->feed_fold_max && ctx->feed_step > 0 &&
@@ -1030,8 +1069,10 @@
                (saved.n_keys + ctx->feed_keys) * 2 <= ctx->nslots;
     bool spec_now = spec;
     u64 step = 0, lim_room = ~0ull;
+    int last_b = -1;
     for (int attempt = 0; attempt < 12; ++attempt) {
-        CK(hipMemsetAsync(&ctx->st->log_fold_max, 0, 2 * sizeof(u32), ctx->stream));
+        const bool zero_fold = !ctx->fold_zero;
+        bool mirrored = false;
         const u64 lim = std::min<u64>(big ? ctx->chunk_bytes : std::min<u64>(ctx->chunk_bytes, RANGE_FIRST_MAX),
                                       lim_room);
         const u64 nr = (len + lim - 1) / lim;
@@ -1039,12 +1080,19 @@
         ctx->spec_commit = spec_now ? 1u : 0u;
         for (u64 off = 0; off < len; off += step) {
             const u64 n = std::min<u64>(step, len - off);
-            rc = launch_range(ctx, dev_data + off, n, len - off, off == 0 ? 1 : 0, 1, off ? 1 : 0);
+            rc = launch_range(ctx, dev_data + off, n, len - off, off == 0 ? 1 : 0, 1, off ? 1 : 0, 0,
+                              off + n == len, &mirrored, zero_fold && off == 0);
             if (rc) break;
         }
         ctx->spec_commit = 0;
-        if (!rc && len) CK(hipMemcpyAsync(ctx->h_byte, dev_data + len - 1, 1, hipMemcpyDeviceToHost, ctx->stream));
-        if (!rc) rc = read_state(ctx);
+        if (!rc && mirrored) {
+            rc = take_mirror(ctx);
+            last_b = (int)(ctx->h_mir->last_byte & 0xFFu);
+        } else if (!rc) {
+            if (len) CK(copy_async(ctx, ctx->h_byte, dev_data + len - 1, 1, hipMemcpyDeviceToHost));
+            rc = read_state(ctx);
+            if (!rc && len) last_b = *ctx->h_byte;
+        }
         if (rc) break;
         const bool spec_bad = spec_now && ctx->h_st->spec_fail;
         const bool room_bad = spec && (ctx->h_st->cap_flags & 2u) && step > RANGE_ROOM_MIN;
@@ -1067,13 +1115,14 @@
             ctx->tab.mask = snap_slots - 1;
             ctx->nslots = snap_slots;
         }
-        if (empty) CK(launch_table_init(ctx->tab.slots, ctx->nslots, ctx->stream));
-        else CK(hipMemcpyAsync(ctx->tab.slots, snap, snap_slots * sizeof(GSlot), hipMemcpyDeviceToDevice, ctx->stream));
+        if (empty) CK(launch_table_init(ctx->tab.slots, ctx->nslots, nullptr, ctx->stream));
+        else CK(copy_async(ctx, ctx->tab.slots, snap, snap_slots * sizeof(GSlot), hipMemcpyDeviceToDevice));
         *ctx->h_st = saved;
-        CK(hipMemcpyAsync(ctx->st, ctx->h_st, sizeof(DevState), hipMemcpyHostToDevice, ctx->stream));
+        CK(copy_async(ctx, ctx->st, ctx->h_st, sizeof(DevState), hipMemcpyHostToDevice));
         CK(hipStreamSynchronize(ctx->stream));
         ctx->st_pending = false;
         ctx->st_fresh = true;
+        ctx->fold_zero = false;
         ctx->par = par0;
         ctx->file_offset = ctx->file_base;
         if (!room_bad) ctx->spec_replays++;
@@ -1095,7 +1144,7 @@
         s.exo_pool_used = 0;
         s.cap_flags &= ~4u;
         s.lines[par0] = saved.lines[par0];
-        CK(hipMemcpyAsync(ctx->st, ctx->h_st, sizeof(DevState), hipMemcpyHostToDevice, ctx->stream));
+        CK(copy_async(ctx, ctx->st, ctx->h_st, sizeof(DevState), hipMemcpyHostToDevice));
         ctx->par = par0;
         ctx->file_offset = ctx->file_base;
         ctx->exo_replays++;
@@ -1111,7 +1160,7 @@
     }
     rc = drain_exotic(ctx);
     if (rc) return rc;
-    if (len) ctx->last_byte = *ctx->h_byte;
+    if (len) ctx->last_byte = last_b;
     ctx->carry.clear();
     return FR_OK;
 }
@@ -1272,6 +1321,7 @@
             CK(hipMalloc(&ctx->d_bins, cap * sizeof(u32)));
             CK(hipMalloc(&ctx->d_binbase, cap * sizeof(u32)));
             ctx->bins_cap = cap;
+            ctx->bins_dirty = true;
         }
         size_t need = 0;
         CK(launch_fin_scan(ctx->d_bins, ctx->d_binbase, nbins + 1, nullptr, &need, ctx->stream));
@@ -1282,14 +1332,18 @@
         }
         size_t tb = ctx->temp_bytes;
         const bool set_uidx = ctx->pres_defer_tag == 0;
-        CK(hipMemsetAsync(ctx->d_bins, 0, (nbins + 1) * sizeof(u32), ctx->stream));
+        if (ctx->bins_dirty) CK(fill_async(ctx, ctx->d_bins, 0, ctx->bins_cap * sizeof(u32)));
+        ctx->bins_dirty = true;
         CK(launch_fin_hist(ctx->tab.slots, ctx->nslots, bm, ctx->d_bins, ctx->d_arr, ctx->stream));
         CK(launch_fin_scan(ctx->d_bins, ctx->d_binbase, nbins + 1, ctx->d_temp, &tb, ctx->stream));
-        CK(launch_fin_scatter(ctx->tab.slots, ctx->nslots, bm, ctx->d_binbase, ctx->d_arr, ctx->d_rows, ctx->stream));
+        ctx->h_mir->fin_count = 0;
+        CK(launch_fin_scatter(ctx->tab.slots, ctx->nslots, bm, ctx->d_binbase, ctx->d_arr, ctx->d_rows, ctx->d_bins,
+                              &ctx->d_mir->fin_count, ctx->stream));
+        ctx->bins_dirty = false;
         CK(launch_fin_rank(ctx->tab.slots, nk, bm, ctx->d_binbase, ctx->d_rows, ctx->d_keys_s, ctx->d_counts_s,
                            ctx->d_first_s, set_uidx, ctx->stream));
     } else {
-        CK(hipMemsetAsync(ctx->d_counter, 0, sizeof(u64), ctx->stream));
+        CK(fill_async(ctx, ctx->d_counter, 0, sizeof(u64)));
         CK(launch_compact(ctx->tab.slots, ctx->nslots, ctx->d_keys, ctx->d_counts, ctx->d_first, ctx->d_pos,
                           ctx->d_counter, ctx->stream));
         int begin_bit = 0, end_bit = 64;
@@ -1334,11 +1388,9 @@
     else
         CK(launch_presence_map(ctx->tab.slots, ctx->tab.mask, ctx->tab.pres, np, ctx->d_pres_u, ctx->d_pres_f,
                                ctx->d_pres_c, ctx->stream));
+    ctx->fin_binned = nbins != 0;
     *ctx->h_fin = 0;
-    if (nbins)
-        CK(hipMemcpyAsync(ctx->h_fin, ctx->d_binbase + nbins, sizeof(u32), hipMemcpyDeviceToHost, ctx->stream));
-    else
-        CK(hipMemcpyAsync(ctx->h_fin, ctx->d_counter, sizeof(u64), hipMemcpyDeviceToHost, ctx->stream));
+    if (!nbins) CK(copy_async(ctx, ctx->h_fin, ctx->d_counter, sizeof(u64), hipMemcpyDeviceToHost));
     CK(hipEventRecord(e1, ctx->stream));
     ctx->fin_pending = true;
     ctx->fin_expect = nk;
@@ -1436,9 +1488,11 @@
     CK(dalloc(&ctx->d_rcls, cap));
     CK(dalloc(&ctx->d_errw, cap));
     const int names = std::max(ctx->n_names, 1);
-    CK(dalloc(&ctx->d_errf, 1 + 2 * (u64)names));
-    ctx->d_rcf = ctx->d_errf + 1;
-    ctx->d_rcr = ctx->d_rcf + names;
+    ctx->errf_words = 1 + 2 * (u64)names;
+    CK(dalloc(&ctx->d_errf, 2 * ctx->errf_words));
+    CK(fill_async(ctx, ctx->d_errf, 0, 2 * ctx->errf_words * 8));
+    ctx->errf_cur = 0;
+    ctx->d_rcf = ctx->d_rcr = nullptr;
     ctx->ccap = cap;
     ctx->rc_names_cap = names;
     return FR_OK;
@@ -1475,7 +1529,7 @@
     m.mmask[0] = (u32)(n1 - 1);
     m.mmask[1] = m.mmask[2] = (u32)(n2 - 1);
     m.pmask[0] = m.pmask[1] = (u32)(np - 1);
-    CK(hipMemsetAsync(ctx->d_nbr, 0, bytes, ctx->stream));
+    CK(fill_async(ctx, ctx->d_nbr, 0, bytes));
     CK(launch_nbr_build(sh, ctx->d_canon, nsubs, rc, m, ctx->stream));
     m.on = 1;
     return FR_OK;
@@ -1488,19 +1542,28 @@
     int rc = ensure_class_scratch(ctx, n);
     if (rc) return rc;
     hipEvent_t e0 = ctx->cls_e0, e1 = ctx->cls_e1;
-    CK(hipMemsetAsync(ctx->d_errf, 0, (1 + 2 * (u64)ctx->rc_names_cap) * 8, ctx->stream));
+    u64* blk = ctx->d_errf + (u64)ctx->errf_cur * ctx->errf_words;
+    u64* next = ctx->d_errf + (u64)(ctx->errf_cur ^ 1) * ctx->errf_words;
     SheetArgs sh{ctx->S, ctx->n_names, ctx->L1u, ctx->L2u, ctx->d_i1, ctx->d_i2, ctx->d_i2rc, ctx->d_name};
     if ((rc = ensure_nbr(ctx, sh, num_subs, rc_mode ? 1 : 0))) return rc;
     ClassOut o{ctx->d_m1, ctx->d_m2, ctx->d_cls, ctx->d_row, ctx->d_rm2, ctx->d_rcls, ctx->d_rrow,
-               ctx->d_rcf, ctx->d_rcr, ctx->d_errf, ctx->d_errw};
+               blk + 1, blk + 1 + ctx->rc_names_cap, blk, ctx->d_errw};
     const bool timed = ctx->timing;
     if (timed) CK(hipEventRecord(e0, ctx->stream));
-    CK(launch_classify(ctx->d_keys_s, ctx->d_counts_s, n, sh, num_subs, rc_mode ? 1 : 0, o, ctx->nbr, ctx->stream));
+    ctx->h_mir->err_flag = 0;
+    CK(launch_classify(ctx->d_keys_s, ctx->d_counts_s, n, sh, num_subs, rc_mode ? 1 : 0, o, ctx->nbr, next,
+                       (u32)ctx->errf_words, &ctx->d_mir->err_flag, ctx->stream));
+    ctx->errf_cur ^= 1;
+    ctx->d_rcf = o.rc_f;
+    ctx->d_rcr = o.rc_r;
     if (timed) CK(hipEventRecord(e1, ctx->stream));
-    CK(hipMemcpyAsync(ctx->h_byte + 8, ctx->d_errf, 8, hipMemcpyDeviceToHost, ctx->stream));
     CK(hipStreamSynchronize(ctx->stream));
-    u64 ef;
-    std::memcpy(&ef, ctx->h_byte + 8, 8);
+    u64 ef = 0;
+    if (ctx->h_mir->err_flag) {
+        CK(copy_async(ctx, ctx->h_byte + 8, blk, 8, hipMemcpyDeviceToHost));
+        CK(hipStreamSynchronize(ctx->stream));
+        std::memcpy(&ef, ctx->h_byte + 8, 8);
+    }
     ef = ~ef;
     if (int src = settle_finalize(ctx)) return src;
     float ms = 0;
@@ -1593,9 +1656,9 @@
     if (int src = settle_finalize(ctx)) return src;
     if (ctx->U > cap) return fail(ctx, FR_ERR_CAPACITY, "export buffer too small");
     if (ctx->U) {
-        CK(hipMemcpyAsync(dev_keys, ctx->d_keys_s, ctx->U * 8, hipMemcpyDeviceToDevice, ctx->stream));
-        CK(hipMemcpyAsync(dev_counts, ctx->d_counts_s, ctx->U * 8, hipMemcpyDeviceToDevice, ctx->stream));
-        CK(hipMemcpyAsync(dev_first, ctx->d_first_s, ctx->U * 8, hipMemcpyDeviceToDevice, ctx->stream));
+        CK(copy_async(ctx, dev_keys, ctx->d_keys_s, ctx->U * 8, hipMemcpyDeviceToDevice));
+        CK(copy_async(ctx, dev_counts, ctx->d_counts_s, ctx->U * 8, hipMemcpyDeviceToDevice));
+        CK(copy_async(ctx, dev_first, ctx->d_first_s, ctx->U * 8, hipMemcpyDeviceToDevice));
     }
     CK(hipStreamSynchronize(ctx->stream));
     return FR_OK;
diff --git a/frender_amd/csrc/fr_internal.h b/frender_amd/csrc/fr_internal.h
--- a/frender_amd/csrc/fr_internal.h
+++ b/frender_amd/csrc/fr_internal.h
@@ -119,6 +119,13 @@
     u32 log_red_done;
     u32 log_fold_max;
     u32 log_fold_over;
+};
+
+struct HostMirror {
+    DevState st;
+    u32 last_byte;
+    alignas(64) u64 fin_count;
+    alignas(64) u64 err_flag;
 };
 
 struct Table {
@@ -172,6 +179,7 @@
     u32 log_hot;
     u32 exo_only;
     u32 spec_commit;
+    u32 zero_fold;
     DevState* st;
     u64* tiles;
     const Table* tab;
@@ -245,7 +253,7 @@
     return (u32)(mix64(key) >> (64 - LOG_REGION_BITS - LOG_SUB_BITS)) & (LOG_SUBS - 1);
 }
 
-hipError_t launch_table_init(GSlot* slots, u64 n, hipStream_t s);
+hipError_t launch_table_init(GSlot* slots, u64 n, DevState* st, hipStream_t s);
 hipError_t launch_chunk_scan(const ScanArgs& a, int grid, hipStream_t s);
 int chunk_occupancy();
 hipError_t launch_reinsert_overflow(Table t, DevState* st, const Overflow* src, u64 n, hipStream_t s);
@@ -276,11 +284,11 @@
 hipError_t launch_fin_hist(const GSlot* slots, u64 nslots, const BinMap& m, u32* cnt, u32* arr, hipStream_t s);
 hipError_t launch_fin_scan(const u32* cnt, u32* base, u64 n, void* temp, size_t* temp_bytes, hipStream_t s);
 hipError_t launch_fin_scatter(const GSlot* slots, u64 nslots, const BinMap& m, const u32* base, const u32* arr,
-                              FinRow* rows, hipStream_t s);
+                              FinRow* rows, u32* cnt, u64* fin_out, hipStream_t s);
 hipError_t launch_fin_rank(GSlot* slots, u64 nk, const BinMap& m, const u32* base, const FinRow* rows, u64* keys_o,
                            u64* counts_o, u64* first_o, bool set_uidx, hipStream_t s);
 hipError_t launch_classify(const u64* keys, const u64* counts, u64 n, SheetArgs sh, int nsubs, int rc,
-                           ClassOut o, const NbrMap& nm, hipStream_t s);
+                           ClassOut o, const NbrMap& nm, u64* zero_next, u32 zero_n, u64* err_flag, hipStream_t s);
 u64 nbr_codes_per_row(int L, int nsubs);
 hipError_t launch_nbr_build(const SheetArgs& sh, const int32_t* canon, int nsubs, int rc, const NbrMap& nm,
                             hipStream_t s);
@@ -296,7 +304,7 @@
                                  u64* counts, u64* cursor, u64* rows, hipStream_t s);
 hipError_t launch_merge_rows(Table t, DevState* st, const u64* rows, u64 n, hipStream_t s);
 hipError_t launch_log_aggregate(Table t, DevState* st, const LogEntry* log, u32 rcap, LogEntry* sub, u32 scap,
-                                u32 file_tag, u64 file_offset, hipStream_t s);
+                                u32 file_tag, u64 file_offset, HostMirror* mir, const u8* last_byte, hipStream_t s);
 size_t log_aggregate_temp_bytes();
 hipError_t launch_synth(u8* out, u64 r0, u64 n, int R, u64 seed, const u8* idx1, const u8* idx2, int S, int L1,
                         int L2, hipStream_t s);
diff --git a/frender_amd/csrc/fr_kernels.hip b/frender_amd/csrc/fr_kernels.hip
--- a/frender_amd/csrc/fr_kernels.hip
+++ b/frender_amd/csrc/fr_kernels.hip
@@ -1470,6 +1470,7 @@
         sh.ncold = 0;
         sh.nexo = 0;
         sh.err_off = 0xFFFFFFFFu;
+        if (a.zero_fold && blockIdx.x == 0) a.st->log_fold_max = a.st->log_fold_over = 0;
     }
 #if defined(FR_STAMPS) && FR_STAMPS == 3
     if (tid == 0 && blockIdx.x < TRACE_WGS) g_wg_trace[(a.par * TRACE_WGS + blockIdx.x) * 2] = __builtin_amdgcn_s_memrealtime();
@@ -1648,7 +1649,15 @@
 }
 
 
-__global__ void table_init_kernel(GSlot* slots, u64 n) {
+__global__ void table_init_kernel(GSlot* slots, u64 n, DevState* st) {
+    if (st && blockIdx.x == 0) {
+        static_assert(sizeof(DevState) % sizeof(u32) == 0 && offsetof(DevState, err_nospace) % sizeof(u32) == 0,
+                      "DevState is written as 32-bit words");
+        constexpr u32 E = (u32)(offsetof(DevState, err_nospace) / sizeof(u32));
+        u32* w = (u32*)st;
+        for (u32 i = threadIdx.x; i < (u32)(sizeof(DevState) / sizeof(u32)); i += blockDim.x)
+            w[i] = (i == E || i == E + 1) ? 0xFFFFFFFFu : 0u;
+    }
     for (u64 i = blockIdx.x * (u64)blockDim.x + threadIdx.x; i < n; i += (u64)gridDim.x * blockDim.x) {
         GSlot g;
         g.key = 0;
@@ -1660,9 +1669,9 @@
     }
 }
 
-hipError_t launch_table_init(GSlot* slots, u64 n, hipStream_t s) {
+hipError_t launch_table_init(GSlot* slots, u64 n, DevState* st, hipStream_t s) {
     const int grid = (int)std::min<u64>((n + 255) / 256, 8192);
-    hipLaunchKernelGGL(table_init_kernel, dim3(grid > 0 ? grid : 1), dim3(256), 0, s, slots, n);
+    hipLaunchKernelGGL(table_init_kernel, dim3(grid > 0 ? grid : 1), dim3(256), 0, s, slots, n, st);
     return hipGetLastError();
 }
 
@@ -1927,9 +1936,8 @@
 #endif
 constexpr int RED_WG = FR_RED_WG;
 constexpr int RED_FB = RED_WG >= 512 ? 4 : 8;
-__global__ __launch_bounds__(RED_WG) void log_reduce_kernel(Table t, DevState* st, const LogEntry* sub, u32 scap,
-                                                         u32 file_tag, u64 ord0) {
-    if (st->log_n == 0) return;
+__device__ __forceinline__ void log_reduce_fold(Table t, DevState* st, const LogEntry* sub, u32 scap, u32 file_tag,
+                                                u64 ord0) {
     __shared__ AggSlot ls[AGG_LNS];
     __shared__ u32 zone_bits[CLAIM_WORDS];
     __shared__ u16 occ[AGG_LNS];
@@ -2030,24 +2038,51 @@
         made += insert_rows<FB, true>(t, st, key, cnt, ord, tag, v, cz);
     }
     add_created(st, made);
+}
+
+__global__ __launch_bounds__(RED_WG) void log_reduce_kernel(Table t, DevState* st, const LogEntry* sub, u32 scap,
+                                                         u32 file_tag, u64 ord0, HostMirror* mir,
+                                                         const u8* last_byte) {
+    const bool logged = st->log_n != 0;
+    if (logged) log_reduce_fold(t, st, sub, scap, file_tag, ord0);
+    else if (!mir) return;
     if (last_block(&st->log_red_done)) {
-        for (int i = threadIdx.x; i < LOG_NR; i += RED_WG)
-            __hip_atomic_store(&st->log_rcur[i], 0u, __ATOMIC_RELAXED, __HIP_MEMORY_SCOPE_AGENT);
-        for (int i = threadIdx.x; i < LOG_NSUB; i += RED_WG)
-            __hip_atomic_store(&st->log_scur[i], 0u, __ATOMIC_RELAXED, __HIP_MEMORY_SCOPE_AGENT);
-        if (threadIdx.x == 0) __hip_atomic_store(&st->log_n, 0ull, __ATOMIC_RELAXED, __HIP_MEMORY_SCOPE_AGENT);
+        if (logged) {
+            for (int i = threadIdx.x; i < LOG_NR; i += RED_WG)
+                __hip_atomic_store(&st->log_rcur[i], 0u, __ATOMIC_RELAXED, __HIP_MEMORY_SCOPE_AGENT);
+            for (int i = threadIdx.x; i < LOG_NSUB; i += RED_WG)
+                __hip_atomic_store(&st->log_scur[i], 0u, __ATOMIC_RELAXED, __HIP_MEMORY_SCOPE_AGENT);
+            if (threadIdx.x == 0) __hip_atomic_store(&st->log_n, 0ull, __ATOMIC_RELAXED, __HIP_MEMORY_SCOPE_AGENT);
+        }
+        if (mir && threadIdx.x < 64) {
+            constexpr u32 HEAD = (u32)(offsetof(DevState, log_rcur) / sizeof(u32));
+            static_assert(offsetof(DevState, log_rcur) % sizeof(u32) == 0 && HEAD <= 64, "one wave mirrors the state's head");
+            const u32* src = (const u32*)st;
+            u32* dst = (u32*)&mir->st;
+            constexpr u32 LOGN = (u32)(offsetof(DevState, log_n) / sizeof(u32));
+            if (threadIdx.x < HEAD)
+                dst[threadIdx.x] = (threadIdx.x == LOGN || threadIdx.x == LOGN + 1) ? 0u
+                                   : __hip_atomic_load(src + threadIdx.x, __ATOMIC_RELAXED, __HIP_MEMORY_SCOPE_AGENT);
+            if (threadIdx.x == 0) {
+                mir->st.log_fold_max = __hip_atomic_load(&st->log_fold_max, __ATOMIC_RELAXED, __HIP_MEMORY_SCOPE_AGENT);
+                mir->st.log_fold_over = __hip_atomic_load(&st->log_fold_over, __ATOMIC_RELAXED, __HIP_MEMORY_SCOPE_AGENT);
+                mir->last_byte = last_byte ? (u32)*last_byte : 0u;
+            }
+            __threadfence_system();
+        }
     }
 }
 
 size_t log_aggregate_temp_bytes() { return 0; }
 
 hipError_t launch_log_aggregate(Table t, DevState* st, const LogEntry* log, u32 rcap, LogEntry* sub, u32 scap,
-                                u32 file_tag, u64 file_offset, hipStream_t s) {
+                                u32 file_tag, u64 file_offset, HostMirror* mir, const u8* last_byte, hipStream_t s) {
     const u64 ord0 = ((u64)file_tag << ORD_SHIFT) | file_offset;
     if (!LOG_DIRECT)
         hipLaunchKernelGGL(log_split_kernel, dim3(LOG_NR * SPLIT_WGS), dim3(256), 0, s, t, st, log, rcap, sub, scap,
                            file_tag, ord0);
-    hipLaunchKernelGGL(log_reduce_kernel, dim3(LOG_NSUB), dim3(RED_WG), 0, s, t, st, sub, scap, file_tag, ord0);
+    hipLaunchKernelGGL(log_reduce_kernel, dim3(LOG_NSUB), dim3(RED_WG), 0, s, t, st, sub, scap, file_tag, ord0,
+                       mir, last_byte);
     return hipGetLastError();
 }
 
@@ -2220,8 +2255,13 @@
 }
 
 __global__ __launch_bounds__(256) void fin_scatter_kernel(const GSlot* slots, u64 n, BinMap m, const u32* base,
-                                                          const u32* arr, FinRow* rows) {
+                                                          const u32* arr, FinRow* rows, u32* cnt, u64* fin_out) {
     const u64 i = blockIdx.x * (u64)blockDim.x + threadIdx.x;
+    for (u64 j = i; j <= m.nbins; j += (u64)gridDim.x * blockDim.x) cnt[j] = 0;
+    if (i == 0 && fin_out) {
+        *fin_out = base[m.nbins];
+        __threadfence_system();
+    }
     if (i >= n) return;
     const u32 k = arr[i];
     if (k == 0xFFFFFFFFu) return;
@@ -2270,8 +2310,9 @@
 }
 
 hipError_t launch_fin_scatter(const GSlot* slots, u64 nslots, const BinMap& m, const u32* base, const u32* arr,
-                              FinRow* rows, hipStream_t s) {
-    hipLaunchKernelGGL(fin_scatter_kernel, dim3(lane_grid(nslots)), dim3(256), 0, s, slots, nslots, m, base, arr, rows);
+                              FinRow* rows, u32* cnt, u64* fin_out, hipStream_t s) {
+    hipLaunchKernelGGL(fin_scatter_kernel, dim3(lane_grid(nslots)), dim3(256), 0, s, slots, nslots, m, base, arr, rows,
+                       cnt, fin_out);
     return hipGetLastError();
 }
 
@@ -2682,8 +2723,10 @@
 template <typename W>
 __global__ __launch_bounds__(CLS_WG) void classify_kernel(const u64* keys, const u64* counts, u64 n, SheetArgs sh,
                                                           int nsubs, int rc, ClassOut o, NbrMap nm,
-                                                          int sheet_in_lds, int names_in_lds) {
+                                                          int sheet_in_lds, int names_in_lds, u64* zero_next,
+                                                          u32 zero_n, u64* err_flag) {
     extern __shared__ __attribute__((aligned(16))) u8 cls_lds[];
+    for (u64 i = blockIdx.x * (u64)CLS_WG + threadIdx.x; i < zero_n; i += (u64)gridDim.x * CLS_WG) zero_next[i] = 0;
     unsigned long long* lf = (unsigned long long*)cls_lds;
     unsigned long long* lr = lf + (names_in_lds ? sh.n_names : 0);
     W* s1 = (W*)(lr + (names_in_lds ? sh.n_names : 0));
@@ -2703,6 +2746,7 @@
     const W* S2 = sheet_in_lds ? s2 : (const W*)sh.i2;
     const W* S2rc = sheet_in_lds ? s2rc : (const W*)sh.i2rc;
 
+    bool any_err = false;
     for (u64 u = blockIdx.x * (u64)CLS_WG + threadIdx.x; u < n; u += (u64)gridDim.x * CLS_WG) {
         const u64 key = keys[u];
         int n1 = 0, n2 = 0;
@@ -2778,6 +2822,7 @@
             }
         }
         if (err) {
+            any_err = true;
             atomicMax((unsigned long long*)o.err_first, (unsigned long long)~u);
             if (o.err_which) o.err_which[u] = err;
         } else if (o.err_which) {
@@ -2804,6 +2849,7 @@
             }
         }
     }
+    if (any_err) *err_flag = 1;
     if (rc && names_in_lds) {
         __syncthreads();
         for (int i = threadIdx.x; i < sh.n_names; i += CLS_WG) {
@@ -2814,8 +2860,7 @@
 }
 
 hipError_t launch_classify(const u64* keys, const u64* counts, u64 n, SheetArgs sh, int nsubs, int rc, ClassOut o,
-                           const NbrMap& nm, hipStream_t s) {
-    if (!n) return hipSuccess;
+                           const NbrMap& nm, u64* zero_next, u32 zero_n, u64* err_flag, hipStream_t s) {
     const bool narrow = sh.S > 0 && sh.L1u >= 0 && sh.L1u <= 10 && sh.L2u >= 0 && sh.L2u <= 10;
     const size_t wb = narrow ? 4 : 8;
     const size_t names_bytes = rc ? 2ull * 8 * sh.n_names : 0;
@@ -2824,14 +2869,14 @@
     const size_t nb = names_in_lds ? names_bytes : 0;
     const int sheet_in_lds = (!FR_CLS_SCALAR && nb + sheet_bytes <= CLS_LDS_BYTES) ? 1 : 0;
     const size_t lds = nb + (sheet_in_lds ? sheet_bytes : 0) + 16;
-    const u64 grid = std::min<u64>((n + CLS_WG - 1) / CLS_WG, 2048);
+    const u64 grid = std::max<u64>(1, std::min<u64>((n + CLS_WG - 1) / CLS_WG, 2048));
     const bool wide = !(narrow && (sheet_in_lds || FR_CLS_SCALAR));
     if (!wide)
         hipLaunchKernelGGL(classify_kernel<u32>, dim3((u32)grid), dim3(CLS_WG), lds, s, keys, counts, n, sh, nsubs, rc,
-                           o, nm, sheet_in_lds, names_in_lds);
+                           o, nm, sheet_in_lds, names_in_lds, zero_next, zero_n, err_flag);
     else
         hipLaunchKernelGGL(classify_kernel<u64>, dim3((u32)grid), dim3(CLS_WG), lds, s, keys, counts, n, sh, nsubs, rc,
-                           o, nm, sheet_in_lds, names_in_lds);
+                           o, nm, sheet_in_lds, names_in_lds, zero_next, zero_n, err_flag);
     return hipGetLastError();
 }
 
```

New measurement: 39270 M reads/s (median of 6 runs). +1.4%, better.
